# LouisRouss/DiffuLab

Measured on AMD Instinct MI355X. Metric: train images/sec/node (DiT-S/2 flow-matching, 256x256 latents), higher is better.
Workload: dtype bf16

## Files before the change

diffulab_amd/_lib.py:

```python

from __future__ import annotations

import ctypes
import os
import re
from functools import lru_cache

_HERE = os.path.dirname(os.path.abspath(__file__))
LIB_PATH = os.environ.get("DIFFULAB_HIP_LIB") or os.path.join(_HERE, "libdiffulab_hip.so")
HEADER_PATH = os.path.join(os.path.dirname(_HERE), "include", "diffulab_hip.h")

_CTYPES = {
    "int": ctypes.c_int,
    "int32_t": ctypes.c_int32,
    "int64_t": ctypes.c_int64,
    "float": ctypes.c_float,
    "dl_stream_t": ctypes.c_void_p,
}


_VALUE_RETURNING = {"dl_version", "dl_mse_loss_partials", "dl_grad_sumsq", "dl_muon_orthogonalize"}


def _ctype_of(decl: str):
    decl = decl.strip()
    if "*" in decl:
        return ctypes.c_char_p if re.match(r"^(const\s+)?char\s*\*", decl) and "arch" not in decl else ctypes.c_void_p
    base = decl.replace("const", "").split()[0]
    return _CTYPES[base]


def parse_header(path: str = HEADER_PATH) -> dict[str, tuple[object, list[object], list[str]]]:
    text = open(path).read()
    text = re.sub(r"/\*.*?\*/", " ", text, flags=re.S)
    protos: dict[str, tuple[object, list[object], list[str]]] = {}
    for m in re.finditer(r"DL_API\s+([\w\s\*]+?)\s*\b(dl_\w+)\s*\(([^;]*?)\)\s*;", text, flags=re.S):
        ret, name, args = m.group(1).strip(), m.group(2), m.group(3).strip()
        if ret.replace(" ", "") == "constchar*":
            restype = ctypes.c_char_p
        else:
            restype = _CTYPES[ret]
        argtypes, argnames = [], []
        if args and args != "void":
            for a in args.split(","):
                a = " ".join(a.split())
                argnames.append(re.split(r"[\s\*]+", a)[-1])
                argtypes.append(_ctype_of(a))
        protos[name] = (restype, argtypes, argnames)
    return protos


class _Lib:
    def __init__(self) -> None:
        if not os.path.exists(LIB_PATH):
            raise RuntimeError(
                f"{LIB_PATH} not found: build it with `python -c 'import __graft_entry__ as g; g.build()'` "
                "(or `make -C diffulab_amd/csrc`).  There is no CPU / PyTorch fallback for the hot path."
            )
        self.cdll = ctypes.CDLL(LIB_PATH)
        self.protos = parse_header()
        self._fns: dict[str, tuple] = {}
        for name, (restype, argtypes, _) in self.protos.items():
            fn = getattr(self.cdll, name)
            fn.restype = restype
            fn.argtypes = argtypes
            self._fns[name] = (fn, restype is ctypes.c_int and name not in _VALUE_RETURNING)

    def call(self, name: str, *args):
        fn, status = self._fns[name]
        rc = fn(*args)
        if status and rc != 0:
            raise RuntimeError(f"{name} failed ({rc}): {self.cdll.dl_last_error().decode()}")
        return rc


@lru_cache(maxsize=1)
def lib() -> _Lib:
    return _Lib()


def available() -> bool:
    return os.path.exists(LIB_PATH)
```

diffulab_amd/csrc/block.hip:

```cpp
#include <stdlib.h>

#include "common.h"

static thread_local hipEvent_t g_blk_event = nullptr;
static int fork_to_side(hipStream_t main, hipStream_t side) {
  if (main == side) return 0;
  if (!g_blk_event && hipEventCreateWithFlags(&g_blk_event, hipEventDisableTiming) != hipSuccess) return -1;
  if (hipEventRecord(g_blk_event, main) != hipSuccess) return -1;
  return hipStreamWaitEvent(side, g_blk_event, 0) == hipSuccess ? 0 : -1;
}

extern "C" int dl_stream_wait_stream(dl_stream_t waiter, dl_stream_t waited) {
  if (fork_to_side((hipStream_t)waited, (hipStream_t)waiter) != 0) {
    dl_set_error("dl_stream_wait_stream: %s", hipGetErrorString(hipGetLastError()));
    return DL_ERR_LAUNCH;
  }
  return DL_OK;
}
extern "C" int dl_memset_zero(void* p, int64_t bytes, dl_stream_t stream) {
  DL_CHECK_ARG(p && bytes >= 0, "dl_memset_zero: bad args");
  if (bytes && hipMemsetAsync(p, 0, (size_t)bytes, (hipStream_t)stream) != hipSuccess) {
    dl_set_error("dl_memset_zero: %s", hipGetErrorString(hipGetLastError()));
    return DL_ERR_LAUNCH;
  }
  return DL_OK;
}

#define P(k) (b->p[DL_BLK_##k])
#define RUN(call)               \
  do {                          \
    const int rc__ = (call);    \
    if (rc__ != DL_OK) return rc__; \
  } while (0)

static int mlp_up_swiglu(const dl_dit_block_t* b, int train, dl_stream_t stream) {
  const int64_t D = b->D, F = b->F, M = b->B * b->N;
  void* u = train ? P(U) : nullptr;
  if (!u) {
    const int rc = dl_gemm_nt_swiglu_stationary(P(XM2), D, P(W_UP_PERM), b->ldw_d, u, 2 * F, P(H), F, M, F, D, 0, stream);
    if (rc != DL_ERR_UNSUPPORTED) return rc;
  }
  return dl_gemm_nt_swiglu(P(XM2), D, P(W_UP_PERM), b->ldw_d, u, 2 * F, P(H), F, M, F, D, stream);
}

extern "C" int dl_dit_block_fwd(const dl_dit_block_t* b, int train, dl_stream_t stream) {
  DL_CHECK_ARG(b, "dl_dit_block_fwd: null block");
  const int64_t B = b->B, N = b->N, D = b->D, H = b->H, F = b->F, M = B * N, dh = D / H;
  DL_CHECK_ARG(B > 0 && N > 0 && D > 0 && H > 0 && F > 0 && dh == 64, "dl_dit_block_fwd: bad dims (head_dim must be 64)");
  const DlWgCapScope cap_scope(b->max_workgroups);
  const float sm = 0.125f;
  if (b->row_gemms & 1) {
    DL_CHECK_ARG(P(V) == nullptr && P(NEXT_X) && P(NEXT_XM) && P(NEXT_SCALE) && P(NEXT_SHIFT) && P(NEXT_MEAN) && P(NEXT_RSTD),
                 "dl_dit_block_fwd: row_gemms needs V in place and the DL_BLK_NEXT_* slots");
    if ((b->row_gemms & 8) && P(SSQ)) {
      const int rc = dl_dit_block_fwd_chain(b, train, stream);
      if (rc != DL_ERR_UNSUPPORTED) return rc;
    }
    if (P(SSQ)) {
      int rq = dl_gemm_nt_ssq_stationary(P(XM1), D, P(W_QKV), b->ldw_d, P(QKV), 3 * D, M, 3 * D, D, (float*)P(SSQ), 2, 0, stream);
      if (rq == DL_ERR_UNSUPPORTED) rq = dl_gemm_nt_ssq(P(XM1), D, P(W_QKV), b->ldw_d, P(QKV), 3 * D, M, 3 * D, D, (float*)P(SSQ), 2, stream);
      if (rq != DL_OK) return rq;
      RUN(dl_attn_fwd_qkn(P(QKV), (const float*)P(SSQ), (const float*)P(QN_SCALE), (const float*)P(KN_SCALE), (const float*)P(ROPE_COS),
                          (const float*)P(ROPE_SIN), 1e-6f, b->rot, train ? P(Q) : nullptr, train ? P(K) : nullptr,
                          train ? (float*)P(RRMS) : nullptr, P(A), (float*)P(LSE), B, H, N, dh, sm, stream));
    } else if (b->row_gemms & 2) {
      RUN(dl_gemm_nt_qk_norm_rope(P(XM1), D, P(W_QKV), b->ldw_d, B, N, H, dh, b->rot, 1e-6f, (const float*)P(QN_SCALE),
                                  (const float*)P(KN_SCALE), (const float*)P(ROPE_COS), (const float*)P(ROPE_SIN), P(QKV), P(Q), P(K),
                                  (float*)P(RRMS), N, 0, stream));
    } else {
      RUN(dl_gemm_nt(P(XM1), D, P(W_QKV), b->ldw_d, P(QKV), 3 * D, M, 3 * D, D, nullptr, DL_ACT_NONE, DL_BF16, nullptr, nullptr, 0, nullptr,
                     0, 1, stream));
      RUN(dl_qk_norm_rope_fwd(P(QKV), (const float*)P(QN_SCALE), (const float*)P(KN_SCALE), (const float*)P(ROPE_COS),
                              (const float*)P(ROPE_SIN), P(Q), P(K), nullptr, (float*)P(RRMS), B, N, H, dh, b->rot, 1e-6f, stream));
    }
    if (!P(SSQ))
      RUN(dl_attn_fwd_sv(P(Q), P(K), (const char*)P(QKV) + 2 * D * 2, N * 3 * D, dh, 3 * D, P(A), (float*)P(LSE), B, H, N, dh, sm, stream));
    RUN(dl_ln_modulate_gemm_fwd(P(A), D, P(W_PROJ), b->ldw_d, M, D, P(X_IN), P(GATE1), b->ld_mod, (const float*)P(LN2_W),
                                (const float*)P(LN2_B), P(SCALE2), P(SHIFT2), b->ld_mod, N, b->eps, P(T1), P(X1), P(XM2), (float*)P(MEAN2),
                                (float*)P(RSTD2), D, stream));
    RUN(mlp_up_swiglu(b, train, stream));
    RUN(dl_ln_modulate_gemm_fwd(P(H), F, P(W_DOWN), b->ldw_f, M, F, P(X1), P(GATE2), b->ld_mod, (const float*)P(NEXT_LN_W),
                                (const float*)P(NEXT_LN_B), P(NEXT_SCALE), P(NEXT_SHIFT), b->ld_mod, N, b->next_eps, P(T2), P(NEXT_X),
                                P(NEXT_XM), (float*)P(NEXT_MEAN), (float*)P(NEXT_RSTD), D, stream));
    return DL_OK;
  }
  RUN(dl_ln_modulate_fwd(P(PEND_X) ? P(PEND_X) : P(X_IN), (const float*)P(LN1_W), (const float*)P(LN1_B), P(SCALE1), P(SHIFT1),
                         b->ld_mod, N, b->eps, P(XM1), (float*)P(MEAN1), (float*)P(RSTD1), P(PEND_X) ? P(PEND_T) : nullptr,
                         P(PEND_X) ? P(PEND_GATE) : nullptr, b->ld_mod, P(PEND_X) ? P(X_IN) : nullptr, M, D, stream));
  RUN(dl_gemm_nt(P(XM1), D, P(W_QKV), b->ldw_d, P(QKV), 3 * D, M, 3 * D, D, nullptr, DL_ACT_NONE, DL_BF16, nullptr, nullptr, 0, nullptr, 0,
                 1, stream));
  const bool v_in_place = P(V) == nullptr;
  RUN(dl_qk_norm_rope_fwd(P(QKV), (const float*)P(QN_SCALE), (const float*)P(KN_SCALE), (const float*)P(ROPE_COS),
                          (const float*)P(ROPE_SIN), P(Q), P(K), P(V), (float*)P(RRMS), B, N, H, dh, b->rot, 1e-6f, stream));
  if (v_in_place)
    RUN(dl_attn_fwd_sv(P(Q), P(K), (const char*)P(QKV) + 2 * D * 2, N * 3 * D, dh, 3 * D, P(A), (float*)P(LSE), B, H, N, dh, sm, stream));
  else
    RUN(dl_attn_fwd(P(Q), P(K), P(V), P(A), (float*)P(LSE), B, H, N, dh, sm, stream));
  RUN(dl_gemm_nt(P(A), D, P(W_PROJ), b->ldw_d, P(T1), D, M, D, D, nullptr, DL_ACT_NONE, DL_BF16, nullptr, nullptr, 0, nullptr, 0, 1, stream));
  RUN(dl_ln_modulate_fwd(P(X_IN), (const float*)P(LN2_W), (const float*)P(LN2_B), P(SCALE2), P(SHIFT2), b->ld_mod, N, b->eps, P(XM2),
                         (float*)P(MEAN2), (float*)P(RSTD2), P(T1), P(GATE1), b->ld_mod, P(X1), M, D, stream));
  int rc = mlp_up_swiglu(b, train, stream);
  if (rc == DL_ERR_UNSUPPORTED) {
    DL_CHECK_ARG(P(U), "dl_dit_block_fwd: this shape has no fused MLP-up kernel and needs the U buffer");
    RUN(dl_gemm_nt(P(XM2), D, P(W_UP), b->ldw_d, P(U), 2 * F, M, 2 * F, D, nullptr, DL_ACT_NONE, DL_BF16, nullptr, nullptr, 0, nullptr, 0, 1,
                   stream));
    RUN(dl_swiglu_fwd(P(U), P(H), M, F, stream));
  } else if (rc != DL_OK) {
    return rc;
  }
  RUN(dl_gemm_nt(P(H), F, P(W_DOWN), b->ldw_f, P(T2), D, M, D, F, nullptr, DL_ACT_NONE, DL_BF16, nullptr, nullptr, 0, nullptr, 0, 1, stream));
  return DL_OK;
}

extern "C" int dl_dit_block_bwd(const dl_dit_block_t* b, dl_stream_t main_, dl_stream_t side_, int side_wgs) {
  DL_CHECK_ARG(b, "dl_dit_block_bwd: null block");
  hipStream_t main = (hipStream_t)main_, side = (hipStream_t)side_;
  const DlWgCapScope cap_scope(b->max_workgroups);
  const int64_t B = b->B, N = b->N, D = b->D, H = b->H, F = b->F, M = B * N, dh = D / H;
  const float sm = 0.125f;
  dl_wgrad_t wg[4];
  int nwg = 0;
  bool grouped = P(TN_SLAB) != nullptr && ((D % 384 == 0 && F % 192 == 0) || (D % 256 == 0 && F % 256 == 0)) && M % 32 == 0 && M >= 2048;
  auto wgrad = [&](const void* dy, int64_t ldy, const void* x, int64_t ldx, void* g, int64_t Mo, int64_t No) -> int {
    if (grouped) {
      wg[nwg++] = dl_wgrad_t{dy, ldy, x, ldx, (float*)g, Mo, No};
      return DL_OK;
    }
    if (fork_to_side(main, side)) return DL_ERR_LAUNCH;
    return dl_gemm_tn_ex(dy, ldy, x, ldx, (float*)g, No, Mo, No, M, side_wgs, side);
  };
  auto fold = [&](void* partial, void* g) -> int {
    if (fork_to_side(main, side)) return DL_ERR_LAUNCH;
    return dl_reduce_rows_f32((float*)partial, (float*)g, B, 2 * D, 1, side);
  };
  RUN(wgrad(P(DT2), D, P(H), F, P(G_DOWN), D, F));
  if (P(U)) {
    RUN(dl_gemm_nt(P(DT2), D, P(WT_DOWN), b->ldwt_d, P(DH), F, M, F, D, nullptr, DL_ACT_NONE, DL_BF16, nullptr, nullptr, 0, nullptr, 0, 1, main));
    RUN(dl_swiglu_bwd(P(DH), P(U), P(DU), M, F, main));
  } else {
    RUN(dl_mlp_dswiglu_recompute(P(XM2), D, P(W_UP_PERM), b->ldw_d, P(DT2), D, P(WT_DOWN), b->ldwt_d, P(DU), 2 * F, M, F, D, D, main));
  }
  RUN(wgrad(P(DU), 2 * F, P(XM2), D, P(G_UP), 2 * F, D));
  const bool rows = (b->row_gemms & 1) != 0, fold_here = (b->row_gemms & 4) == 0;
  if (rows) {
    RUN(dl_ln_modulate_gemm_bwd(P(DU), 2 * F, P(WT_UP), b->ldwt_f2, M, 2 * F, P(X1), (const float*)P(LN2_W), (const float*)P(LN2_B),
                                P(SCALE2), b->ld_mod, N, (const float*)P(MEAN2), (const float*)P(RSTD2), P(DX_IN), P(DX_MID),
                                (float*)P(DSCALE2), (float*)P(DSHIFT2), b->ld_dmod, (float*)P(DWB2), P(T1), P(GATE1), b->ld_mod, P(DT1),
                                (float*)P(DGATE1), D, main));
  } else {
    RUN(dl_gemm_nt(P(DU), 2 * F, P(WT_UP), b->ldwt_f2, P(DXM), D, M, D, 2 * F, nullptr, DL_ACT_NONE, DL_BF16, nullptr, nullptr, 0, nullptr,
                   0, 1, main));
    RUN(dl_ln_modulate_bwd(P(DXM), P(X1), (const float*)P(LN2_W), (const float*)P(LN2_B), P(SCALE2), b->ld_mod, N,
                           (const float*)P(MEAN2), (const float*)P(RSTD2), P(DX_IN), P(DX_MID), (float*)P(DSCALE2), (float*)P(DSHIFT2),
                           b->ld_dmod, (float*)P(DWB2), P(T1), P(GATE1), b->ld_mod, P(DT1), (float*)P(DGATE1), M, D, main));
  }
  if (fold_here) RUN(fold(P(DWB2), P(G_LN2)));
  RUN(wgrad(P(DT1), D, P(A), D, P(G_PROJ), D, D));
  RUN(dl_gemm_nt(P(DT1), D, P(WT_PROJ), b->ldwt_d, P(DA), D, M, D, D, nullptr, DL_ACT_NONE, DL_BF16, nullptr, nullptr, 0, nullptr, 0, 1, main));
  const bool v_in_place = P(V) == nullptr;
  if (v_in_place && P(QK_PARTIALS) && D <= 512) {
    RUN(dl_attn_bwd_tok(P(Q), P(K), P(QKV), P(A), P(DA), (const float*)P(LSE), P(DQKV), B, H, N, dh, sm, main));
    RUN(dl_qk_norm_rope_bwd_inplace(P(QKV), (const float*)P(QN_SCALE), (const float*)P(KN_SCALE), (const float*)P(ROPE_COS),
                                    (const float*)P(ROPE_SIN), (const float*)P(RRMS), P(DQKV), (float*)P(G_QK_SCALE),
                                    (float*)P(QK_PARTIALS), B, N, H, dh, b->rot, nullptr, main));
  } else {
    if (v_in_place)
      RUN(dl_attn_bwd_sv(P(Q), P(K), (const char*)P(QKV) + 2 * D * 2, N * 3 * D, dh, 3 * D, P(A), P(DA), (const float*)P(LSE), P(DQ), P(DK),
                         (char*)P(DQKV) + 2 * D * 2, N * 3 * D, dh, 3 * D, B, H, N, dh, sm, main));
    else
      RUN(dl_attn_bwd(P(Q), P(K), P(V), P(A), P(DA), (const float*)P(LSE), P(DQ), P(DK), P(DV), B, H, N, dh, sm, main));
    RUN(dl_qk_norm_rope_bwd(P(DQ), P(DK), v_in_place ? nullptr : P(DV), P(QKV), (const float*)P(QN_SCALE), (const float*)P(KN_SCALE),
                            (const float*)P(ROPE_COS), (const float*)P(ROPE_SIN), (const float*)P(RRMS), P(DQKV), (float*)P(G_QK_SCALE), B, N,
                            H, dh, b->rot, main));
  }
  RUN(wgrad(P(DQKV), 3 * D, P(XM1), D, P(G_QKV), 3 * D, D));
  if (grouped) {
    if (fork_to_side(main, side)) return DL_ERR_LAUNCH;
    RUN(dl_gemm_tn_group(wg, nwg, M, (float*)P(TN_SLAB), b->tn_slab_floats, side_wgs, side));
  }
  if (!rows)
    RUN(dl_gemm_nt(P(DQKV), 3 * D, P(WT_QKV), b->ldwt_3d, P(DXM), D, M, D, 3 * D, nullptr, DL_ACT_NONE, DL_BF16, nullptr, nullptr, 0,
                   nullptr, 0, 1, main));
  if (P(DFEAT)) RUN(dl_add_bf16(P(DX_MID), P(DFEAT), P(DX_MID), M * D, main));
  if (rows) {
    RUN(dl_ln_modulate_gemm_bwd(P(DQKV), 3 * D, P(WT_QKV), b->ldwt_3d, M, 3 * D, P(X_IN), (const float*)P(LN1_W), (const float*)P(LN1_B),
                                P(SCALE1), b->ld_mod, N, (const float*)P(MEAN1), (const float*)P(RSTD1), P(DX_MID), P(DX_OUT),
                                (float*)P(DSCALE1), (float*)P(DSHIFT1), b->ld_dmod, (float*)P(DWB1), P(PREV_T2), P(PREV_GATE2), b->ld_mod,
                                P(PREV_DT2), (float*)P(PREV_DGATE2), D, main));
  } else {
    RUN(dl_ln_modulate_bwd(P(DXM), P(X_IN), (const float*)P(LN1_W), (const float*)P(LN1_B), P(SCALE1), b->ld_mod, N,
                           (const float*)P(MEAN1), (const float*)P(RSTD1), P(DX_MID), P(DX_OUT), (float*)P(DSCALE1), (float*)P(DSHIFT1),
                           b->ld_dmod, (float*)P(DWB1), P(PREV_T2), P(PREV_GATE2), b->ld_mod, P(PREV_DT2), (float*)P(PREV_DGATE2), M, D,
                           main));
  }
  if (fold_here) RUN(fold(P(DWB1), P(G_LN1)));
  return DL_OK;
}
```

diffulab_amd/csrc/block_fused.hip:

```cpp
#include <stdlib.h>

#include "common.h"
#include "attention_body.h"
#include "gemm_rows_body.h"
#include "gemm_stationary_body.h"

#define CH_THREADS 512
#define CH_NKS 6

struct ChainRowGemm {
  const bf16_t* A;
  int64_t lda;
  const bf16_t* W;
  int64_t ldw;
  int K;
  RowEpi ep;
};
struct ChainAttn {
  const bf16_t* qkv;
  bf16_t* out;
  float* lse;
  int H;
  float scale;
  QkNorm qn;
};
struct ChainArgs {
  int B;
  StArgs qkv;
  ChainAttn attn;
  ChainRowGemm proj;
  StArgs up;
  ChainRowGemm down;
};

constexpr int ch_max(int a, int b) { return a > b ? a : b; }
constexpr int ch_lds_bytes() { return ch_max(ch_max(st_lds_bytes<CH_NKS>(), 2 * RK_STAGE), attn_pipe_lds_bytes(RK_BN)); }

static __device__ __forceinline__ void ch_phase_sync() {
  asm volatile("s_waitcnt vmcnt(0) lgkmcnt(0)" ::: "memory");
  __builtin_amdgcn_fence(__ATOMIC_RELEASE, "workgroup");
  __syncthreads();
  __builtin_amdgcn_fence(__ATOMIC_ACQUIRE, "workgroup");
}

static __device__ __forceinline__ const ChainArgs* ch_args() {
  auto p = __builtin_amdgcn_kernarg_segment_ptr();
  asm volatile("" : "+s"(p));
  return (const ChainArgs*)p;
}
static __device__ __forceinline__ int ch_tid() {
  int t = threadIdx.x;
  asm volatile("" : "+v"(t));
  return t;
}
static __device__ __forceinline__ void ch_row_gemm(const ChainRowGemm* gp, char* smem, int sample) {
  const ChainRowGemm g = *gp;
  rk_gemm_body<RK_LNF>(g.A, g.lda, g.W, g.ldw, RK_BN, g.K, g.ep, smem, ch_tid(), sample, 0, 1);
}
template <int EPI>
static __device__ __forceinline__ void ch_st_gemm(const StArgs* ap, char* smem, int sample) {
  const StArgs a = *ap;
  st_gemm_body<CH_NKS, EPI>(a, smem, ch_tid(), sample, 0, 1);
}
static __device__ __forceinline__ void ch_attention(const ChainAttn* ap, char* smem, int sample) {
  const ChainAttn a = *ap;
  attn_qkn_pipe_body(a.qkv, a.out, a.lse, a.H, a.scale, a.qn, smem, ch_tid(), sample * a.H, 1, a.H);
}

__global__ __launch_bounds__(CH_THREADS, 2) void dit_block_fwd_chain_k(ChainArgs a) {
  extern __shared__ __attribute__((aligned(16))) char smem[];
  for (int s = blockIdx.x; s < a.B; s += gridDim.x) {
    ch_st_gemm<1>(&ch_args()->qkv, smem, s);
    ch_phase_sync();
    ch_attention(&ch_args()->attn, smem, s);
    ch_phase_sync();
    ch_row_gemm(&ch_args()->proj, smem, s);
    ch_phase_sync();
    ch_st_gemm<0>(&ch_args()->up, smem, s);
    ch_phase_sync();
    ch_row_gemm(&ch_args()->down, smem, s);
    ch_phase_sync();
  }
}

#define P(k) (b->p[DL_BLK_##k])
#define CH_ALIGNED16(p) ((((uintptr_t)(p)) & 15) == 0)

static void ch_row_epi(RowEpi& ep, const void* resid, const void* gate, int64_t ld_gate, const void* ln_w, const void* ln_b,
                       const void* scale, const void* shift, int64_t ld_mod, float eps, void* t_out, void* x_out, void* xm_out,
                       void* mean, void* rstd) {
  ep.resid = (const bf16_t*)resid;
  ep.gate = (const bf16_t*)gate;
  ep.ld_gate = ld_gate;
  ep.ln_w = (const float*)ln_w;
  ep.ln_b = (const float*)ln_b;
  ep.scale = (const bf16_t*)scale;
  ep.shift = (const bf16_t*)shift;
  ep.ld_mod = ld_mod;
  ep.eps = eps;
  ep.t_out = (bf16_t*)t_out;
  ep.x_out = (bf16_t*)x_out;
  ep.xm_out = (bf16_t*)xm_out;
  ep.mean = (float*)mean;
  ep.rstd = (float*)rstd;
}

extern "C" int dl_dit_block_fwd_chain(const dl_dit_block_t* b, int train, dl_stream_t stream) {
  DL_CHECK_ARG(b, "dl_dit_block_fwd_chain: null block");
  const int64_t B = b->B, N = b->N, D = b->D, H = b->H, F = b->F;
  DL_CHECK_ARG(B > 0 && N > 0 && D > 0 && H > 0 && F > 0, "dl_dit_block_fwd_chain: bad dims");
  if (!(b->row_gemms & 1) || !P(SSQ) || P(V) || N != RK_BM || D != RK_BN || D != H * 64 || F % 64 || F % RK_BK ||
      B * N >= (1ll << 31) || F >= (1ll << 30)) {
    dl_set_error("dl_dit_block_fwd_chain: needs row_gemms bit 0, SSQ, V in place, N == 256, D == 384, head_dim == 64, F %% 64 == 0 "
                 "(N=%lld D=%lld H=%lld F=%lld)", (long long)N, (long long)D, (long long)H, (long long)F);
    return DL_ERR_UNSUPPORTED;
  }
  DL_CHECK_ARG(P(XM1) && P(W_QKV) && P(QKV) && P(QN_SCALE) && P(KN_SCALE) && P(LSE) && (!train || (P(Q) && P(K) && P(RRMS))) &&
                   b->rot >= 0 && b->rot % 8 == 0 && b->rot <= 64 && (b->rot == 0 || (P(ROPE_COS) && P(ROPE_SIN))),
               "dl_dit_block_fwd_chain: null qkv / attention operand, or rot not a multiple of 8 up to 64");
  DL_CHECK_ARG(CH_ALIGNED16(P(XM1)) && CH_ALIGNED16(P(W_QKV)) && CH_ALIGNED16(P(QKV)) && CH_ALIGNED16(P(QN_SCALE)) && CH_ALIGNED16(P(KN_SCALE)) &&
                   CH_ALIGNED16(P(ROPE_COS)) && CH_ALIGNED16(P(ROPE_SIN)) && CH_ALIGNED16(P(Q)) && CH_ALIGNED16(P(K)) &&
                   (((uintptr_t)P(SSQ)) & 7) == 0,
               "dl_dit_block_fwd_chain: 16-byte alignment (qkv / attention operands)");
  DL_CHECK_ARG(P(A) && P(W_PROJ) && P(X_IN) && P(GATE1) && P(SCALE2) && P(SHIFT2) && P(T1) && P(X1) && P(XM2) && P(MEAN2) && P(RSTD2) &&
                   P(W_UP_PERM) && P(H) && P(W_DOWN) && P(GATE2) && P(T2) && P(NEXT_X) && P(NEXT_XM) && P(NEXT_SCALE) && P(NEXT_SHIFT) &&
                   P(NEXT_MEAN) && P(NEXT_RSTD),
               "dl_dit_block_fwd_chain: null operand");
  DL_CHECK_ARG((P(LN2_W) == nullptr) == (P(LN2_B) == nullptr) && (P(NEXT_LN_W) == nullptr) == (P(NEXT_LN_B) == nullptr),
               "dl_dit_block_fwd_chain: LayerNorm w and b must both be given or both NULL");
  DL_CHECK_ARG(b->ldw_d % 8 == 0 && b->ldw_f % 8 == 0 && b->ldw_d >= D && b->ldw_f >= F && b->ldw_d < (1ll << 24) && b->ld_mod % 8 == 0,
               "dl_dit_block_fwd_chain: leading dimensions");
  void* u = train ? P(U) : nullptr;
  DL_CHECK_ARG(CH_ALIGNED16(P(A)) && CH_ALIGNED16(P(W_PROJ)) && CH_ALIGNED16(P(X_IN)) && CH_ALIGNED16(P(GATE1)) && CH_ALIGNED16(P(SCALE2)) &&
                   CH_ALIGNED16(P(SHIFT2)) && CH_ALIGNED16(P(T1)) && CH_ALIGNED16(P(X1)) && CH_ALIGNED16(P(XM2)) && CH_ALIGNED16(P(LN2_W)) &&
                   CH_ALIGNED16(P(LN2_B)) && CH_ALIGNED16(P(W_UP_PERM)) && CH_ALIGNED16(u) && CH_ALIGNED16(P(H)) && CH_ALIGNED16(P(W_DOWN)) &&
                   CH_ALIGNED16(P(GATE2)) && CH_ALIGNED16(P(T2)) && CH_ALIGNED16(P(NEXT_X)) && CH_ALIGNED16(P(NEXT_XM)) &&
                   CH_ALIGNED16(P(NEXT_SCALE)) && CH_ALIGNED16(P(NEXT_SHIFT)) && CH_ALIGNED16(P(NEXT_LN_W)) && CH_ALIGNED16(P(NEXT_LN_B)),
               "dl_dit_block_fwd_chain: 16-byte alignment");

  ChainArgs a{};
  a.B = (int)B;
  a.qkv = StArgs{(const bf16_t*)P(XM1), D, (const bf16_t*)P(W_QKV), b->ldw_d, (bf16_t*)P(QKV), 3 * D, nullptr, 0, 0, (float*)P(SSQ), 2,
                 (int)(B * N), (int)(3 * D)};
  a.attn.qkv = (const bf16_t*)P(QKV);
  a.attn.out = (bf16_t*)P(A);
  a.attn.lse = (float*)P(LSE);
  a.attn.H = (int)H;
  a.attn.scale = 0.125f;
  a.attn.qn = QkNorm{(const float*)P(SSQ), (const float*)P(QN_SCALE), (const float*)P(KN_SCALE), (const float*)P(ROPE_COS),
                     (const float*)P(ROPE_SIN), (bf16_t*)(train ? P(Q) : nullptr), (bf16_t*)(train ? P(K) : nullptr),
                     (float*)(train ? P(RRMS) : nullptr), 1.0f / (float)D, 1e-6f, (int)b->rot, (int)(3 * D)};
  a.proj.A = (const bf16_t*)P(A);
  a.proj.lda = D;
  a.proj.W = (const bf16_t*)P(W_PROJ);
  a.proj.ldw = b->ldw_d;
  a.proj.K = (int)D;
  ch_row_epi(a.proj.ep, P(X_IN), P(GATE1), b->ld_mod, P(LN2_W), P(LN2_B), P(SCALE2), P(SHIFT2), b->ld_mod, b->eps, P(T1), P(X1), P(XM2),
             P(MEAN2), P(RSTD2));
  a.up = StArgs{(const bf16_t*)P(XM2), D, (const bf16_t*)P(W_UP_PERM), b->ldw_d, (bf16_t*)u, 2 * F, (bf16_t*)P(H), F, (int)F, nullptr, 0,
                (int)(B * N), (int)(2 * F)};
  a.down.A = (const bf16_t*)P(H);
  a.down.lda = F;
  a.down.W = (const bf16_t*)P(W_DOWN);
  a.down.ldw = b->ldw_f;
  a.down.K = (int)F;
  ch_row_epi(a.down.ep, P(X1), P(GATE2), b->ld_mod, P(NEXT_LN_W), P(NEXT_LN_B), P(NEXT_SCALE), P(NEXT_SHIFT), b->ld_mod, b->next_eps,
             P(T2), P(NEXT_X), P(NEXT_XM), P(NEXT_MEAN), P(NEXT_RSTD));

  constexpr int LDS = ch_lds_bytes();
  static_assert(LDS <= 160 * 1024, "the chain kernel's LDS is the largest phase's");
  static DevOnce once;
  const int n_cu = dev_cus(once, [] {
    (void)hipFuncSetAttribute((const void*)dit_block_fwd_chain_k, hipFuncAttributeMaxDynamicSharedMemorySize, LDS);
  });
  const DlWgCapScope cap_scope(b->max_workgroups);
  const int budget = dl_wg_budget(n_cu);
  int grid = (int)(B < budget ? B : budget);
  if (b->max_workgroups > 0 && b->max_workgroups < grid) grid = b->max_workgroups;
  hipLaunchKernelGGL(dit_block_fwd_chain_k, grid, CH_THREADS, LDS, (hipStream_t)stream, a);
  DL_LAUNCH_CHECK();
  return DL_OK;
}
```

diffulab_amd/csrc/gemm_stationary_body.h:

```cpp
#ifndef DIFFULAB_GEMM_STATIONARY_BODY_H
#define DIFFULAB_GEMM_STATIONARY_BODY_H

#include <type_traits>

#include "common.h"

#define ST_THREADS 512
#define ST_PANEL 256
#define ST_ROWS 64

typedef __attribute__((address_space(3))) void st_lds_void_t;
typedef const __attribute__((address_space(1))) void st_glb_void_t;

struct StArgs {
  const bf16_t* X;
  int64_t ldx;
  const bf16_t* W;
  int64_t ldw;
  bf16_t* C;
  int64_t ldc;
  bf16_t* H;
  int64_t ldh;
  int F;
  float* ssq;
  int ssq_tiles;
  int M, N;
};

template <int NKS>
constexpr int st_lds_bytes() {
  constexpr int STAGE = ST_ROWS * NKS * 128;
  return ((3 * STAGE <= 160 * 1024) ? 3 : 2) * STAGE;
}

template <int N>
__device__ __forceinline__ void st_wait_vmcnt() {
  asm volatile("s_waitcnt vmcnt(%0)" ::"n"(N) : "memory");
}

template <int OFF>
__device__ __forceinline__ void st_lds_read(bf16x8_t& v, unsigned addr) {
  asm volatile("ds_read_b128 %0, %1 offset:%2" : "=v"(v) : "v"(addr), "n"(OFF));
}
template <int N>
__device__ __forceinline__ void st_lds_landed(bf16x8_t& v) {
  asm volatile("s_waitcnt lgkmcnt(%1)" : "+v"(v) : "n"(N));
}

static __device__ __forceinline__ void st_lds_landed_n(int n, bf16x8_t& v) {
  if (n >= 3) st_lds_landed<3>(v);
  else if (n == 2) st_lds_landed<2>(v);
  else if (n == 1) st_lds_landed<1>(v);
  else st_lds_landed<0>(v);
}

template <int NKS, int EPI>
__device__ __forceinline__ void st_gemm_body(const StArgs& a, char* smem, int tid, int first, int stride, int cnt) {
  constexpr int NF = NKS * 4;
  constexpr int PITCH = NKS * 128;
  constexpr int STAGE = ST_ROWS * PITCH;
  constexpr int NST = (3 * STAGE <= 160 * 1024) ? 3 : 2;
  constexpr bool WIDE = (PITCH % 256) == 0;
  constexpr int PD = NKS == 8 ? 2 : 3;
  const int lane = tid & 63, hi = lane >> 5, l31 = lane & 31;
  const int wave = __builtin_amdgcn_readfirstlane(tid >> 6);
  const int S = a.N / ST_ROWS;
  const int total = cnt * S;

  int src_off[NKS];
#pragma unroll
  for (int i = 0; i < NKS; ++i) {
    const int o = (wave * NKS + i) * 1024 + lane * 16;
    const int row = o / PITCH, sl = (o % PITCH) >> 4;
    const int g = WIDE ? (row & 15) : ((row >> 1) & 7);
    src_off[i] = row * (int)a.ldw + ((sl ^ g) << 3);
  }
  int s_it = 0, s_st = 0;
  auto stage_next = [&]() {
    char* base = smem + (s_it % NST) * STAGE + wave * (NKS * 1024);
    const bf16_t* w = a.W + (int64_t)s_st * ST_ROWS * a.ldw;
#pragma unroll
    for (int i = 0; i < NKS; ++i)
      __builtin_amdgcn_global_load_lds((st_glb_void_t*)(w + src_off[i]), (st_lds_void_t*)(base + i * 1024), 16, 0, 0);
    ++s_it;
    if (++s_st == S) s_st = 0;
  };
  const int g_rd = WIDE ? (l31 & 15) : ((l31 >> 1) & 7);
  const int rd_base = l31 * PITCH, rd_x = (hi ^ g_rd) << 4;
  const unsigned smem_lds = (unsigned)(uintptr_t)(st_lds_void_t*)smem;

  f32x16_t acc[4];
#pragma unroll
  for (int j = 0; j < 4; ++j)
#pragma unroll
    for (int r = 0; r < 16; ++r) acc[j][r] = 0.f;
  bf16x8_t x[NF];
  const bool upper = wave >= 4;
  int m = 0;
  float ss = 0.f;
  float ss_lo = 0.f;

#pragma unroll
  for (int s = 0; s < NST - 1; ++s)
    if (s < total) stage_next();

  auto epilogue = [&](auto half_tag, int st) {
    constexpr int HALF = decltype(half_tag)::value;
    const int n_base = st * ST_ROWS;
    if constexpr (EPI == 0) {
#pragma unroll
      for (int j = 0; j < 2; ++j) {
        f32x16_t& c = acc[2 * HALF + j];
        const int u0 = ((n_base + j * 32) >> 1) + 8 * hi;
        float v1[8], v3[8], hv[8], h8[8];
#pragma unroll
        for (int e = 0; e < 8; ++e) hv[e] = silu_f(c[e]) * c[8 + e];
#pragma unroll
        for (int e = 0; e < 4; ++e) {
          auto s1 = __builtin_amdgcn_permlane32_swap(__float_as_uint(c[e]), __float_as_uint(c[4 + e]), false, false);
          auto s3 = __builtin_amdgcn_permlane32_swap(__float_as_uint(c[8 + e]), __float_as_uint(c[12 + e]), false, false);
          auto sh = __builtin_amdgcn_permlane32_swap(__float_as_uint(hv[e]), __float_as_uint(hv[4 + e]), false, false);
          v1[e] = __uint_as_float(s1[0]);
          v1[4 + e] = __uint_as_float(s1[1]);
          v3[e] = __uint_as_float(s3[0]);
          v3[4 + e] = __uint_as_float(s3[1]);
          h8[e] = __uint_as_float(sh[0]);
          h8[4 + e] = __uint_as_float(sh[1]);
        }
#pragma unroll
        for (int e = 0; e < 16; ++e) c[e] = 0.f;
        if (a.C) {
          *(u32x4_t*)(a.C + (int64_t)m * a.ldc + u0) = pack8(v1);
          *(u32x4_t*)(a.C + (int64_t)m * a.ldc + a.F + u0) = pack8(v3);
        }
        *(u32x4_t*)(a.H + (int64_t)m * a.ldh + u0) = pack8(h8);
      }
    } else {
#pragma unroll
      for (int j = 0; j < 2; ++j)
#pragma unroll
        for (int gp = 0; gp < 2; ++gp) {
          f32x16_t& c = acc[2 * HALF + j];
          float v[8];
#pragma unroll
          for (int e = 0; e < 4; ++e) {
            auto sw2 = __builtin_amdgcn_permlane32_swap(__float_as_uint(c[8 * gp + e]), __float_as_uint(c[8 * gp + 4 + e]), false, false);
            v[e] = __uint_as_float(sw2[0]);
            v[4 + e] = __uint_as_float(sw2[1]);
            c[8 * gp + e] = 0.f;
            c[8 * gp + 4 + e] = 0.f;
          }
          const u32x4_t pk = pack8(v);
          *(u32x4_t*)(a.C + (int64_t)m * a.ldc + n_base + j * 32 + 16 * gp + 8 * hi) = pk;
          float r[8];
          unpack8(pk, r);
#pragma unroll
          for (int e = 0; e < 8; ++e) ss += r[e] * r[e];
        }
      if (st % 6 == 2) {
        ss_lo = xor32_sum(ss);
        ss = 0.f;
      }
      if ((st + 1) % 6 == 0 || st + 1 == S) {
        if (st / 6 < a.ssq_tiles) {
          const float t = ss_lo + xor32_sum(ss);
          if (hi == 0) a.ssq[(int64_t)m * a.ssq_tiles + st / 6] = t;
        }
        ss = 0.f;
        ss_lo = 0.f;
      }
    }
  };

  int it = 0;
  auto stage = [&](auto half_tag, int st) {
    constexpr int HALF = decltype(half_tag)::value;
    constexpr int YOUNG = (NST - 2) * NKS;
    if (it + NST - 2 < total) {
      if (st < 2) st_wait_vmcnt<YOUNG>();
      else if (EPI == 1) st_wait_vmcnt<YOUNG + 4>();
      else if (a.C) st_wait_vmcnt<YOUNG + 6>();
      else st_wait_vmcnt<YOUNG + 2>();
    } else {
      st_wait_vmcnt<0>();
    }
    __builtin_amdgcn_s_barrier();
    if (NST < 3 && s_it < total) stage_next();
    if (upper && st > 0) epilogue(std::integral_constant<int, 1 - HALF>{}, st - 1);
    const unsigned sw = smem_lds + (it % NST) * STAGE + rd_base;
    bf16x8_t wq[PD + 1];
    auto rd = [&](int s) {
      const int f = s >> 1;
      const unsigned ad = sw + (((f & 7) << 5) ^ rd_x);
      bf16x8_t& v = wq[s % (PD + 1)];
      switch ((f >> 3) * 2 + (s & 1)) {
        case 0: st_lds_read<0>(v, ad); break;
        case 1: st_lds_read<32 * PITCH>(v, ad); break;
        case 2: st_lds_read<256>(v, ad); break;
        case 3: st_lds_read<32 * PITCH + 256>(v, ad); break;
        case 4: st_lds_read<512>(v, ad); break;
        case 5: st_lds_read<32 * PITCH + 512>(v, ad); break;
        case 6: st_lds_read<768>(v, ad); break;
        default: st_lds_read<32 * PITCH + 768>(v, ad); break;
      }
    };
#pragma unroll
    for (int s = 0; s < PD; ++s) rd(s);
#pragma unroll
    for (int s = 0; s < 2 * NF; ++s) {
      __builtin_amdgcn_sched_barrier(0);
      if (s + PD < 2 * NF) rd(s + PD);
      st_lds_landed_n(2 * NF - 1 - s < PD ? 2 * NF - 1 - s : PD, wq[s % (PD + 1)]);
      acc[2 * HALF + (s & 1)] =
          __builtin_amdgcn_mfma_f32_32x32x16_bf16(wq[s % (PD + 1)], x[s >> 1], acc[2 * HALF + (s & 1)], 0, 0, 0);
    }
    __builtin_amdgcn_sched_barrier(0);
    if (NST >= 3 && s_it < total) stage_next();
    if (!upper) epilogue(half_tag, st);
    ++it;
  };

  int panel = first;
  for (int p = 0; p < cnt; ++p, panel += stride) {
    m = panel * ST_PANEL + wave * 32 + l31;
    {
      const bf16_t* xr = a.X + (int64_t)m * a.ldx + hi * 8;
#pragma unroll
      for (int f = 0; f < NF; ++f) x[f] = *(const bf16x8_t*)(xr + f * 16);
      st_wait_vmcnt<0>();
#pragma unroll
      for (int f = 0; f < NF; ++f) asm volatile("" : "+v"(x[f]));
    }
    for (int st = 0; st < S; st += 2) {
      stage(std::integral_constant<int, 0>{}, st);
      stage(std::integral_constant<int, 1>{}, st + 1);
    }
    if (upper) epilogue(std::integral_constant<int, 1>{}, S - 1);
  }
}

#endif
```

diffulab_amd/csrc/norm.hip:

```cpp
#include <stdlib.h>

#include "common.h"

#define MAXJ 2
#define ROW_MAX_D 4096

template <int NJ, int S = 64>
__device__ __forceinline__ void load_row(const bf16_t* __restrict__ p, int D8, int lane, float (&v)[NJ][8]) {
#pragma unroll
  for (int j = 0; j < NJ; ++j) {
    const int c = lane + S * j;
    if (c < D8) {
      unpack8(*(const u32x4_t*)(p + c * 8), v[j]);
    } else {
#pragma unroll
      for (int e = 0; e < 8; ++e) v[j][e] = 0.f;
    }
  }
}
template <int NJ, int S = 64>
__device__ __forceinline__ void load_row_f32(const float* __restrict__ p, int D8, int lane, float (&v)[NJ][8], float fill) {
#pragma unroll
  for (int j = 0; j < NJ; ++j) {
    const int c = lane + S * j;
// ... 1207 lines not shown
                                   const float* rrms, void* dqkv, float* dscale, int64_t B, int64_t N, int64_t H,
                                   int64_t dh, int64_t rot, const int32_t* pos, int64_t n_dst, int64_t n_off, dl_stream_t stream);
extern "C" int dl_qk_norm_rope_bwd(const void* dq, const void* dk, const void* dv, const void* qkv,
                                   const float* scale_q, const float* scale_k, const float* cos, const float* sin,
                                   const float* rrms, void* dqkv, float* dscale, int64_t B, int64_t N, int64_t H,
                                   int64_t dh, int64_t rot, dl_stream_t stream) {
  return dl_qk_norm_rope_bwd_ex(dq, dk, dv, qkv, scale_q, scale_k, cos, sin, rrms, dqkv, dscale, B, N, H, dh, rot, nullptr, N, 0, stream);
}
extern "C" int dl_qk_norm_rope_bwd_ex(const void* dq, const void* dk, const void* dv, const void* qkv,
                                   const float* scale_q, const float* scale_k, const float* cos, const float* sin,
                                   const float* rrms, void* dqkv, float* dscale, int64_t B, int64_t N, int64_t H,
                                   int64_t dh, int64_t rot, const int32_t* pos, int64_t n_dst, int64_t n_off, dl_stream_t stream) {
  DL_CHECK_ARG(dq && dk && qkv && scale_q && scale_k && cos && sin && rrms && dqkv && dscale && B > 0 && N > 0,
               "dl_qk_norm_rope_bwd: null operand");
  const int64_t D = H * dh;
  DL_CHECK_ARG(H > 0 && D <= ROW_MAX_D, "dl_qk_norm_rope_bwd: inner width H * dh = %lld (at most 4096)", (long long)D);
  DL_CHECK_ARG(dh % 8 == 0 && rot % 8 == 0 && rot <= dh && n_off >= 0 && n_off + N <= n_dst,
               "dl_qk_norm_rope_bwd: bad dims (dh=%lld rot=%lld, rows [%lld, %lld) of n_dst=%lld)", (long long)dh, (long long)rot,
               (long long)n_off, (long long)(n_off + N), (long long)n_dst);
  const int64_t M = B * N;
  int grid = cdiv(M, M >= 32768 ? 4 * 16 : 4 * 4);
  if (grid > 1024) grid = 1024;
  if (grid < 1) grid = 1;
  const int nj = cdiv(D, 512);
  if (nj > 2) {
    const int grid_r = (int)(cdiv(M, 16) < 1024 ? cdiv(M, 16) : 1024);
#define LAUNCH_ROWS(NJ)                                                                                                        \
  hipLaunchKernelGGL(qk_norm_rope_bwd_rows_k<NJ>, grid_r, 256, 0, (hipStream_t)stream, (const bf16_t*)dq, (const bf16_t*)dk, \
                     (const bf16_t*)dv, (const bf16_t*)qkv, scale_q, scale_k, cos, sin, rrms, (bf16_t*)dqkv, dscale, M,       \
                     (int)N, (int)H, (int)dh, (int)rot, pos, (int)n_dst, (int)n_off)
    if (D <= 2048) LAUNCH_ROWS(1);
    else LAUNCH_ROWS(2);
#undef LAUNCH_ROWS
    DL_LAUNCH_CHECK();
    return DL_OK;
  }
  const size_t lds = (size_t)4 * 2 * D * sizeof(float);
#define QKB_KERN_1 qk_norm_rope_bwd_k
#define QKB_KERN_2 qk_norm_rope_bwd_wide_k
#define LAUNCH(NJ)                                                                                                   \
  hipLaunchKernelGGL(QKB_KERN_##NJ, grid, 256, lds, (hipStream_t)stream, (const bf16_t*)dq, (const bf16_t*)dk, \
                     (const bf16_t*)dv, (const bf16_t*)qkv, scale_q, scale_k, cos, sin, rrms, (bf16_t*)dqkv, dscale, M, \
                     (int)N, (int)H, (int)dh, (int)rot, pos, (int)n_dst, (int)n_off)
  if (nj == 1) LAUNCH(1);
  else LAUNCH(2);
#undef LAUNCH
  DL_LAUNCH_CHECK();
  return DL_OK;
}

template <int OCC>
__device__ __forceinline__ void qk_norm_rope_bwd_inplace_body(
    const bf16_t* __restrict__ qkv, const float* __restrict__ sq, const float* __restrict__ sk, const float* __restrict__ cs,
    const float* __restrict__ sn, const float* __restrict__ rrms, bf16_t* dqkv, float* __restrict__ partials, int64_t M, int N,
    int H, int dh, int rot, const int* __restrict__ pos) {
  extern __shared__ __attribute__((aligned(16))) char smem[];
  float* red = (float*)smem;
  const int lane = threadIdx.x & 63, wave = threadIdx.x >> 6;
  const int D = H * dh, D8 = D >> 3;
  const bool on = lane < D8;
  const float invD = 1.0f / (float)D;
  const int col = lane * 8, hh = on ? col / dh : 0, d0 = col - hh * dh;
  const bool rope = on && d0 < rot;
  float wq[8], wk[8], aq[8], ak[8];
#pragma unroll
  for (int e = 0; e < 8; ++e) {
    wq[e] = on ? sq[col + e] : 0.f;
    wk[e] = on ? sk[col + e] : 0.f;
    aq[e] = ak[e] = 0.f;
  }
  const int64_t stride = (int64_t)gridDim.x * 4;
  u32x4_t nxq = {0, 0, 0, 0}, nxk = nxq, ngq = nxq, ngk = nxq;
  f32x4_t ncc = {0.f, 0.f, 0.f, 0.f}, nss = ncc;
  float nrq = 0.f, nrk = 0.f;
  auto fetch = [&](int64_t r) {
    const bf16_t* p = qkv + r * 3 * D + col;
    const bf16_t* g = dqkv + r * 3 * D + col;
    if (on) {
      nxq = *(const u32x4_t*)p;
      nxk = *(const u32x4_t*)(p + D);
      ngq = *(const u32x4_t*)g;
      ngk = *(const u32x4_t*)(g + D);
    }
    nrq = rrms[r * 2];
    nrk = rrms[r * 2 + 1];
    if (rope) {
      const int nt = pos ? pos[r] : (int)(r % N);
      ncc = *(const f32x4_t*)(cs + (int64_t)nt * (rot >> 1) + (d0 >> 1));
      nss = *(const f32x4_t*)(sn + (int64_t)nt * (rot >> 1) + (d0 >> 1));
    }
  };
  int64_t row = (int64_t)blockIdx.x * 4 + wave;
  if (row < M) fetch(row);
  for (; row < M; row += stride) {
    float xq[8], xk[8], gq[8], gk[8];
    unpack8(nxq, xq);
    unpack8(nxk, xk);
    unpack8(ngq, gq);
    unpack8(ngk, gk);
    const f32x4_t cc = ncc, ss = nss;
    const float rq = nrq, rk = nrk;
    if (row + stride < M) fetch(row + stride);
    if (rope) {
#pragma unroll
      for (int i = 0; i < 4; ++i) {
        const float qa = gq[2 * i], qb = gq[2 * i + 1], ka = gk[2 * i], kb = gk[2 * i + 1];
        gq[2 * i] = qa * cc[i] + qb * ss[i];
        gq[2 * i + 1] = -qa * ss[i] + qb * cc[i];
        gk[2 * i] = ka * cc[i] + kb * ss[i];
        gk[2 * i + 1] = -ka * ss[i] + kb * cc[i];
      }
    }
    float s1 = 0.f, s2 = 0.f;
#pragma unroll
    for (int e = 0; e < 8; ++e) {
      aq[e] += gq[e] * xq[e] * rq;
      ak[e] += gk[e] * xk[e] * rk;
      gq[e] *= wq[e];
      gk[e] *= wk[e];
      s1 += gq[e] * xq[e];
      s2 += gk[e] * xk[e];
    }
    const float mq = wave_sum(s1) * invD * rq * rq * rq, mk = wave_sum(s2) * invD * rk * rk * rk;
#pragma unroll
    for (int e = 0; e < 8; ++e) {
      gq[e] = rq * gq[e] - xq[e] * mq;
      gk[e] = rk * gk[e] - xk[e] * mk;
    }
    if (on) {
      bf16_t* o = dqkv + row * 3 * D + col;
      *(u32x4_t*)o = pack8(gq);
      *(u32x4_t*)(o + D) = pack8(gk);
    }
  }
  if (on) {
#pragma unroll
    for (int e = 0; e < 8; ++e) {
      red[(size_t)wave * 2 * D + col + e] = aq[e];
      red[(size_t)wave * 2 * D + D + col + e] = ak[e];
    }
  }
  __syncthreads();
  for (int i = threadIdx.x; i < 2 * D; i += 256)
    partials[(size_t)blockIdx.x * 2 * D + i] = (red[i] + red[2 * D + i]) + (red[4 * D + i] + red[6 * D + i]);
}
#define QKI_ARGS                                                                                                                  \
  const bf16_t *__restrict__ qkv, const float *__restrict__ sq, const float *__restrict__ sk, const float *__restrict__ cs,         \
      const float *__restrict__ sn, const float *__restrict__ rrms, bf16_t *dqkv, float *__restrict__ partials, int64_t M, int N, \
      int H, int dh, int rot, const int *__restrict__ pos
__global__ __launch_bounds__(256) void qk_norm_rope_bwd_inplace_k(QKI_ARGS) {
  qk_norm_rope_bwd_inplace_body<3>(qkv, sq, sk, cs, sn, rrms, dqkv, partials, M, N, H, dh, rot, pos);
}
#define FOLD_LANES 16
__global__ __launch_bounds__(64 * FOLD_LANES) void fold_rows_k(const float* __restrict__ partial, float* __restrict__ out, int G, int n) {
  __shared__ float red[FOLD_LANES][64];
  const int cl = threadIdx.x & 63, rl = threadIdx.x >> 6;
  const int c = blockIdx.x * 64 + cl;
  float a0 = 0.f, a1 = 0.f, a2 = 0.f, a3 = 0.f;
  if (c < n) {
    const float* p = partial + c;
    int g = rl;
    for (; g + 3 * FOLD_LANES < G; g += 4 * FOLD_LANES) {
      a0 += p[(size_t)g * n];
      a1 += p[(size_t)(g + FOLD_LANES) * n];
      a2 += p[(size_t)(g + 2 * FOLD_LANES) * n];
      a3 += p[(size_t)(g + 3 * FOLD_LANES) * n];
    }
    for (; g < G; g += FOLD_LANES) a0 += p[(size_t)g * n];
  }
  red[rl][cl] = (a0 + a1) + (a2 + a3);
  __syncthreads();
  float t = 0.f;
  if (rl < 4) t = (red[rl][cl] + red[rl + 4][cl]) + (red[rl + 8][cl] + red[rl + 12][cl]);
  __syncthreads();
  if (rl < 4) red[rl][cl] = t;
  __syncthreads();
  if (rl == 0 && c < n) out[c] += (red[0][cl] + red[1][cl]) + (red[2][cl] + red[3][cl]);
}
int dl_fold_rows_launch(const float* partial, float* out, int G, int n, hipStream_t stream) {
  hipLaunchKernelGGL(fold_rows_k, cdiv(n, 64), 64 * FOLD_LANES, 0, stream, partial, out, G, n);
  DL_LAUNCH_CHECK();
  return DL_OK;
}
extern "C" int dl_qk_norm_rope_bwd_inplace(const void* qkv, const float* scale_q, const float* scale_k, const float* cos,
                                           const float* sin, const float* rrms, void* dqkv, float* dscale, float* dscale_partials,
                                           int64_t B, int64_t N, int64_t H, int64_t dh, int64_t rot, const int32_t* pos,
                                           dl_stream_t stream) {
  DL_CHECK_ARG(qkv && scale_q && scale_k && cos && sin && rrms && dqkv && dscale && dscale_partials && B > 0 && N > 0,
               "dl_qk_norm_rope_bwd_inplace: null operand");
  const int64_t D = H * dh;
  if (D > 512 || D % 8) {
    dl_set_error("dl_qk_norm_rope_bwd_inplace: inner width %lld (one wave owns a row of at most 512 columns)", (long long)D);
    return DL_ERR_UNSUPPORTED;
  }
  DL_CHECK_ARG(dh % 8 == 0 && rot % 8 == 0 && rot <= dh, "dl_qk_norm_rope_bwd_inplace: dh=%lld rot=%lld", (long long)dh, (long long)rot);
  DL_CHECK_ARG((((uintptr_t)qkv | (uintptr_t)dqkv | (uintptr_t)cos | (uintptr_t)sin) & 15) == 0,
               "dl_qk_norm_rope_bwd_inplace: 16-byte alignment");
  const int64_t M = B * N;
  int grid = cdiv(M, M >= 32768 ? 4 * 16 : 4 * 4);
  if (grid > 768) grid = 768;
  const size_t lds = (size_t)4 * 2 * D * sizeof(float);
  hipLaunchKernelGGL(qk_norm_rope_bwd_inplace_k, grid, 256, lds, (hipStream_t)stream, (const bf16_t*)qkv, scale_q, scale_k, cos, sin,
                     rrms, (bf16_t*)dqkv, dscale_partials, M, (int)N, (int)H, (int)dh, (int)rot, pos);
  hipLaunchKernelGGL(fold_rows_k, cdiv(2 * D, 64), 64 * FOLD_LANES, 0, (hipStream_t)stream, dscale_partials, dscale, grid, (int)(2 * D));
  DL_LAUNCH_CHECK();
  return DL_OK;
}

__global__ void swiglu_fwd_k(const bf16_t* __restrict__ u, bf16_t* __restrict__ h, int64_t M, int F8) {
  const int64_t total = M * F8, stride = (int64_t)gridDim.x * blockDim.x;
  for (int64_t i = (int64_t)blockIdx.x * blockDim.x + threadIdx.x; i < total; i += stride) {
    const int64_t row = i / F8;
    const int c = (int)(i - row * F8);
    const bf16_t* p = u + row * (int64_t)F8 * 16 + c * 8;
    float a[8], b[8];
    unpack8(*(const u32x4_t*)p, a);
    unpack8(*(const u32x4_t*)(p + (int64_t)F8 * 8), b);
#pragma unroll
    for (int e = 0; e < 8; ++e) a[e] = silu_f(a[e]) * b[e];
    *(u32x4_t*)(h + row * (int64_t)F8 * 8 + c * 8) = pack8(a);
  }
}
__global__ void swiglu_bwd_k(const bf16_t* __restrict__ dh, const bf16_t* __restrict__ u, bf16_t* __restrict__ du,
                             int64_t M, int F8) {
  const int64_t total = M * F8, stride = (int64_t)gridDim.x * blockDim.x;
  for (int64_t i = (int64_t)blockIdx.x * blockDim.x + threadIdx.x; i < total; i += stride) {
    const int64_t row = i / F8;
    const int c = (int)(i - row * F8);
    const int64_t uo = row * (int64_t)F8 * 16 + c * 8;
    float a[8], b[8], g[8], da[8], db[8];
    unpack8(*(const u32x4_t*)(u + uo), a);
    unpack8(*(const u32x4_t*)(u + uo + (int64_t)F8 * 8), b);
    unpack8(*(const u32x4_t*)(dh + row * (int64_t)F8 * 8 + c * 8), g);
#pragma unroll
    for (int e = 0; e < 8; ++e) {
      da[e] = g[e] * b[e] * dsilu_f(a[e]);
      db[e] = g[e] * silu_f(a[e]);
    }
    *(u32x4_t*)(du + uo) = pack8(da);
    *(u32x4_t*)(du + uo + (int64_t)F8 * 8) = pack8(db);
  }
}
extern "C" int dl_swiglu_fwd(const void* u, void* h, int64_t M, int64_t F, dl_stream_t stream) {
  DL_CHECK_ARG(u && h && M > 0 && F > 0 && F % 8 == 0, "dl_swiglu_fwd: bad args");
  int64_t g = (M * (F / 8) + 255) / 256;
  if (g > 4096) g = 4096;
  hipLaunchKernelGGL(swiglu_fwd_k, (int)g, 256, 0, (hipStream_t)stream, (const bf16_t*)u, (bf16_t*)h, M, (int)(F / 8));
  DL_LAUNCH_CHECK();
  return DL_OK;
}
extern "C" int dl_swiglu_bwd(const void* dh, const void* u, void* du, int64_t M, int64_t F, dl_stream_t stream) {
  DL_CHECK_ARG(dh && u && du && M > 0 && F > 0 && F % 8 == 0, "dl_swiglu_bwd: bad args");
  int64_t g = (M * (F / 8) + 255) / 256;
  if (g > 4096) g = 4096;
  hipLaunchKernelGGL(swiglu_bwd_k, (int)g, 256, 0, (hipStream_t)stream, (const bf16_t*)dh, (const bf16_t*)u,
                     (bf16_t*)du, M, (int)(F / 8));
  DL_LAUNCH_CHECK();
  return DL_OK;
}
```

diffulab_amd/engine.py:

```python

from __future__ import annotations

import functools
import math
from dataclasses import dataclass, field

import torch
from torch import Tensor

from . import ops, tuning


_PARAM_EPOCH = 0


def bump_param_epoch() -> None:
    global _PARAM_EPOCH
    _PARAM_EPOCH += 1


def _must(ok: bool) -> None:
    if not ok:
        raise RuntimeError("a HIP kernel declined a shape the engine had selected it for")

# ... 347 lines not shown

    def params_changed(self) -> None:
        self.manual_version += 1

    def _z(self, *shape, dtype: torch.dtype = torch.bfloat16) -> Tensor:
        with torch.inference_mode(False):
            return torch.zeros(*shape, device=self.dev, dtype=dtype)

    def _zr(self, rows: int, *rest, dtype: torch.dtype = torch.bfloat16) -> Tensor:
        return self._z(_rup(rows, 64), *rest, dtype=dtype)[:rows]

    def _cached(self, key: tuple) -> bool:
        if key == self._ws_key:
            return True
        if key in self._ws_cache:
            self.ws, self.geo = self._ws_cache[key]
            self._ws_key = key
            return True
        return False

    def _publish(self, w: dict, key: tuple, geo: tuple, rope_key: tuple, rope_fn) -> None:
        self.ws, self._ws_key, self.geo = w, key, geo
        if len(self._ws_cache) >= 8:
            self._ws_cache.pop(next(iter(self._ws_cache)))
        self._ws_cache[key] = (w, geo)
        if rope_key not in self._rope:
            c, s = rope_fn()
            self._rope[rope_key] = (c.to(self.dev), s.to(self.dev))

    def _cond_buffers(self, w: dict, B: int, H: int, W: int, train: bool, grouped: bool) -> None:
        d, z, f32 = self.d, self._z, torch.float32
        D, E, p = d.inner_dim, d.embedding_dim, d.patch_size
        M, Bp, Fo, R = B * (H // p) * (W // p), _rup(B, 64), p * p * d.output_channels, self.layout.mod_rows
        w["tokP"] = z(M, self._ki)
        w["temb"], w["pre1"], w["h1"] = z(Bp, d.frequency_embedding), z(Bp, E), z(Bp, E)
        w["e"], w["emb"], w["se"] = z(Bp, E, dtype=f32), z(Bp, E, dtype=f32), z(Bp, E)
        w["mod"] = z(Bp, R)
        if self._pooled_dim:
            w["poolP"], w["ppre1"], w["ph1"], w["pe"] = z(Bp, _rup(self._pooled_dim, 64)), z(Bp, 2 * E), z(Bp, 2 * E), z(Bp, E, dtype=f32)
            if train:
                w["dph1"], w["dppre1"] = z(Bp, 2 * E, dtype=f32), z(Bp, 2 * E)
        w["meanf"], w["rstdf"], w["xf"] = z(M, dtype=f32), z(M, dtype=f32), z(M, D)
        w["otok"] = z(M, _rup(Fo, 8), dtype=f32)
        w["pred"] = z(B, d.output_channels, H, W, dtype=f32)
        if not train:
            return
        w["dO"] = z(M, self._ko)
        w["dmod"] = z(Bp, R)
        w["dmod32"] = z(Bp, R, dtype=f32)
        w["dse"], w["demb"], w["demb16"] = z(Bp, E, dtype=f32), z(Bp, E, dtype=f32), z(Bp, E)
        w["dh1"], w["dpre1"] = z(Bp, E, dtype=f32), z(Bp, E)
        w["scr_last"], w["scr_conv"] = z(_rup(Fo, 8), D, dtype=f32), z(D, self._ki, dtype=f32)
        w["det_scr"] = torch.empty(max(2 * R * E, 1 << 22), device=self.dev, dtype=f32)
        if grouped:
            w["tn_slab"] = torch.empty(ops.WgradGroups.slab_floats(D, d.mlp_ratio * D), device=self.dev, dtype=f32)

    def _grouped_widths(self) -> bool:
        return ops.WgradGroups.widths_ok(self.d.inner_dim, self.d.mlp_ratio * self.d.inner_dim) and tuning.on("DL_WGRAD_GROUP")

    def _dit_block_buffers(self, B: int, nt: int, train: bool, nq: int | None = None) -> dict:
        d, z, f32 = self.d, self._z, torch.float32
        D, Hh, F, mt = d.inner_dim, d.num_heads, d.mlp_ratio * d.inner_dim, B * nt
        nq = nt if nq is None else nq
        a = {"x0": z(mt, D), "mean1": z(mt, dtype=f32), "rstd1": z(mt, dtype=f32), "xm1": z(mt, D), "qkv": z(mt, 3 * D),
             "q": z(B, Hh, nq, 64), "k": z(B, Hh, nq, 64), "v": z(B, Hh, nq, 64), "rrms": z(mt, 2, dtype=f32), "a": z(mt, D),
             "lse": z(B, Hh, nq, dtype=f32), "t1": z(mt, D), "x1": z(mt, D), "mean2": z(mt, dtype=f32), "rstd2": z(mt, dtype=f32),
             "xm2": z(mt, D), "u": ops.mlp_u_buffer(z, mt, D, F, train), "h": z(mt, F), "t2": z(mt, D)}
        if train:
            a["wg"] = {"dt2": z(mt, D), "du": z(mt, 2 * F), "dt1": z(mt, D), "dqkv": z(mt, 3 * D)}
        return a

    def _joint_stream_buffers(self, B: int, nt: int, train: bool) -> dict:
        d, zr, f32 = self.d, self._zr, torch.float32
        D, F, mt = d.inner_dim, d.mlp_ratio * d.inner_dim, B * nt
        a = {"x0": zr(mt, D), "mean1": zr(mt, dtype=f32), "rstd1": zr(mt, dtype=f32), "xm1": zr(mt, D), "qkv": zr(mt, 3 * D),
             "rrms": zr(mt, 2, dtype=f32), "a": zr(mt, D), "t1": zr(mt, D), "x1": zr(mt, D), "mean2": zr(mt, dtype=f32),
             "rstd2": zr(mt, dtype=f32), "xm2": zr(mt, D), "u": ops.mlp_u_buffer(zr, mt, D, F, train), "h": zr(mt, F), "t2": zr(mt, D)}
        if train:
            a["wg"] = {"dt2": zr(mt, D), "du": zr(mt, 2 * F), "dt1": zr(mt, D), "dqkv": zr(mt, 3 * D)}
            a["dwb"] = self._z(2, B, 2, D, dtype=f32)
        return a

    def _single_stream_buffers(self, B: int, T: int, train: bool) -> dict:
        d, zr, f32 = self.d, self._zr, torch.float32
        D, F, mt = d.inner_dim, d.mlp_ratio * d.inner_dim, B * T
        a = {"x0": zr(mt, D), "mean": zr(mt, dtype=f32), "rstd": zr(mt, dtype=f32), "m": zr(mt, D), "qkv": zr(mt, 3 * D),
             "rrms": zr(mt, 2, dtype=f32), "a": zr(mt, D), "ta": zr(mt, D), "u": ops.mlp_u_buffer(zr, mt, D, F, train), "h": zr(mt, F),
             "t": zr(mt, D)}
        if train:
            a["wg"] = {"dt": zr(mt, D), "du": zr(mt, 2 * F), "dqkv": zr(mt, 3 * D)}
            a["dwb"] = self._z(1, B, 2, D, dtype=f32)
        return a

    def _joint_attn_buffers(self, B: int, Tp: int) -> dict:
        z, Hh = self._z, self.d.num_heads
        return {"ao": z(B * Tp, self.d.inner_dim), "lse": z(B, Hh, Tp, dtype=torch.float32), "q": z(B, Hh, Tp, 64),
                "k": z(B, Hh, Tp, 64), "v": z(B, Hh, Tp, 64)}

    def _alloc(self, B: int, H: int, W: int, train: bool) -> None:
        key = (B, H, W, train)
        if self._cached(key):
            return
        d, z = self.d, self._z
        D, p, L = d.inner_dim, d.patch_size, d.depth
        gh, gw = H // p, W // p
        N = gh * gw
        M = B * N
        pad = ops.attn_needs_padding(N)
        Nd = _rup(N, 256) if pad else N
        if pad and type(self) is DiTEngine and Nd <= ops.ATTN_MAX_TOKENS and M % 64:
            raise NotImplementedError(f"token grid {gh}x{gw} ({N} tokens) in the bf16 regime: batch * tokens must be a multiple of 64 (got "
                                      f"{B} * {N}); the fp32 regime (precision_type=\"no\" / set_precision(\"fp32\")) takes any grid and batch")
        if Nd > ops.ATTN_MAX_TOKENS or (pad and type(self) is not DiTEngine):
            raise NotImplementedError(f"token grid {gh}x{gw}: the bf16 regime's attention takes up to {ops.ATTN_MAX_TOKENS} tokens"
                                      + ("" if type(self) is DiTEngine else ", N % 64 == 0 up to 256 or N % 256 == 0 beyond, in this engine")
                                      + f" (got {N}); the fp32 regime (precision_type=\"no\" / set_precision(\"fp32\")) takes any grid")
        Bp = _rup(B, 64)
        Fo = p * p * d.output_channels
        ops.check_row_extent(B * Nd, max(2 * d.mlp_ratio * D, 6 * D), "DiT bf16 path")
        f32 = torch.float32
        w: dict[str, object] = {}
        self._cond_buffers(w, B, H, W, train, train and self._grouped_wgrad(M))
        nl = L if train else 1
        F_ = d.mlp_ratio * D
        rc_u = train and type(self) is DiTEngine and ops.mlp_recompute_ok(M, D, F_)
        w["mlp_recompute"] = rc_u
        w["x"] = [z(M, D) for _ in range((L + 1) if train else 2)]
        per = []
        for _ in range(nl):
            per.append({
                "mean1": z(M, dtype=f32), "rstd1": z(M, dtype=f32), "xm1": z(M, D), "qkv": z(M, 3 * D),
                "q": z(B, d.num_heads, Nd, 64), "k": z(B, d.num_heads, Nd, 64),
                "v": None if ops.v_in_place(N) else z(B, d.num_heads, Nd, 64),
                "ao": z(B * Nd, D) if pad else None,
                "rrms": z(M, 2, dtype=f32), "a": z(M, D), "lse": z(B, d.num_heads, Nd, dtype=f32), "t1": z(M, D),
                "x1": z(M, D), "mean2": z(M, dtype=f32), "rstd2": z(M, dtype=f32), "xm2": z(M, D),
                "u": None if rc_u else z(M, 2 * d.mlp_ratio * D), "h": z(M, d.mlp_ratio * D), "t2": z(M, D),
            })
        w["layers"] = per
        if pad:
            w["kb"] = z(B, Nd, dtype=f32)
            w["kb"][:, N:] = float("-inf")
        if self._qkn_on_load(M, N):
            w["ssq_all"] = z(L, M, 2, dtype=f32)
        if train:
            w["dxa"], w["dxb"] = z(M, D), z(M, D)
            w["dxm"], w["da"] = z(M, D), z(M, D)
            w["dh"] = z(M, d.mlp_ratio * D)
            w["wg"] = [{"dt2": z(M, D), "du": z(M, 2 * d.mlp_ratio * D), "dt1": z(M, D), "dqkv": z(M, 3 * D)}
                       for _ in range(L)]
            if ops.v_in_place(N) and D <= 512 and M >= 32768 and type(self) is DiTEngine and tuning.on("DL_QK_INPLACE"):
                w["qk_part"] = torch.empty(1024 * 2 * D, device=self.dev, dtype=f32)
                w["dq"] = w["dk"] = None
            else:
                w["dq"], w["dk"] = z(B, d.num_heads, Nd, 64), z(B, d.num_heads, Nd, 64)
            w["dv"] = None if ops.v_in_place(N) else z(B, d.num_heads, Nd, 64)
            if pad:
                w["dao"] = z(B * Nd, D)
            w["dwb"] = z(2 * L, B, 2, D, dtype=f32)
        self._publish(w, key, (B, H, W, gh, gw, N, M, Bp, Fo), (gh, gw), lambda: rope_grid_tables(gh, gw, d.rope_axes_dim, d.rope_base))

    def _stem_fwd(self, x: Tensor, t: Tensor, y_eff: Tensor | None, x0: Tensor | None = None, patch_gemm: bool = True) -> Tensor:
        d, w, sh = self.d, self.ws, self.sh
        B, _, _, _, _, _, M, _, _ = self.geo
        D, E = d.inner_dim, d.embedding_dim
        ops.patchify(x, w["tokP"], d.patch_size, ops.PATCH_CPP)
        if patch_gemm:
            ops.gemm_nt(w["tokP"], sh[self._conv_name + "|f"], w["x"][0] if x0 is None else x0, M=M, N=D, K=self._ki)
        ops.timestep_embedding(t, w["temb"][:B])
        ops.gemm_nt(w["temb"], sh["time_embed.0.weight|f"], w["h1"], bias=self.P("time_embed.0.bias"), act=ops.ACT_SILU,
                    pre_out=w["pre1"], M=B, N=E, K=d.frequency_embedding)
        ops.gemm_nt(w["h1"], sh["time_embed.2.weight|f"], w["e"], bias=self.P("time_embed.2.bias"), M=B, N=E, K=E)
        if self._pooled_dim:
            self._pooled_fwd(B)
        else:
            table = self.P("label_embed.embedding.weight") if d.n_classes is not None else None
            ops.cond_combine_fwd(w["e"][:B], table, y_eff if table is not None else None, w["emb"][:B], w["se"][:B])
        mod_bias = self.params[self.layout.entries[self.layout.mod_b0][0] :][: self.layout.mod_rows]
        ops.gemm_nt(w["se"], sh["@mod|f"], w["mod"], bias=mod_bias, M=B, N=self.layout.mod_rows, K=E)
        return w["mod"]

    def _pooled_fwd(self, B: int) -> None:
        d, w, sh = self.d, self.ws, self.sh
        E, P = d.embedding_dim, self._pooled_dim
        pooled = self.pooled
        assert pooled is not None and tuple(pooled.shape) == (B, P), "pooled context embedding [B, pooled_dim] not set for this step"
        w["poolP"][:B, :P].copy_(pooled)
        ops.gemm_nt(w["poolP"], sh["mlp_pooled_context.0.weight|f"], w["ph1"], bias=self.P("mlp_pooled_context.0.bias"), act=ops.ACT_SILU,
                    pre_out=w["ppre1"], M=B, N=2 * E, K=w["poolP"].shape[1])
        ops.gemm_nt(w["ph1"], sh["mlp_pooled_context.2.weight|f"], w["pe"], bias=self.P("mlp_pooled_context.2.bias"), M=B, N=E, K=2 * E)
        ops.cond_combine_dense_fwd(w["e"][:B], w["pe"][:B], w["emb"][:B], w["se"][:B])

    def _pooled_bwd(self, B: int, det: Tensor | None) -> None:
        d, w, sh = self.d, self.ws, self.sh
        E, P = d.embedding_dim, self._pooled_dim
        ops.colsum(w["demb"], self.G("mlp_pooled_context.2.bias"), B, E, scratch=det)
        ops.gemm_tn(w["demb16"], w["ph1"], self.G("mlp_pooled_context.2.weight"), scratch=det)
        ops.gemm_nt(w["demb16"], sh["mlp_pooled_context.2.weight|t"], w["dph1"], M=B, N=2 * E, K=E)
        ops.silu_bwd(w["dph1"][:B], w["ppre1"][:B], w["dppre1"][:B])
        ops.gemm_tn(w["dppre1"], w["poolP"], self.G("mlp_pooled_context.0.weight"), M=2 * E, N=P, scratch=det)
        ops.colsum(w["dppre1"], self.G("mlp_pooled_context.0.bias"), B, 2 * E, scratch=det)

    def _main_wgs(self) -> int:
        explicit = tuning.integer("DL_MAIN_WGS", 0)
        if explicit:
            return explicit
        reserve = tuning.integer("DL_DP_RESERVE_CUS", 0)
        if reserve and self.reducer is not None and getattr(self.reducer, "enabled", True):
            if getattr(self, "_cus", None) is None:
                self._cus = torch.cuda.get_device_properties(self.dev).multi_processor_count
            return max(8, (self._cus - reserve) & ~7)
        return 0

    def _native_blocks(self) -> bool:
        return type(self) is DiTEngine and tuning.on("DL_NATIVE_BLOCK") and not (self.geo is not None and ops.attn_needs_padding(self.geo[5]))

    def _block_args(self, i: int, train: bool):
        key = (self._ws_key, i, self.reducer is None, self._main_wgs())
        blk = self._blk_cache.get(key)
        if blk is not None:
            return blk
        from ._block import DitBlock

        d, w, sh = self.d, self.ws, self.sh
        B, _, _, gh, gw, N, M, Bp, Fo = self.geo
        D, L, F = d.inner_dim, d.depth, d.mlp_ratio * d.inner_dim
        pre, mo = f"layers.{i}.", i * 6 * D
        mod, xs = w["mod"], w["x"]
        a = w["layers"][i if train else 0]
        xin = xs[i] if train else xs[i & 1]
        cos, sin = self._rope[(gh, gw)]
        mrow = lambda off: mod.data_ptr() + 2 * off
        blk = DitBlock()
        blk.B, blk.N, blk.D, blk.H, blk.F = B, N, D, d.num_heads, F
        blk.ld_mod = mod.stride(0)
        blk.ldw_d, blk.ldw_f = sh[pre + "attention.qkv.weight|f"].stride(0), sh[pre + "mlp_input.2.weight|f"].stride(0)
        blk.ldwt_d, blk.ldwt_f2 = sh[pre + "attention.proj_out.weight|t"].stride(0), sh[pre + "mlp_input.0.weight|t"].stride(0)
        blk.ldwt_3d = sh[pre + "attention.qkv.weight|t"].stride(0)
        blk.rot, blk.eps = sum(d.rope_axes_dim), 1e-5
        blk.max_workgroups = self._main_wgs()
        prev = None
        if i > 0:
            ap = w["layers"][(i - 1) if train else 0]
            prev = (ap["x1"], ap["t2"], mrow((i - 1) * 6 * D + 5 * D))
        blk.set(x_in=xin, pend_x=prev[0] if prev else None, pend_t=prev[1] if prev else None, pend_gate=prev[2] if prev else None,
                scale1=mrow(mo), shift1=mrow(mo + D), gate1=mrow(mo + 2 * D), scale2=mrow(mo + 3 * D), shift2=mrow(mo + 4 * D),
                gate2=mrow(mo + 5 * D),
                ln1_w=self.P(pre + "norm_1.weight"), ln1_b=self.P(pre + "norm_1.bias"), ln2_w=self.P(pre + "norm_2.weight"),
                ln2_b=self.P(pre + "norm_2.bias"), qn_scale=self.P(pre + "attention.qk_norm.query_norm.scale"),
                kn_scale=self.P(pre + "attention.qk_norm.key_norm.scale"),
                w_qkv=sh[pre + "attention.qkv.weight|f"], w_proj=sh[pre + "attention.proj_out.weight|f"],
                w_up=sh[pre + "mlp_input.0.weight|f"], w_up_perm=sh[pre + "mlp_input.0.weight|g"], w_down=sh[pre + "mlp_input.2.weight|f"],
                wt_qkv=sh[pre + "attention.qkv.weight|t"], wt_proj=sh[pre + "attention.proj_out.weight|t"],
                wt_up=sh[pre + "mlp_input.0.weight|t"], wt_down=sh[pre + "mlp_input.2.weight|t"], rope_cos=cos, rope_sin=sin,
                xm1=a["xm1"], mean1=a["mean1"], rstd1=a["rstd1"], qkv=a["qkv"], q=a["q"], k=a["k"], v=a["v"], rrms=a["rrms"], a=a["a"],
                lse=a["lse"], t1=a["t1"], x1=a["x1"], xm2=a["xm2"], mean2=a["mean2"], rstd2=a["rstd2"], u=a["u"], h=a["h"], t2=a["t2"],
                ssq=w["ssq_all"][i] if "ssq_all" in w else None)
        rows = self._row_gemms(M, N)
        blk.row_gemms = 0
        if rows:
            if i + 1 < L:
                nx, mn, nxt = w["layers"][(i + 1) if train else 0], (i + 1) * 6 * D, f"layers.{i + 1}."
                lnw, lnb, blk.next_eps = self.P(nxt + "norm_1.weight"), self.P(nxt + "norm_1.bias"), 1e-5
                xm_n, mu_n, rs_n = nx["xm1"], nx["mean1"], nx["rstd1"]
            else:
                mn, lnw, lnb, blk.next_eps = L * 6 * D, None, None, 1e-6
                xm_n, mu_n, rs_n = w["xf"], w["meanf"], w["rstdf"]
            blk.set(next_ln_w=lnw, next_ln_b=lnb, next_scale=mrow(mn), next_shift=mrow(mn + D),
                    next_x=xs[i + 1] if train else xs[(i + 1) & 1], next_xm=xm_n, next_mean=mu_n, next_rstd=rs_n)
            blk.row_gemms = (1 | (2 if tuning.on("DL_ROW_GEMM_QK") else 0) | (4 if self.reducer is None else 0)
                             | (8 if tuning.on("DL_BLOCK_CHAIN") else 0))
        if train and self.grads is not None:
            g, dmod = w["wg"][i], w["dmod32"]
            blk.ld_dmod = dmod.stride(0)
            drow = lambda off: dmod.data_ptr() + 4 * off
            pg = None
            if i > 0:
                mp = (i - 1) * 6 * D
                pg = (w["layers"][i - 1]["t2"], mrow(mp + 5 * D), w["wg"][i - 1]["dt2"], drow(mp + 5 * D))
            blk.set(dt2=g["dt2"], dx_in=w["dxa"], dx_mid=w["dxb"], dx_out=w["dxa"], dh=w["dh"], du=g["du"], dxm=w["dxm"], dt1=g["dt1"],
                    da=w["da"], dq=w["dq"], dk=w["dk"], dv=w["dv"], dqkv=g["dqkv"], dfeat=None,
                    dscale1=drow(mo), dshift1=drow(mo + D), dgate1=drow(mo + 2 * D), dscale2=drow(mo + 3 * D), dshift2=drow(mo + 4 * D),
                    dwb1=w["dwb"][2 * i], dwb2=w["dwb"][2 * i + 1],
                    prev_t2=pg[0] if pg else None, prev_gate2=pg[1] if pg else None, prev_dt2=pg[2] if pg else None,
                    prev_dgate2=pg[3] if pg else None,
                    g_qkv=self.G(pre + "attention.qkv.weight"), g_proj=self.G(pre + "attention.proj_out.weight"),
                    g_up=self.G(pre + "mlp_input.0.weight"), g_down=self.G(pre + "mlp_input.2.weight"),
                    g_ln1=self.G(pre + "norm_1.weight"), g_ln2=self.G(pre + "norm_2.weight"),
                    g_qk_scale=self.G(pre + "attention.qk_norm.query_norm.scale"), tn_slab=w.get("tn_slab"),
                    qk_partials=w.get("qk_part"))
            blk.tn_slab_floats = w["tn_slab"].numel() if "tn_slab" in w else 0
        self._blk_cache[key] = blk
        return blk

    def forward(self, x: Tensor, t: Tensor, y_eff: Tensor | None, train: bool = True, refresh: bool = True) -> Tensor:
        d = self.d
        B, C, H, W = x.shape
        assert C == d.input_channels and x.dtype == torch.float32 and x.is_cuda
        self._alloc(B, H, W, train)
        if refresh:
            self.refresh_shadows(force=train)
        w, sh = self.ws, self.sh
        _, _, _, gh, gw, N, M, _, _ = self.geo
        D, L = d.inner_dim, d.depth
        cos, sin = self._rope[(gh, gw)]
        self._train = train
        self._yeff = y_eff

        fused = self._row_gemms(M, N)
        if "ssq_all" in w:
            w["ssq_all"].zero_()
        mod = self._stem_fwd(x, t, y_eff, patch_gemm=not fused)
        xs = w["x"]
        if fused:
            if self._native_blocks():
                a0 = w["layers"][0]
                _must(ops.ln_modulate_gemm_fwd(w["tokP"], sh[self._conv_name + "|f"], None, None, self.P("layers.0.norm_1.weight"),
                                               self.P("layers.0.norm_1.bias"), mod[:, 0:D], mod[:, D : 2 * D], N, 1e-5, None, xs[0],
                                               a0["xm1"], a0["mean1"], a0["rstd1"], K=self._ki))
                for i in range(L):
                    ops.dit_block_fwd(self._block_args(i, train), train)
            else:
                self._forward_row_gemms(mod, train)
            return self._head_fwd(None, w["xf"])

        pend = None
        native = self._native_blocks()
        for i in range(L):
            a = w["layers"][i if train else 0]
            if native:
                ops.dit_block_fwd(self._block_args(i, train), train)
                pend = (a["x1"], a["t2"], mod[:, i * 6 * D + 5 * D : i * 6 * D + 6 * D])
                continue
            pend = self._dit_block_fwd(a, f"layers.{i}.", xs[i] if train else xs[i & 1], pend, Modulation(mod, None, i * 6 * D, D, N), N,
                                       cos, sin, kb=w.get("kb"))
        return self._head_fwd(Modulation(mod, None, L * 6 * D, D, N), xs[L] if train else xs[L & 1], pend)

    def _half1_fwd(self, a: dict, nm: dict, xin: Tensor, pend: tuple | None, m: Modulation, nt: int, cos: Tensor, sin: Tensor,
                   q: Tensor, k: Tensor, v: Tensor | None, pos: Tensor | None = None, n_off: int = 0) -> None:
        n1w, n1b = self.P(nm["n1"] + ".weight"), self.P(nm["n1"] + ".bias")
        if pend is None:
            ops.ln_modulate_fwd(xin, n1w, n1b, m.col(0), m.col(1), m.rows, 1e-5, a["xm1"], a["mean1"], a["rstd1"])
        else:
            ops.ln_modulate_fwd(pend[0], n1w, n1b, m.col(0), m.col(1), m.rows, 1e-5, a["xm1"], a["mean1"], a["rstd1"], t=pend[1],
                                gate=pend[2], x_out=xin)
        ops.gemm_nt(a["xm1"], self.sh[nm["qkv"] + ".weight|f"], a["qkv"])
        ops.qk_norm_rope_fwd(a["qkv"], self.P(nm["qk"] + ".query_norm.scale"), self.P(nm["qk"] + ".key_norm.scale"), cos, sin, q, k, v,
                             a["rrms"], self.geo[0], nt, self.d.num_heads, 64, sum(self.d.rope_axes_dim), pos=pos, n_off=n_off)

    def _half2_fwd(self, a: dict, nm: dict, xin: Tensor, m: Modulation) -> tuple:
        sh = self.sh
        ops.gemm_nt(a["a"], sh[nm["proj"] + ".weight|f"], a["t1"])
        ops.ln_modulate_fwd(xin, self.P(nm["n2"] + ".weight"), self.P(nm["n2"] + ".bias"), m.col(3), m.col(4), m.rows, 1e-5, a["xm2"],
                            a["mean2"], a["rstd2"], t=a["t1"], gate=m.col(2), x_out=a["x1"])
        u = a["u"] if self._train else None
        if not ops.gemm_nt_swiglu(a["xm2"], sh[nm["up"] + ".weight|g"], u, a["h"], stationary=u is None):
            assert a["u"] is not None, "the recompute mode is only chosen for shapes the fused MLP-up kernel serves"
            ops.gemm_nt(a["xm2"], sh[nm["up"] + ".weight|f"], a["u"])
            ops.swiglu_fwd(a["u"], a["h"])
        ops.gemm_nt(a["h"], sh[nm["down"] + ".weight|f"], a["t2"])
        return a["x1"], a["t2"], m.col(5)

    def _attn_fwd(self, a: dict, nt: int, kb: Tensor | None) -> None:
        B, Hh, D = self.geo[0], self.d.num_heads, self.d.inner_dim
        if a.get("ao") is not None:
            Np = a["q"].shape[2]
            ops.attn_fwd_ex(a["q"], a["k"], a["v"], a["ao"], a["lse"], B, Hh, Np, Np, 64, 64**-0.5, kb)
            ops.copy_rows3d(a["ao"], Np * D, D, a["a"], nt * D, D, B, nt, D)
        elif ops.v_in_place(nt):
            ops.attn_fwd_qkv(a["q"], a["k"], a["qkv"], a["a"], a["lse"], B, Hh, nt, 64, 64**-0.5)
        else:
            ops.attn_fwd(a["q"], a["k"], a["v"], a["a"], a["lse"], B, Hh, nt, 64, 64**-0.5)

    def _dit_block_fwd(self, a: dict, pre: str, xin: Tensor, pend: tuple | None, m: Modulation, nt: int, cos: Tensor, sin: Tensor,
                       pos: Tensor | None = None, kb: Tensor | None = None) -> tuple:
        nm = block_names(pre)
        self._half1_fwd(a, nm, xin, pend, m, nt, cos, sin, a["q"], a["k"], None if ops.v_in_place(nt) else a["v"], pos)
        self._attn_fwd(a, nt, kb)
        return self._half2_fwd(a, nm, xin, m)

    def _head_fwd(self, m: Modulation | None, x: Tensor, pend: tuple | None = None) -> Tensor:
        w = self.ws
        M, Fo = self.geo[6], self.geo[8]
        if m is not None and pend is None:
            ops.ln_modulate_fwd(x, None, None, m.col(0), m.col(1), m.rows, 1e-6, w["xf"], w["meanf"], w["rstdf"])
        elif m is not None:
            ops.ln_modulate_fwd(pend[0], None, None, m.col(0), m.col(1), m.rows, 1e-6, w["xf"], w["meanf"], w["rstdf"], t=pend[1],
                                gate=pend[2], x_out=x)
        ops.gemm_nt(w["xf"], self.sh["last_layer.linear.weight|f"], w["otok"], bias=self.P("last_layer.linear.bias"), M=M, N=Fo,
                    K=self.d.inner_dim)
        ops.unpatchify(w["otok"], w["pred"], self.d.patch_size)
        return w["pred"]

    def _half2_bwd(self, a: dict, g: dict, nm: dict, s: dict, m: Modulation, dx: Tensor | None, sw: "SideWork") -> Tensor:
        sh = self.sh
        sw.wgrad(g["dt2"], a["h"], nm["down"] + ".weight")
        ops.mlp_swiglu_bwd(g["dt2"], sh[nm["down"] + ".weight|t"], a["xm2"], sh[nm["up"] + ".weight|g"], a["u"], s["dh"], g["du"])
        sw.wgrad(g["du"], a["xm2"], nm["up"] + ".weight")
        ops.gemm_nt(g["du"], sh[nm["up"] + ".weight|t"], s["dxm"])
        nx = _other(s, dx)
        m.ln_bwd(s["dxm"], a["x1"], self.P(nm["n2"] + ".weight"), self.P(nm["n2"] + ".bias"), 3, a["mean2"], a["rstd2"], dx, nx,
                 m.part[1], gate=(a["t1"], m.off + 2 * m.D, g["dt1"]))
        sw.fold(m.part[1], nm["n2"] + ".weight", m.groups)
        sw.wgrad(g["dt1"], a["a"], nm["proj"] + ".weight")
        ops.gemm_nt(g["dt1"], sh[nm["proj"] + ".weight|t"], s["da"])
        return nx

    def _half1_bwd(self, a: dict, g: dict, nm: dict, s: dict, m: Modulation, xin: Tensor, dx: Tensor | None, prev: tuple | None,
                   dres: Tensor | None, sw: "SideWork") -> Tensor:
        sw.wgrad(g["dqkv"], a["xm1"], nm["qkv"] + ".weight")
        ops.gemm_nt(g["dqkv"], self.sh[nm["qkv"] + ".weight|t"], s["dxm"])
        if dres is not None and dx is not None:
            ops.add_bf16(dx, dres, dx)
        nx = _other(s, dx)
        m.ln_bwd(s["dxm"], xin, self.P(nm["n1"] + ".weight"), self.P(nm["n1"] + ".bias"), 0, a["mean1"], a["rstd1"], dx, nx, m.part[0],
                 gate=prev)
        sw.fold(m.part[0], nm["n1"] + ".weight", m.groups)
        return nx

    def _attn_bwd(self, a: dict, g: dict, nm: dict, s: dict, nt: int, cos: Tensor, sin: Tensor, pos: Tensor | None,
                  kb: Tensor | None, dao: Tensor | None) -> None:
        w = self.ws
        B, Hh, D, rot = self.geo[0], self.d.num_heads, self.d.inner_dim, sum(self.d.rope_axes_dim)
        sq, sk = self.P(nm["qk"] + ".query_norm.scale"), self.P(nm["qk"] + ".key_norm.scale")
        dscale = self._qk_scale_sink(nm["qk"]) if self._input_only else self.G(nm["qk"] + ".query_norm.scale")
        if ops.qk_inplace_ok(w, B, nt):
            ops.attn_bwd_tok(a["q"], a["k"], a["qkv"], a["a"], s["da"], a["lse"], g["dqkv"], B, Hh, nt, 64, 64**-0.5)
            _must(ops.qk_norm_rope_bwd_inplace(a["qkv"], sq, sk, cos, sin, a["rrms"], g["dqkv"], dscale, w["qk_part"], B, nt, Hh, 64, rot,
                                                pos=pos))
            return
        v_in_place = ops.v_in_place(nt)
        if a.get("ao") is not None:
            Np = a["q"].shape[2]
            ops.copy_rows3d(s["da"], nt * D, D, dao, Np * D, D, B, nt, D)
            ops.attn_bwd_ex(a["q"], a["k"], a["v"], a["ao"], dao, a["lse"], s["dq"], s["dk"], s["dv"], B, Hh, Np, Np, 64, 64**-0.5, kb)
        elif v_in_place:
            ops.attn_bwd_qkv(a["q"], a["k"], a["qkv"], a["a"], s["da"], a["lse"], s["dq"], s["dk"], g["dqkv"], B, Hh, nt, 64, 64**-0.5)
        else:
            ops.attn_bwd(a["q"], a["k"], a["v"], a["a"], s["da"], a["lse"], s["dq"], s["dk"], s["dv"], B, Hh, nt, 64, 64**-0.5)
        ops.qk_norm_rope_bwd(s["dq"], s["dk"], None if v_in_place else s["dv"], a["qkv"], sq, sk, cos, sin, a["rrms"], g["dqkv"], dscale,
                             B, nt, Hh, 64, rot, pos=pos)

    def _dit_block_bwd(self, a: dict, g: dict, pre: str, xin: Tensor, dx: Tensor, prev: tuple | None, dres: Tensor | None, s: dict,
                       m: Modulation, nt: int, cos: Tensor, sin: Tensor, sw: "SideWork", pos: Tensor | None = None,
                       kb: Tensor | None = None, dao: Tensor | None = None) -> Tensor:
        nm = block_names(pre)
        dx = self._half2_bwd(a, g, nm, s, m, dx, sw)
        self._attn_bwd(a, g, nm, s, nt, cos, sin, pos, kb, dao)
        return self._half1_bwd(a, g, nm, s, m, xin, dx, prev, dres, sw)

    def _grouped_wgrad(self, M: int) -> bool:
        D, F = self.d.inner_dim, self.d.mlp_ratio * self.d.inner_dim
        return (type(self) is DiTEngine and ops.WgradGroups.shapes_ok(D, F, M) and tuning.on("DL_WGRAD_GROUP"))

    def _qkn_on_load(self, M: int, N: int) -> bool:
        return (self._row_gemms(M, N) and self.d.inner_dim % 384 == 0 and (M // 256) * (3 * self.d.inner_dim // 384) >= 64
                and tuning.on("DL_QKN_ON_LOAD") and not tuning.on("DL_ROW_GEMM_QK"))

    def _row_gemms(self, M: int, N: int) -> bool:
        return type(self) is DiTEngine and ops.v_in_place(N) and ops.row_gemm_ok(M, self.d.inner_dim, N)

    def _forward_row_gemms(self, mod: Tensor, train: bool) -> None:
        d, w, sh = self.d, self.ws, self.sh
        B, _, _, gh, gw, N, M, _, _ = self.geo
        D, L, Hh = d.inner_dim, d.depth, d.num_heads
        cos, sin = self._rope[(gh, gw)]
        rot = sum(d.rope_axes_dim)
        xs = w["x"]
        lay = lambda i: w["layers"][i if train else 0]
        xbuf = lambda i: xs[i] if train else xs[i & 1]
        fused_qk = tuning.on("DL_ROW_GEMM_QK")
        a0 = lay(0)
        _must(ops.ln_modulate_gemm_fwd(w["tokP"], sh[self._conv_name + "|f"], None, None, self.P("layers.0.norm_1.weight"),
                                        self.P("layers.0.norm_1.bias"), mod[:, 0:D], mod[:, D : 2 * D], N, 1e-5, None, xbuf(0),
                                        a0["xm1"], a0["mean1"], a0["rstd1"], K=self._ki))
        for i in range(L):
            a, xin, pre, mo = lay(i), xbuf(i), f"layers.{i}.", i * 6 * D
            if "ssq_all" in w:
                ssq = w["ssq_all"][i]
                _must(ops.gemm_nt_ssq(a["xm1"], sh[pre + "attention.qkv.weight|f"], a["qkv"], ssq, stationary=True))
                ops.attn_fwd_qkn(a["qkv"], ssq, self.P(pre + "attention.qk_norm.query_norm.scale"),
                                 self.P(pre + "attention.qk_norm.key_norm.scale"), cos, sin, a["q"] if train else None,
                                 a["k"] if train else None, a["rrms"] if train else None, a["a"], a["lse"], B, Hh, N, 64, rot, 64**-0.5)
            elif fused_qk:
                _must(ops.gemm_nt_qk_norm_rope(a["xm1"], sh[pre + "attention.qkv.weight|f"],
                                                self.P(pre + "attention.qk_norm.query_norm.scale"),
                                                self.P(pre + "attention.qk_norm.key_norm.scale"), cos, sin, a["qkv"], a["q"], a["k"],
                                                a["rrms"], B, N, Hh, 64, rot))
            else:
                ops.gemm_nt(a["xm1"], sh[pre + "attention.qkv.weight|f"], a["qkv"])
                ops.qk_norm_rope_fwd(a["qkv"], self.P(pre + "attention.qk_norm.query_norm.scale"),
                                     self.P(pre + "attention.qk_norm.key_norm.scale"), cos, sin, a["q"], a["k"], None, a["rrms"], B, N,
                                     Hh, 64, rot)
            if "ssq_all" not in w:
                ops.attn_fwd_qkv(a["q"], a["k"], a["qkv"], a["a"], a["lse"], B, Hh, N, 64, 64**-0.5)
            _must(ops.ln_modulate_gemm_fwd(a["a"], sh[pre + "attention.proj_out.weight|f"], xin, mod[:, mo + 2 * D : mo + 3 * D],
                                            self.P(pre + "norm_2.weight"), self.P(pre + "norm_2.bias"), mod[:, mo + 3 * D : mo + 4 * D],
                                            mod[:, mo + 4 * D : mo + 5 * D], N, 1e-5, a["t1"], a["x1"], a["xm2"], a["mean2"], a["rstd2"]))
            u = a["u"] if train else None
            if not ops.gemm_nt_swiglu(a["xm2"], sh[pre + "mlp_input.0.weight|g"], u, a["h"], stationary=u is None):
                raise RuntimeError("the row-complete path needs the fused MLP-up kernel")
            if i + 1 < L:
                nx, mn, nxt = lay(i + 1), (i + 1) * 6 * D, f"layers.{i + 1}."
                lnw, lnb, eps = self.P(nxt + "norm_1.weight"), self.P(nxt + "norm_1.bias"), 1e-5
                xm_n, mu_n, rs_n = nx["xm1"], nx["mean1"], nx["rstd1"]
            else:
                mn, lnw, lnb, eps = L * 6 * D, None, None, 1e-6
                xm_n, mu_n, rs_n = w["xf"], w["meanf"], w["rstdf"]
            _must(ops.ln_modulate_gemm_fwd(a["h"], sh[pre + "mlp_input.2.weight|f"], a["x1"], mod[:, mo + 5 * D : mo + 6 * D], lnw, lnb,
                                            mod[:, mn : mn + D], mod[:, mn + D : mn + 2 * D], N, eps, a["t2"], xbuf(i + 1), xm_n, mu_n,
                                            rs_n))

    def _jstage_fwd(self, blocks, x_in: Tensor, c_in: Tensor, nx: int, pos: Tensor | None, kb: Tensor, x_out: Tensor | None,
                    c_out: Tensor | None) -> tuple | None:
        d, w = self.d, self.ws
        B, Lc = self.geo[0], self._Lc
        D, Hh = d.inner_dim, d.num_heads
        cos, sin = self._tabs
        mod = w["mod"]
        Tp = kb.shape[1]
        streams = (("input", nx, Lc, 0, pos), ("context", Lc, 0, 6 * D, None))
        cur = {"input": x_in, "context": c_in}
        pend: dict[str, tuple | None] = {"input": None, "context": None}
        blocks = list(blocks)
        for bi in blocks:
            per, pre, base = w["blk"][bi], self.prefixes[bi], self.layout.mod_off[bi]
            q, k, v = (per["q"], per["k"], per["v"]) if "q" in per else (w["q"], w["k"], w["v"])
            for st, nt, off, mc, ps in streams:
                a = per[st]
                a["xin"] = cur[st] if pend[st] is None else a["x0"]
                self._half1_fwd(a, block_names(pre, st), a["xin"], pend[st], Modulation(mod, None, base + mc, D, nt), nt, cos[off:],
                                sin[off:], q, k, v, ps, off)
            ops.attn_fwd_ex(q, k, v, per["ao"], per["lse"], B, Hh, Tp, Tp, 64, 64**-0.5, kb)
            for st, nt, off, mc, ps in streams:
                if st == "context" and c_out is None and bi == blocks[-1]:
                    continue
                a = per[st]
                ops.copy_rows3d(per["ao"][off:], Tp * D, D, a["a"], nt * D, D, B, nt, D)
                pend[st] = self._half2_fwd(a, block_names(pre, st), a["xin"], Modulation(mod, None, base + mc, D, nt))
        if x_out is None:
            return pend["input"]
        ops.gated_residual_fwd(*pend["input"], nx, x_out)
        if c_out is not None:
            ops.gated_residual_fwd(*pend["context"], Lc, c_out)
        return None

    def _jstage_bwd(self, blocks, dx_x: Tensor, dx_c: Tensor | None, nx: int, pos: Tensor | None, kb: Tensor, scr: dict, att: tuple,
                    dfe: dict, sw: "SideWork", pending: bool = False):
        d, w = self.d, self.ws
        B, Lc = self.geo[0], self._Lc
        D, Hh = d.inner_dim, d.num_heads
        cos, sin = self._tabs
        rot = sum(d.rope_axes_dim)
        mod, dmod = w["mod"], w["dmod32"]
        Tp = kb.shape[1]
        streams = (("input", nx, Lc, 0, pos), ("context", Lc, 0, 6 * D, None))
        dao, dq, dk, dv = att
        blocks = list(blocks)
        last = blocks[-1]
        dx: dict[str, Tensor | None] = {"input": dx_x, "context": dx_c}
        if not pending:
            if last in dfe:
                ops.add_bf16(dx_x, dfe[last], dx_x)
            for st, nt, off, mc, ps in streams:
                if dx[st] is None:
                    continue
                a, mo = w["blk"][last][st], self.layout.mod_off[last] + mc
                ops.gate_bwd(dx[st], a["t2"], mod[:, mo + 5 * D : mo + 6 * D], nt, a["wg"]["dt2"], dmod[:, mo + 5 * D : mo + 6 * D])
        skip_ctx_last = dx_c is None
        for j in reversed(range(len(blocks))):
            bi = blocks[j]
            per, pre = w["blk"][bi], self.prefixes[bi]
            ms = {st: Modulation(mod, dmod, self.layout.mod_off[bi] + mc, D, nt, part=per[st]["dwb"], groups=B) for st, nt, _, mc, _ in streams}
            dao.zero_()
            for st, nt, off, mc, ps in streams:
                if st == "context" and skip_ctx_last and bi == last:
                    continue
                a, s = per[st], scr[st]
                dx[st] = self._half2_bwd(a, a["wg"], block_names(pre, st), s, ms[st], dx[st], sw)
                ops.copy_rows3d(s["da"], nt * D, D, dao[off:], Tp * D, D, B, nt, D)
            ops.attn_bwd_ex(per["q"], per["k"], per["v"], per["ao"], dao, per["lse"], dq, dk, dv, B, Hh, Tp, Tp, 64, 64**-0.5, kb)
            for st, nt, off, mc, ps in streams:
                a, nm = per[st], block_names(pre, st)
                ops.qk_norm_rope_bwd(dq, dk, dv, a["qkv"], self.P(nm["qk"] + ".query_norm.scale"), self.P(nm["qk"] + ".key_norm.scale"),
                                     cos[off:], sin[off:], a["rrms"], a["wg"]["dqkv"], self.G(nm["qk"] + ".query_norm.scale"), B, nt, Hh,
                                     64, rot, pos=ps, n_off=off)
                prev = dres = None
                if j > 0:
                    bp = blocks[j - 1]
                    ap = w["blk"][bp][st]
                    prev = (ap["t2"], self.layout.mod_off[bp] + mc + 5 * D, ap["wg"]["dt2"])
                    dres = dfe.get(bp) if st == "input" else None
                dx[st] = self._half1_bwd(a, a["wg"], nm, scr[st], ms[st], a["xin"], dx[st], prev, dres, sw)
            self._end_block(sw, bi)
        return dx["input"], dx["context"]

    def feature(self, k: int) -> Tensor:
        assert self._train, "block outputs are only kept by the train-mode launch sequence"
        B, _, _, _, _, N, _, _, _ = self.geo
        return self.ws["x"][k + 1].view(B, N, self.d.inner_dim)

    def backward(self, dpred: Tensor, dfeats: dict[int, Tensor] | None = None, need_dx: bool = False,
                 input_only: bool = False) -> Tensor | None:
        assert self._train and self.grads is not None
        if input_only:
            self._input_only = True
            try:
                return self._backward_input_only(dpred, dfeats)
            finally:
                self._input_only = False
        dfeats = self._dfeat_rows(dfeats)
        d, w, sh = self.d, self.ws, self.sh
        B, _, _, gh, gw, N, M, _, _ = self.geo
        D, E, L = d.inner_dim, d.embedding_dim, d.depth
        cos, sin = self._rope[(gh, gw)]
        mod, dmod, xs = w["mod"], w["dmod32"], w["x"]
        dmod[:B].zero_()
        s = {k: w[k] for k in ("dxa", "dxb", "dxm", "da", "dh", "dq", "dk", "dv")}

        fused = self._row_gemms(M, N)
        self._head_bwd(dpred, None if fused else w["dxm"], scratch=w["det_scr"])
        mo, ml = L * 6 * D, (L - 1) * 6 * D
        dx = w["dxa"]
        if fused:
            _must(ops.ln_modulate_gemm_bwd(w["dO"], sh["last_layer.linear.weight|t"], xs[L], None, None, mod[:, mo : mo + D], N,
                                            w["meanf"], w["rstdf"], dfeats.get(L - 1), dx, dmod[:, mo : mo + D],
                                            dmod[:, mo + D : mo + 2 * D], None, gate_t=w["layers"][L - 1]["t2"],
                                            gate=mod[:, ml + 5 * D : ml + 6 * D], dt=w["wg"][L - 1]["dt2"],
                                            dgate=dmod[:, ml + 5 * D : ml + 6 * D], K=self._ko))
        else:
            Modulation(mod, dmod, mo, D, N).ln_bwd(w["dxm"], xs[L], None, None, 0, w["meanf"], w["rstdf"], dfeats.get(L - 1), dx, None,
                                                   gate=(w["layers"][L - 1]["t2"], ml + 5 * D, w["wg"][L - 1]["dt2"]))

        serial = tuning.on("DL_WGRAD_SERIAL")
        sw = SideWork(self, grouped_wgs=256, serial=serial, strict=True)
        main, side = sw.main, sw.side

        early_mod = self.reducer is not None and type(self) is DiTEngine and tuning.on("DL_DP_EARLY_MOD")
        self._early_mod_done = early_mod
        w_mod = self.layout.entries[self.mod_name][0]
        b_mod = self.layout.entries[self.layout.mod_b0][0]

        def early_mod_rows(r0: int, r1: int) -> None:
            ops.cast2d_f32_to_bf16(w["dmod32"][:B, r0:r1], w["dmod"][:B, r0:r1])
            ops.gemm_tn(w["dmod"][:, r0:r1], w["se"], self.grads[w_mod + r0 * E : w_mod + r1 * E].view(r1 - r0, E))
            ops.colsum(w["dmod"][:, r0:r1], self.grads[b_mod + r0 : b_mod + r1], B, r1 - r0)

        def block_done(i: int) -> None:
            if self.reducer is None:
                return
            if early_mod:
                sw.run(lambda: early_mod_rows(i * 6 * D, (i + 1) * 6 * D))
            ev_side = side.record_event()
            self.reducer.ready(*self.layer_ranges[i], extra_events=(ev_side,))
            if early_mod:
                self.reducer.ready(w_mod + i * 6 * D * E, w_mod + (i + 1) * 6 * D * E, flush=i < 3)

        native = self._native_blocks() and not serial
        inline_wgrad = tuning.on("DL_WGRAD_INLINE")
        defer_fold = fused and self.reducer is None
        for i in reversed(range(L)):
            dres = dfeats.get(i - 1)
            if native:
                blk = self._block_args(i, True)
                blk.set(dfeat=dres)
                ops.dit_block_bwd(blk, main.cuda_stream, main.cuda_stream if inline_wgrad else side.cuda_stream, sw.side_wgs)
            elif fused:
                dx = self._block_bwd_row_gemms(i, dx, dres, s, sw, not defer_fold)
            else:
                prev = (w["layers"][i - 1]["t2"], (i - 1) * 6 * D + 5 * D, w["wg"][i - 1]["dt2"]) if i > 0 else None
                m = Modulation(mod, dmod, i * 6 * D, D, N, part=(w["dwb"][2 * i], w["dwb"][2 * i + 1]), groups=B)
                dx = self._dit_block_bwd(w["layers"][i], w["wg"][i], f"layers.{i}.", xs[i], dx, prev, dres, s, m, N, cos, sin, sw,
                                         kb=w.get("kb"), dao=w.get("dao"))
            block_done(i)
        join_last = self.reducer is None and tuning.on("DL_JOIN_LAST")
        if not join_last:
            sw.join()
        if defer_fold:
            ent = self.layout.entries
            stride = ent[self.prefixes[1] + "norm_1.weight"][0] - ent[self.prefixes[0] + "norm_1.weight"][0] if L > 1 else 0
            for j, nm in enumerate(("norm_1.weight", "norm_2.weight")):
                ops.reduce_rows_batched_f32(w["dwb"][j], 2 * B * 2 * D, self.G(self.prefixes[0] + nm), stride, L, B, 2 * D)

        self._cond_bwd(dx)
        if join_last:
            sw.join()
        return self._input_grad(dx) if need_dx else None

    _input_only = False

    def _input_grad(self, dx: Tensor) -> Tensor:
        B, H, W = self.geo[0], self.geo[1], self.geo[2]
        dimg = torch.empty(B, self.d.input_channels, H, W, device=self.dev, dtype=torch.float32)
        return ops.patch_embed_dgrad(dx, self.P(self._conv_name), dimg, self.d.patch_size)

    def _qk_scale_sink(self, qk: str) -> Tensor:
        ent = self.layout.entries
        (q0, qs), (k0, ks) = ent[qk + ".query_norm.scale"], ent[qk + ".key_norm.scale"]
        n = k0 - q0 + math.prod(ks)
        sink = getattr(self, "_qk_sink", None)
        if sink is None or sink.numel() < n:
            sink = self._qk_sink = self._z(n, dtype=torch.float32)
        return sink[: math.prod(qs)]

    def _backward_input_only(self, dpred: Tensor, dfeats: dict[int, Tensor] | None) -> Tensor:
        dfeats = self._dfeat_rows(dfeats)
        d, w, sh = self.d, self.ws, self.sh
        B, _, _, gh, gw, N, M, _, _ = self.geo
        D, L = d.inner_dim, d.depth
        cos, sin = self._rope[(gh, gw)]
        mod, dmod, xs = w["mod"], w["dmod32"], w["x"]
        dmod[:B].zero_()
        s = {k: w[k] for k in ("dxa", "dxb", "dxm", "da", "dh", "dq", "dk", "dv")}
        fused = self._row_gemms(M, N)
        ops.patchify(dpred, w["dO"], d.patch_size, ops.PATCH_PPC)
        if not fused:
            ops.gemm_nt(w["dO"], sh["last_layer.linear.weight|t"], w["dxm"], M=M, N=D, K=self._ko)
        mo, ml = L * 6 * D, (L - 1) * 6 * D
        dx = w["dxa"]
        if fused:
            _must(ops.ln_modulate_gemm_bwd(w["dO"], sh["last_layer.linear.weight|t"], xs[L], None, None, mod[:, mo : mo + D], N,
                                            w["meanf"], w["rstdf"], dfeats.get(L - 1), dx, dmod[:, mo : mo + D],
                                            dmod[:, mo + D : mo + 2 * D], None, gate_t=w["layers"][L - 1]["t2"],
                                            gate=mod[:, ml + 5 * D : ml + 6 * D], dt=w["wg"][L - 1]["dt2"],
                                            dgate=dmod[:, ml + 5 * D : ml + 6 * D], K=self._ko))
        else:
            Modulation(mod, dmod, mo, D, N).ln_bwd(w["dxm"], xs[L], None, None, 0, w["meanf"], w["rstdf"], dfeats.get(L - 1), dx, None,
                                                   gate=(w["layers"][L - 1]["t2"], ml + 5 * D, w["wg"][L - 1]["dt2"]))
        sw = _NoSideWork()
        for i in reversed(range(L)):
            dres = dfeats.get(i - 1)
            if fused:
                dx = self._block_bwd_row_gemms(i, dx, dres, s, sw, False)
            else:
                prev = (w["layers"][i - 1]["t2"], (i - 1) * 6 * D + 5 * D, w["wg"][i - 1]["dt2"]) if i > 0 else None
                m = Modulation(mod, dmod, i * 6 * D, D, N, part=(None, None), groups=B)
                dx = self._dit_block_bwd(w["layers"][i], w["wg"][i], f"layers.{i}.", xs[i], dx, prev, dres, s, m, N, cos, sin, sw,
                                         kb=w.get("kb"), dao=w.get("dao"))
        return self._input_grad(dx)

    def _block_bwd_row_gemms(self, i: int, dx: Tensor, dres: Tensor | None, s: dict, sw: "SideWork", fold: bool) -> Tensor:
        d, w, sh = self.d, self.ws, self.sh
        _, _, _, gh, gw, N, _, _, _ = self.geo
        D = d.inner_dim
        mod, dmod = w["mod"], w["dmod32"]
        a, g, nm, mo = w["layers"][i], w["wg"][i], block_names(f"layers.{i}."), i * 6 * D
        sw.wgrad(g["dt2"], a["h"], nm["down"] + ".weight")
        ops.mlp_swiglu_bwd(g["dt2"], sh[nm["down"] + ".weight|t"], a["xm2"], sh[nm["up"] + ".weight|g"], a["u"], s["dh"], g["du"])
        sw.wgrad(g["du"], a["xm2"], nm["up"] + ".weight")
        nx = _other(s, dx)
        _must(ops.ln_modulate_gemm_bwd(g["du"], sh[nm["up"] + ".weight|t"], a["x1"], self.P(nm["n2"] + ".weight"),
                                        self.P(nm["n2"] + ".bias"), mod[:, mo + 3 * D : mo + 4 * D], N, a["mean2"], a["rstd2"], dx, nx,
                                        dmod[:, mo + 3 * D : mo + 4 * D], dmod[:, mo + 4 * D : mo + 5 * D], w["dwb"][2 * i + 1],
                                        gate_t=a["t1"], gate=mod[:, mo + 2 * D : mo + 3 * D], dt=g["dt1"],
                                        dgate=dmod[:, mo + 2 * D : mo + 3 * D]))
        if fold:
            sw.fold(w["dwb"][2 * i + 1], nm["n2"] + ".weight", self.geo[0])
        dx = nx
        sw.wgrad(g["dt1"], a["a"], nm["proj"] + ".weight")
        ops.gemm_nt(g["dt1"], sh[nm["proj"] + ".weight|t"], s["da"])
        self._attn_bwd(a, g, nm, s, N, *self._rope[(gh, gw)], None, None, None)
        sw.wgrad(g["dqkv"], a["xm1"], nm["qkv"] + ".weight")
        if dres is not None:
            ops.add_bf16(dx, dres, dx)
        nxt = {}
        if i > 0:
            mp = (i - 1) * 6 * D
            nxt = dict(gate_t=w["layers"][i - 1]["t2"], gate=mod[:, mp + 5 * D : mp + 6 * D], dt=w["wg"][i - 1]["dt2"],
                       dgate=dmod[:, mp + 5 * D : mp + 6 * D])
        nx = _other(s, dx)
        _must(ops.ln_modulate_gemm_bwd(g["dqkv"], sh[nm["qkv"] + ".weight|t"], w["x"][i], self.P(nm["n1"] + ".weight"),
                                        self.P(nm["n1"] + ".bias"), mod[:, mo : mo + D], N, a["mean1"], a["rstd1"], dx, nx,
                                        dmod[:, mo : mo + D], dmod[:, mo + D : mo + 2 * D], w["dwb"][2 * i], **nxt))
        if fold:
            sw.fold(w["dwb"][2 * i], nm["n1"] + ".weight", self.geo[0])
        return nx

    def _head_bwd(self, dpred: Tensor, dxm: Tensor | None, scratch: Tensor | None = None) -> None:
        d, w = self.d, self.ws
        M, Fo, D = self.geo[6], self.geo[8], d.inner_dim
        ops.patchify(dpred, w["dO"], d.patch_size, ops.PATCH_PPC)
        gl = self.G("last_layer.linear.weight")
        if Fo % 8 == 0:
            ops.gemm_tn(w["dO"], w["xf"], gl, M=Fo, N=D, scratch=scratch)
        else:
            w["scr_last"].zero_()
            ops.gemm_tn(w["dO"], w["xf"], w["scr_last"], M=_rup(Fo, 8), N=D, scratch=scratch)
            ops.reduce_rows_f32(w["scr_last"], gl, 1, Fo * D)
        ops.colsum(w["dO"], self.G("last_layer.linear.bias"), M, Fo, scratch=scratch)
        if dxm is not None:
            ops.gemm_nt(w["dO"], self.sh["last_layer.linear.weight|t"], dxm, M=M, N=D, K=self._ko)

    def _dfeat_rows(self, dfeats: dict[int, Tensor] | None) -> dict[int, Tensor]:
        return {k: g.reshape(-1, self.d.inner_dim).to(torch.bfloat16).contiguous() for k, g in (dfeats or {}).items()}

    def _patch_wgrad(self, dx: Tensor, name: str, scratch: Tensor | None) -> None:
        d, w = self.d, self.ws
        D, Fi = d.inner_dim, d.input_channels * d.patch_size**2
        gc = self.G(name).view(D, Fi)
        if Fi % 8 == 0:
            ops.gemm_tn(dx, w["tokP"], gc, M=D, N=Fi, scratch=scratch)
        else:
            w["scr_conv"].zero_()
            ops.gemm_tn(dx, w["tokP"], w["scr_conv"], M=D, N=_rup(Fi, 8), scratch=scratch)
            gc.add_(w["scr_conv"][:, :Fi])

    def _end_block(self, sw: "SideWork", bi: int) -> None:
        sw.flush()
        if self.reducer is not None:
            self.reducer.ready(*self.layer_ranges[bi], extra_events=(sw.side.record_event(),))

    def _cond_bwd(self, dx: Tensor, extra_demb: Tensor | None = None) -> None:
        d, w, sh = self.d, self.ws, self.sh
        B, _, _, _, _, _, M, _, _ = self.geo
        D, E = d.inner_dim, d.embedding_dim
        dmod = w["dmod32"]
        det = w.get("det_scr")
        self._patch_wgrad(dx, self._conv_name, det)

        R = self.layout.mod_rows
        g_modw = self.grads[self.layout.entries[self.mod_name][0] :][: R * E].view(R, E)
        g_modb = self.grads[self.layout.entries[self.layout.mod_b0][0] :][:R]
        L6 = len(self.prefixes) * 6 * D if getattr(self, "_early_mod_done", False) else 0
        if L6:
            ops.cast2d_f32_to_bf16(dmod[:B, L6:], w["dmod"][:B, L6:])
            dmod = w["dmod"]
            ops.gemm_tn(dmod[:, L6:], w["se"], g_modw[L6:], scratch=det)
            ops.colsum(dmod[:, L6:], g_modb[L6:], B, R - L6, scratch=det)
        else:
            ops.cast_f32_to_bf16(dmod[:B], w["dmod"][:B])
            dmod = w["dmod"]
            ops.gemm_tn(dmod, w["se"], g_modw, scratch=det)
            ops.colsum(dmod, g_modb, B, R, scratch=det)
        ops.gemm_nt(dmod, sh["@mod|t"], w["dse"], M=B, N=E, K=R, scratch=det)
        table = d.n_classes is not None
        if self._pooled_dim:
            ops.cond_combine_dense_bwd(w["dse"][:B], w["emb"][:B], w["demb"][:B], w["demb16"][:B])
            self._pooled_bwd(B, det)
        else:
            ops.cond_combine_bwd(w["dse"][:B], w["emb"][:B], self._yeff if table else None, w["demb"][:B], w["demb16"][:B],
                                 self.G("label_embed.embedding.weight") if table else None)
        if extra_demb is not None:
            w["demb"][:B].add_(extra_demb[:B])
            ops.cast_f32_to_bf16(w["demb"][:B], w["demb16"][:B])
        ops.colsum(w["demb"], self.G("time_embed.2.bias"), B, E, scratch=det)
        ops.gemm_tn(w["demb16"], w["h1"], self.G("time_embed.2.weight"), scratch=det)
        ops.gemm_nt(w["demb16"], sh["time_embed.2.weight|t"], w["dh1"], M=B, N=E, K=E)
        ops.silu_bwd(w["dh1"][:B], w["pre1"][:B], w["dpre1"][:B])
        ops.gemm_tn(w["dpre1"], w["temb"], self.G("time_embed.0.weight"), scratch=det)
        ops.colsum(w["dpre1"], self.G("time_embed.0.bias"), B, E, scratch=det)
        if self.reducer is not None:
            if L6:
                w_mod = self.layout.entries[self.mod_name][0]
                self.reducer.ready(0, w_mod)
                self.reducer.ready(w_mod + L6 * E, self.layer_ranges[0][0])
            else:
                self.reducer.ready(0, self.layer_ranges[0][0])
            self.reducer.finish()


class _StrictWgradGroups(ops.WgradGroups):

    def _issue(self, key: int) -> None:
        probs = self.pending.pop(key, [])
        if probs:
            self.launch(lambda: _must(ops.gemm_tn_group(probs, self.slab, max_wgs=self.max_wgs)))


class _NoSideWork:

    def wgrad(self, dy: Tensor, x: Tensor, name: str) -> None:
        pass

    def fold(self, partial: Tensor | None, name: str, groups: int) -> None:
        pass

    def flush(self) -> None:
        pass

    def join(self) -> None:
        pass


class SideWork:

    def __init__(self, eng: DiTEngine, grouped_wgs: int = 128, serial: bool = False, strict: bool = False) -> None:
        self.G, self.width = eng.G, 2 * eng.d.inner_dim
        self.main = torch.cuda.current_stream()
        self.side = eng._side_stream()
        self.side.wait_stream(self.main)
        slab = eng.ws.get("tn_slab")
        self.side_wgs = tuning.integer("DL_SIDE_WGS", grouped_wgs if slab is not None else 128)
        self.wgs, self.launch = (0, lambda fn: fn()) if serial else (self.side_wgs, self.run)
        groups = _StrictWgradGroups if strict else ops.WgradGroups
        self.groups = groups(slab, self.launch, max_wgs=self.wgs) if slab is not None else None

    def run(self, fn) -> None:
        ev = self.main.record_event()
        with torch.cuda.stream(self.side):
            self.side.wait_event(ev)
            fn()

    def wgrad(self, dy: Tensor, x: Tensor, name: str) -> None:
        if self.groups is not None:
            self.groups.add(dy, x, self.G(name))
        else:
            self.launch(lambda: ops.gemm_tn(dy, x, self.G(name), max_wgs=self.wgs))

    def flush(self) -> None:
        if self.groups is not None:
            self.groups.flush()

    def fold(self, partial: Tensor, name: str, groups: int) -> None:
        self.run(lambda: ops.reduce_rows_f32(partial, self.G(name), groups, self.width, clear=True))
# ... 4 lines not shown
```

diffulab_amd/ops.py:

```python

from __future__ import annotations

import ctypes
import math
import os

import numpy as np
import torch
from torch import Tensor

from ._lib import lib
from . import tuning

BF16, F32 = 0, 1
ACT_NONE, ACT_SILU, ACT_GELU = 0, 1, 2
LOSS_FLOW, LOSS_EPS = 0, 1
MEAN_TYPES = {"epsilon": 0, "xstart": 1, "xprev": 2, "v": 3}
VAR_MODES = {"learned": 0, "learned_range": 1}
VAR_FIXED = -1
PATCH_CPP, PATCH_PPC = 0, 1


_raw_stream = getattr(torch._C, "_cuda_getCurrentRawStream", None)

# ... 650 lines not shown
        def run() -> None:
            if not gemm_tn_group(probs, self.slab, max_wgs=self.max_wgs):
                for dy, x, g in probs:
                    gemm_tn(dy, x, g, max_wgs=self.max_wgs)

        self.launch(run)

    def flush(self) -> None:
        for key in list(self.pending):
            self._issue(key)


def ln_modulate_fwd(x, w, b, scale, shift, rows_per_mod, eps, out, mean, rstd, t=None, gate=None, x_out=None):
    M, D = x.shape
    _call("dl_ln_modulate_fwd", _p(x), _p(w), _p(b), _p(scale), _p(shift), scale.stride(0), rows_per_mod, float(eps),
          _p(out), _p(mean), _p(rstd), _p(t), _p(gate), gate.stride(0) if gate is not None else 0, _p(x_out), M, D, _s())


def ln_modulate_bwd(dout, x, w, b, scale, rows_per_mod, mean, rstd, dres, dx, dscale, dshift, dwb_partial, gate_t=None,
                    gate=None, dt=None, dgate=None):
    M, D = x.shape
    assert dscale.dtype == torch.float32 and dshift.dtype == torch.float32
    assert dgate is None or (dgate.dtype == torch.float32 and dgate.stride(0) == dscale.stride(0))
    _call("dl_ln_modulate_bwd", _p(dout), _p(x), _p(w), _p(b), _p(scale), scale.stride(0), rows_per_mod, _p(mean),
          _p(rstd), _p(dres), _p(dx), _p(dscale), _p(dshift), dscale.stride(0), _p(dwb_partial), _p(gate_t), _p(gate),
          gate.stride(0) if gate is not None else 0, _p(dt), _p(dgate), M, D, _s())


def row_gemm_ok(M: int, D: int, rows_per_mod: int) -> bool:
    return tuning.on("DL_ROW_GEMM") and D == 384 and rows_per_mod == 256 and M % 256 == 0 and M // 256 >= 8


def ln_modulate_gemm_fwd(a, w_sh, resid, gate, ln_w, ln_b, scale, shift, rows_per_mod, eps, t_out, x_out, xm_out, mean, rstd,
                         K=None) -> bool:
    M, D = xm_out.shape
    return _maybe("dl_ln_modulate_gemm_fwd", _p(a), a.stride(0), _p(w_sh), w_sh.stride(0), M, a.shape[1] if K is None else K, _p(resid),
                  _p(gate), gate.stride(0) if gate is not None else 0, _p(ln_w), _p(ln_b), _p(scale), _p(shift), scale.stride(0),
                  rows_per_mod, float(eps), _p(t_out), _p(x_out), _p(xm_out), _p(mean), _p(rstd), D, _s())


def ln_modulate_gemm_bwd(a, wt_sh, x, ln_w, ln_b, scale, rows_per_mod, mean, rstd, dres, dx, dscale, dshift, dwb_partial,
                         gate_t=None, gate=None, dt=None, dgate=None, K=None) -> bool:
    M, D = x.shape
    assert dscale.dtype == torch.float32 and dshift.dtype == torch.float32 and dshift.stride(0) == dscale.stride(0)
    assert dgate is None or (dgate.dtype == torch.float32 and dgate.stride(0) == dscale.stride(0))
    return _maybe("dl_ln_modulate_gemm_bwd", _p(a), a.stride(0), _p(wt_sh), wt_sh.stride(0), M, a.shape[1] if K is None else K, _p(x),
                  _p(ln_w), _p(ln_b), _p(scale), scale.stride(0), rows_per_mod, _p(mean), _p(rstd), _p(dres), _p(dx), _p(dscale),
                  _p(dshift), dscale.stride(0), _p(dwb_partial), _p(gate_t), _p(gate), gate.stride(0) if gate is not None else 0,
                  _p(dt), _p(dgate), D, _s())


def gemm_nt_qk_norm_rope(a, w_qkv, scale_q, scale_k, cos, sin, qkv, q, k, rrms, B, N, H, dh, rot, eps=1e-6, n_off=0) -> bool:
    return _maybe("dl_gemm_nt_qk_norm_rope", _p(a), a.stride(0), _p(w_qkv), w_qkv.stride(0), B, N, H, dh, rot, float(eps),
                  _p(scale_q), _p(scale_k), _p(cos), _p(sin), _p(qkv), _p(q), _p(k), _p(rrms), q.shape[2], n_off, _s())


def ln_modulate_bwd_tok(dout, x, w, b, scale, mean, rstd, dres, dx, dscale, dshift, dwb_partial, gate_t=None, gate=None, dt=None,
                        dgate=None):
    M, D = x.shape
    assert dscale.dtype == torch.bfloat16 and dshift.stride(0) == dscale.stride(0)
    _call("dl_ln_modulate_bwd_tok", _p(dout), _p(x), _p(w), _p(b), _p(scale), scale.stride(0), _p(mean), _p(rstd), _p(dres), _p(dx),
          _p(dscale), _p(dshift), dscale.stride(0), _p(dwb_partial), dwb_partial.shape[0] if dwb_partial is not None else 0,
          _p(gate_t), _p(gate), gate.stride(0) if gate is not None else 0, _p(dt), _p(dgate), M, D, _s())


def ddt_cond_fwd(enc, temb, B, N, out):
    _call("dl_ddt_cond_fwd", _p(enc), enc.stride(0), _p(temb), temb.stride(0), B, N, out.shape[1], _p(out), _s())


def ddt_cond_bwd(dsz, enc, temb, B, N, denc, dtemb):
    _call("dl_ddt_cond_bwd", _p(dsz), _p(enc), enc.stride(0), _p(temb), temb.stride(0), B, N, dsz.shape[1], _p(denc), _p(dtemb), _s())


def gate_bwd(dout, t, gate, rows_per_mod, dt, dgate):
    M, D = dout.shape
    _call("dl_gate_bwd", _p(dout), _p(t), _p(gate), gate.stride(0), rows_per_mod, _p(dt), _p(dgate), dgate.stride(0), M,
          D, _s())


def qk_norm_rope_fwd(qkv, scale_q, scale_k, cos, sin, q, k, v, rrms, B, N, H, dh, rot, eps=1e-6, pos=None, n_off=0):
    _call("dl_qk_norm_rope_fwd_ex", _p(qkv), _p(scale_q), _p(scale_k), _p(cos), _p(sin), _p(q), _p(k), _p(v), _p(rrms), B, N,
          H, dh, rot, float(eps), _p(pos), q.shape[2], n_off, _s())


def qk_norm_rope_bwd(dq, dk, dv, qkv, scale_q, scale_k, cos, sin, rrms, dqkv, dscale, B, N, H, dh, rot, pos=None, n_off=0):
    _call("dl_qk_norm_rope_bwd_ex", _p(dq), _p(dk), _p(dv), _p(qkv), _p(scale_q), _p(scale_k), _p(cos), _p(sin), _p(rrms),
          _p(dqkv), _p(dscale), B, N, H, dh, rot, _p(pos), dq.shape[2], n_off, _s())


def copy_rows3d(src, src_bs, src_rs, dst, dst_bs, dst_rs, B, rows, cols):
    _call("dl_copy_rows3d", _p(src), src_bs, src_rs, _p(dst), dst_bs, dst_rs, B, rows, cols, _s())


def gather_tokens(src, idx, dst, B, N, k, D, keep=None):
    _call("dl_gather_tokens", _p(src), src.stride(0), _p(idx), _p(keep), _p(dst), dst.stride(0), B, N, k, D, _s())


def scatter_tokens_add(src, idx, dst, B, N, k, D):
    _call("dl_scatter_tokens_add", _p(src), src.stride(0), _p(idx), _p(dst), dst.stride(0), B, N, k, D, _s())


def restore_tokens(xd, inv, mask, out, B, N, k, D):
    _call("dl_restore_tokens", _p(xd), xd.stride(0), _p(inv), _p(mask), _p(out), out.stride(0), B, N, k, D, _s())


def masked_colsum(x, sel, out, R, C):
    _call("dl_masked_colsum", _p(x), x.stride(0), _p(sel), _p(out), R, C, _s())


def gated_residual_fwd(x, t, gate, rows_per_mod, out):
    M, D = x.shape
    _call("dl_gated_residual_fwd", _p(x), _p(t), _p(gate), gate.stride(0), rows_per_mod, _p(out), out.stride(0), M, D, _s())


def attn_fwd(q, k, v, out, lse, B, H, N, dh, scale):
    _call("dl_attn_fwd", _p(q), _p(k), _p(v), _p(out), _p(lse), B, H, N, dh, float(scale), _s())


def attn_bwd(q, k, v, out, dout, lse, dq, dk, dv, B, H, N, dh, scale):
    _call("dl_attn_bwd", _p(q), _p(k), _p(v), _p(out), _p(dout), _p(lse), _p(dq), _p(dk), _p(dv), B, H, N, dh,
          float(scale), _s())


ATTN_MAX_TOKENS = 32768
_INT32_ELEMS = 2 ** 31


def check_row_extent(rows: int, width: int, what: str) -> None:
    if rows * width >= _INT32_ELEMS:
        raise NotImplementedError(f"{what}: {rows} token rows x {width} columns = {rows * width} elements exceed the 2^31 elements the "
                                  "bf16 regime's kernels index; use a smaller batch")


def attn_needs_padding(N: int) -> bool:
    return N % 64 != 0 or (N > 256 and N % 256 != 0)


def v_in_place(N: int) -> bool:
    return N <= 256 and N % 64 == 0 and tuning.on("DL_ATTN_V_IN_PLACE")


def dit_block_fwd(blk, train: bool) -> None:
    _call("dl_dit_block_fwd", ctypes.addressof(blk), int(train), _s())


def dit_block_fwd_chain(blk, train: bool) -> bool:
    return _maybe("dl_dit_block_fwd_chain", ctypes.addressof(blk), int(train), _s())


def dit_block_bwd(blk, main_stream: int, side_stream: int, side_wgs: int) -> None:
    _call("dl_dit_block_bwd", ctypes.addressof(blk), main_stream, side_stream, int(side_wgs))


def attn_fwd_qkv(q, k, qkv, out, lse, B, H, N, dh, scale):
    D = H * dh
    _call("dl_attn_fwd_sv", _p(q), _p(k), qkv.data_ptr() + 2 * D * 2, N * 3 * D, dh, 3 * D, _p(out), _p(lse), B, H, N, dh,
          float(scale), _s())


def gemm_nt_ssq(a, w_sh, out, ssq, stationary: bool = False, max_workgroups: int = 0) -> bool:
    args = (_p(a), a.stride(0), _p(w_sh), w_sh.stride(0), _p(out), out.stride(0), a.shape[0], w_sh.shape[0], a.shape[1], _p(ssq), ssq.shape[1])
    if stationary and _maybe("dl_gemm_nt_ssq_stationary", *args, int(max_workgroups), _s()):
        return True
    return _maybe("dl_gemm_nt_ssq", *args, _s())


def attn_fwd_qkn(qkv, ssq, scale_q, scale_k, cos, sin, q, k, rrms, out, lse, B, H, N, dh, rot, scale, eps=1e-6):
    _call("dl_attn_fwd_qkn", _p(qkv), _p(ssq), _p(scale_q), _p(scale_k), _p(cos), _p(sin), float(eps), rot, _p(q), _p(k), _p(rrms), _p(out),
          _p(lse), B, H, N, dh, float(scale), _s())


def attn_bwd_qkv(q, k, qkv, out, dout, lse, dq, dk, dqkv, B, H, N, dh, scale):
    D = H * dh
    _call("dl_attn_bwd_sv", _p(q), _p(k), qkv.data_ptr() + 2 * D * 2, N * 3 * D, dh, 3 * D, _p(out), _p(dout), _p(lse), _p(dq),
          _p(dk), dqkv.data_ptr() + 2 * D * 2, N * 3 * D, dh, 3 * D, B, H, N, dh, float(scale), _s())


def attn_bwd_tok(q, k, qkv, out, dout, lse, dqkv, B, H, N, dh, scale):
    _call("dl_attn_bwd_tok", _p(q), _p(k), _p(qkv), _p(out), _p(dout), _p(lse), _p(dqkv), B, H, N, dh, float(scale), _s())


def qk_inplace_ok(ws: dict, B: int, tokens: int) -> bool:
    return ws.get("qk_part") is not None and v_in_place(tokens) and B * tokens >= 32768


def qk_norm_rope_bwd_inplace(qkv, scale_q, scale_k, cos, sin, rrms, dqkv, dscale, partials, B, N, H, dh, rot, pos=None) -> bool:
    assert partials.numel() >= 1024 * 2 * H * dh and partials.dtype == torch.float32
    return _maybe("dl_qk_norm_rope_bwd_inplace", _p(qkv), _p(scale_q), _p(scale_k), _p(cos), _p(sin), _p(rrms), _p(dqkv), _p(dscale),
                  _p(partials), B, N, H, dh, rot, _p(pos), _s())


def attn_fwd_ex(q, k, v, out, lse, B, H, Nq, Nk, dh, scale, key_bias=None):
    _call("dl_attn_fwd_ex", _p(q), _p(k), _p(v), _p(out), _p(lse), B, H, Nq, Nk, dh, float(scale), _p(key_bias), _s())


def attn_bwd_ex(q, k, v, out, dout, lse, dq, dk, dv, B, H, Nq, Nk, dh, scale, key_bias=None):
    _call("dl_attn_bwd_ex", _p(q), _p(k), _p(v), _p(out), _p(dout), _p(lse), _p(dq), _p(dk), _p(dv), B, H, Nq, Nk, dh,
          float(scale), _p(key_bias), _s())


def swiglu_fwd(u, h):
    _call("dl_swiglu_fwd", _p(u), _p(h), u.shape[0], h.shape[1], _s())


def swiglu_bwd(dh, u, du):
    _call("dl_swiglu_bwd", _p(dh), _p(u), _p(du), u.shape[0], dh.shape[1], _s())


def patchify(x, tok, p, order):
    B, C, H, W = x.shape
    _call("dl_patchify", _p(x), _p(tok), B, C, H, W, p, tok.stride(0), order, _s())


def unpatchify(tok, img, p):
    B, C, H, W = img.shape
    _call("dl_unpatchify", _p(tok), _p(img), B, C, H, W, p, tok.stride(0), _s())


def patch_embed_dgrad(dtok, w, dimg, p):
    B, C, H, W = dimg.shape
    D = w.shape[0]
    assert w.dtype == torch.float32 and w.is_contiguous() and w.numel() == D * C * p * p and dimg.dtype == torch.float32
    assert dimg.is_contiguous() and dtok.stride(1) == 1 and dtok.shape[1] >= D and dtok.dtype in (torch.bfloat16, torch.float32)
    assert dtok.shape[0] >= B * (H // p) * (W // p)
    _call("dl_patch_embed_dgrad", _p(dtok), BF16 if dtok.dtype == torch.bfloat16 else F32, dtok.stride(0), _p(w), _p(dimg), B, C, H, W,
          p, D, _s())
    return dimg


def timestep_embedding(t, out, max_period=10000.0):
    _call("dl_timestep_embedding", _p(t), _p(out), out.shape[0], out.shape[1], float(max_period), _s())


def cond_combine_fwd(e, table, idx, emb, act):
    _call("dl_cond_combine_fwd", _p(e), _p(table), _p(idx), _p(emb), _p(act), e.shape[0], e.shape[1], _s())


def cond_combine_bwd(dact, emb, idx, demb, demb16, dtable):
    _call("dl_cond_combine_bwd", _p(dact), _p(emb), _p(idx), _p(demb), _p(demb16), _p(dtable), emb.shape[0], emb.shape[1],
          _s())


def cond_combine_dense_fwd(e, pe, emb, act):
    _call("dl_cond_combine_dense_fwd", _p(e), _p(pe), _p(emb), _p(act), e.shape[0], e.shape[1], _s())


def cond_combine_dense_bwd(dact, emb, demb, demb16):
    _call("dl_cond_combine_dense_bwd", _p(dact), _p(emb), _p(demb), _p(demb16), emb.shape[0], emb.shape[1], _s())


def silu_bwd(dy, pre, dx):
    _call("dl_silu_bwd", _p(dy), _p(pre), _p(dx), dy.numel(), _s())


def gelu_bwd(dy, pre, dx):
    _call("dl_gelu_bwd", _p(dy), _p(pre), _p(dx), dy.numel(), _s())


def heads_split_rope(src, dst, B, H, n_src, n_off, cos=None, sin=None, rot=0):
    _call("dl_heads_split_rope", _p(src), src.stride(0), _p(dst), B, H, n_src, dst.shape[2], n_off, _p(cos), _p(sin), rot, _s())


def heads_merge_rope_bwd(dst_grad, src_grad, B, H, n_src, n_off, cos=None, sin=None, rot=0, accumulate=False):
    _call("dl_heads_merge_rope_bwd", _p(dst_grad), _p(src_grad), src_grad.stride(0), B, H, n_src, dst_grad.shape[2], n_off,
          _p(cos), _p(sin), rot, int(accumulate), _s())


def colsum(x, out, R=None, C=None, scratch=None):
    R = x.shape[0] if R is None else R
    C = x.shape[1] if C is None else C
    if scratch is not None:
        _call("dl_colsum_det", _p(x), F32 if x.dtype == torch.float32 else BF16, x.stride(0), _p(out), R, C, _p(scratch), scratch.numel(),
              _s())
        return
    _call("dl_colsum", _p(x), F32 if x.dtype == torch.float32 else BF16, x.stride(0), _p(out), R, C, _s())


class _ColsumDesc(ctypes.Structure):
    _fields_ = [("x", ctypes.c_void_p), ("ld", ctypes.c_int64), ("out", ctypes.c_void_p), ("R", ctypes.c_int64), ("C", ctypes.c_int64)]


def colsum_batched(items: list) -> None:
    arr = (_ColsumDesc * len(items))()
    for i, (x, out, R, C) in enumerate(items):
        assert x.dtype == torch.bfloat16 and out.dtype == torch.float32
        arr[i] = _ColsumDesc(_p(x), x.stride(0), _p(out), R, C)
    _call("dl_colsum_batched", ctypes.cast(arr, ctypes.c_void_p), len(items), _s())


def reduce_rows_f32(partial, out, G, n, clear=False):
    _call("dl_reduce_rows_f32", _p(partial), _p(out), G, n, int(clear), _s())


def reduce_rows_batched_f32(partial, partial_stride, out, out_stride, K, G, n):
    _call("dl_reduce_rows_batched_f32", _p(partial), partial_stride, _p(out), out_stride, K, G, n, _s())


def cosine_rows_fwd(p, d, cosv, pn2, dn2, eps=1e-8):
    M, E = p.shape
    _call("dl_cosine_rows_fwd", _p(p), p.stride(0), _p(d), d.stride(0), _p(cosv), _p(pn2), _p(dn2), M, E, float(eps), _s())


def cosine_rows_bwd(p, d, cosv, pn2, dn2, gscale, gscale_dev, dp, eps=1e-8):
    M, E = p.shape
    _call("dl_cosine_rows_bwd", _p(p), p.stride(0), _p(d), d.stride(0), _p(cosv), _p(pn2), _p(dn2), float(gscale),
          _p(gscale_dev), _p(dp), dp.stride(0), M, E, float(eps), _s())


def adamw_step(p, g, m, v, lr, beta1, beta2, eps, wd, step, grad_scale=1.0):
    _call("dl_adamw_step", _p(p), _p(g), _p(m), _p(v), p.numel(), float(lr), float(beta1), float(beta2), float(eps),
          float(wd), float(1.0 - beta1**step), float(1.0 - beta2**step), float(grad_scale), _s())


def adamw_step_dev(p, g, m, v, hyper):
    _call("dl_adamw_step_dev", _p(p), _p(g), _p(m), _p(v), p.numel(), _p(hyper), _s())


def grad_sumsq_chain(n: int) -> int:
    return int(lib().call("dl_grad_sumsq_chain", int(n)))


def grad_sumsq_slots(n: int) -> int:
    return int(lib().call("dl_grad_sumsq_slots", int(n)))


def grad_sumsq(x, partials, slot=0) -> int:
    if x.dtype != torch.float32 or not x.is_contiguous() or partials.dtype != torch.float32 or not partials.is_contiguous():
        raise RuntimeError("grad_sumsq needs contiguous f32 tensors")
    global _LIB
    if _LIB is None:
        _LIB = lib()
    args = (_p(x), x.numel(), _p(partials), int(slot), partials.numel(), _s())
    k = _LIB.call("dl_grad_sumsq", *args)
    if k <= 0:
        raise RuntimeError(f"dl_grad_sumsq failed ({k}): {_LIB.cdll.dl_last_error().decode()}")
    if _REC is not None:
        _REC.calls.append((_negative_is_failure(_LIB._fns["dl_grad_sumsq"][0]), args))
    return k


def _negative_is_failure(fn):
    return lambda *a: fn(*a) < 0
# ... 760 lines not shown
```

diffulab_amd/tuning.py:

```python

from __future__ import annotations

import os

SWITCHES: dict[str, tuple[str, str]] = {
    "DL_NATIVE_BLOCK": ("1", "DiT blocks issued by the C ABI's block drivers (dl_dit_block_fwd / _bwd) instead of one Python call per kernel"),
    "DL_ROW_GEMM": ("1", "LayerNorm-modulate forward / backward as epilogues of the row-complete 256x384 GEMMs (D = 384, 256 tokens per sample)"),
    "DL_ROW_GEMM_QK": ("0", "QK-norm + RoPE as the epilogue of the qkv GEMM (measured slower than the separate row kernel)"),
    "DL_QKN_ON_LOAD": ("1", "QK-RMSNorm statistics leave with the qkv GEMM (dl_gemm_nt_ssq) and norm + RoPE are applied as the attention "
                       "forward stages q and k (dl_attn_fwd_qkn): no qk_norm_rope_fwd pass (row-complete path, <= 256 tokens)"),
    "DL_BLOCK_CHAIN": ("1", "block forward of the row-complete path as one per-sample chain launch (dl_dit_block_fwd_chain; native block "
                       "driver, 256 tokens per sample, QK-norm on load)"),
    "DL_MLP_RECOMPUTE": ("1", "SwiGLU backward recomputes the MLP-up pre-activations instead of storing them in the forward"),
    "DL_ATTN_V_IN_PLACE": ("1", "attention reads V / writes dV inside the token-major qkv rows (N <= 256)"),
    "DL_QK_INPLACE": ("1", "attention backward writes dQ / dK token-major and the QK-norm backward runs in place on the dqkv rows"),
    "DL_WGRAD_GROUP": ("1", "the four weight gradients of a block as one atomics-free launch (dl_gemm_tn_group)"),
    "DL_WGRAD_INLINE": ("0", "grouped weight gradients on the main stream instead of the side stream"),
    "DL_WGRAD_SERIAL": ("0", "per-problem weight gradients on the main stream (engines without the grouped form)"),
    "DL_SIDE_WGS": ("", "workgroup cap of the side-stream weight gradients (default: 256 grouped, 128 per-problem)"),
    "DL_SIDE_CU_MASK": ("", "CU mask of the side stream (dl_stream_create_masked): 'i4' = every 4th CU, 'b128' = the first 128"),
    "DL_SIDE_LOW_PRIORITY": ("0", "DiT engines: the side stream of the weight gradients is created with the device's lowest stream priority "
                             "(measured +-0: DiT-S/2 20.83 / 20.80 vs 20.73 / 20.77 ms; SPRINT joint 28.77 / 28.58 vs 28.79 / 28.62; DDT 38.93 / 38.97 vs "
                             "39.01 / 39.00; joint MMDiT 49.14 / 49.13 vs 49.24 / 49.31; REPA 11.71 / 11.68 vs 11.76 / 11.73)"),
    "DL_UNET_SIDE_LOW_PRIORITY": ("1", "UNet: the same (the dispatcher serves the main chain's workgroups first: 26.42 / 26.50 vs 26.66 / 26.64 ms)"),
    "DL_JOIN_LAST": ("1", "single GPU: the side stream is joined after the conditioning backward instead of before it"),
    "DL_DP_RESERVE_CUS": ("0", "data parallel: CUs left to the communication library's workgroups (persistent main-chain grids shrink by it; "
                          "measured a loss at the headline shape, whose tile counts are whole multiples of 256: DESIGN.md section 5)"),
    "DL_MAIN_WGS": ("", "workgroup budget of the persistent main-chain kernels (experiments; default: all CUs, or CUs - reserve with a reducer)"),
    "DL_DP_EARLY_MOD": ("1", "data parallel: each block's adaLN rows are reduced as the block finishes"),
    "DL_HIPGRAPH": ("1", "samplers replay the denoiser forward as a captured hipGraph"),
    "DL_CFG_PAIR": ("1", "guided sampler steps run the conditional and the label-dropped forward as ONE forward over [x ; x] "
                    "(class-conditional MMDiT / DDT / UNetModel: same values per row, the weights stream once)"),
    "DL_LAUNCH_PLAN": ("0", "UNet (bf16 regime): a training forward / backward is recorded on its second run for a shape and re-issued as a "
                       "flat list of C calls afterwards (ops.LaunchPlan: the engine's Python costs the host ~24 us per launch, 716 "
                       "launches per step).  Measured (profiles/r06_e_*): the step at B = 64 is NOT host-bound -- its main queue is busy "
                       "19.2 of 20.3 ms and `host_issue` is the full launch queue pushing back -- so the plan changes nothing there "
                       "(20.03 vs 20.11 ms); it pays where the host is the slower side (under a profiler's per-launch overhead: 20.3 vs "
                       "22.7 ms), hence opt-in"),
    "DL_UNET_SIDE": ("1", "UNet weight gradients on a side stream"),
    "DL_UNET_NT_PAIR": ("1", "UNet AttentionBlock: the q and kv projections (and their data gradients) as one launch of the 128 x 128 GEMM "
                        "kernel where both are small (dl_gemm_nt_pair: 64 + 128 tiles on 256 CUs at the 4 x 4 level); bit-identical"),
    "DL_UNET_XATTN_HIP": ("1", "UNet TransformerBlock (context conditioning): the cross-attention core as dl_attn_cross_* (bf16 operands, f32 "
                          "softmax; MFMA with the keys streamed in 64-key tiles where dh % 64 == 0, VALU otherwise) where Nq <= 64, L <= 512, "
                          "dh % 8 == 0; 0 = the f32 copies + batched dl_f32_gemm + masked softmax fallback"),
    "DL_UNET_SPLITK": ("1", "split-K convolutions at the UNet's low-resolution levels (partial images + fixed-order fold: -7 % per step)"),
    "DL_UNET_WGRAD_WGS": ("128", "workgroup cap of the UNet's side-stream convolution weight gradients (0 = one per CU).  Round 6, with the "
                          "tap-reusing kernel and partial images (every workgroup stores its 295 KB of accumulators once, so the cap also "
                          "halves the stage bytes), B = 128: 0 -> 25.4 ms/step, 160 -> 24.1, 128 -> 23.9, 96 -> 24.4, 64 -> 25.0, 48 -> 26.8; "
                          "B = 64: 0 -> 19.0, 128 -> 18.0 (profiles/r06_q_*).  Round 5 (implicit-GEMM kernels, atomics): 0 was best"),
    "DL_UNET_FOLD_BATCHED": ("1", "UNet convolution weight gradients stay in a persistent transposed staging arena during the backward; one "
                             "launch at its end folds all of them into the [Co, Ci, 3, 3] gradients (instead of a zero-fill and a fold per convolution)"),
    "DL_UNET_WGRAD_PARTS": ("1", "UNet convolution weight gradients as partial images per pixel range (plain stores + fixed-order fold in the "
                            "batched fold launch: bit-reproducible) instead of f32 atomics into one image.  With the tap-reusing kernel of "
                            "round 6 (conv_wgrad.hip) the atomics were 56 % of a launch (1.45 TB/s of read-modify-writes against 6 TB/s of "
                            "stores) and the fold takes one tap of a channel tile per workgroup when eight or more images wait: B = 128 "
                            "24.7 -> 23.9 ms/step, B = 64 19.0 -> 18.0 (same workgroup cap).  With the implicit-GEMM kernels alone it was "
                            "slower (28.5 vs 26.8 ms: session e)"),
    "DL_UNET_DET_COLSUM": ("0", "UNet bias gradients through the bit-reproducible column sum (measured 2 % slower)"),
}


def text(name: str) -> str:
    return os.environ.get(name, SWITCHES[name][0])


def on(name: str) -> bool:
    return text(name) not in ("", "0")


def integer(name: str, default: int) -> int:
    v = text(name)
    return int(v) if v else default
```

include/diffulab_hip.h:

```cpp
#ifndef DIFFULAB_HIP_H
#define DIFFULAB_HIP_H

#include <stdint.h>

#ifdef __cplusplus
extern "C" {
#endif

#define DL_API __attribute__((visibility("default")))

typedef void* dl_stream_t;

enum { DL_OK = 0, DL_ERR_INVALID = -1, DL_ERR_LAUNCH = -2, DL_ERR_UNSUPPORTED = -3 };
enum { DL_BF16 = 0, DL_F32 = 1 };
enum { DL_ACT_NONE = 0, DL_ACT_SILU = 1, DL_ACT_GELU = 2 };
enum { DL_LOSS_FLOW = 0, DL_LOSS_EPS = 1 };
enum { DL_MEAN_EPSILON = 0, DL_MEAN_XSTART = 1, DL_MEAN_XPREV = 2, DL_MEAN_V = 3 };
enum { DL_VAR_LEARNED = 0, DL_VAR_LEARNED_RANGE = 1 };
enum { DL_VAR_FIXED = -1 };
enum { DL_PATCH_CPP = 0, DL_PATCH_PPC = 1 };

DL_API int dl_version(void);
DL_API const char* dl_last_error(void);
DL_API int dl_device_info(int device, int* cu_count, int* lds_bytes_per_cu, int64_t* hbm_bytes, char* arch,
// ... 67 lines not shown
                        int64_t batch, int64_t chw, dl_stream_t stream);
DL_API int dl_ddpm_step_lv(const float* pred, const float* pred_uncond, float guidance, const float* xt,
                           const float* noise, const int32_t* t, const float* tables, int32_t T, int mean_type,
                           int var_mode, int clamp_x, float* x_prev, float* x0_est, float* mean, float* std,
                           float* logprob, int64_t batch, int64_t chw, dl_stream_t stream);
DL_API int dl_ddim_step(const float* pred, const float* pred_uncond, float guidance, const float* xt,
                        const float* noise, const int32_t* t, const float* tables, int32_t T, int mean_type,
                        const float* ddpm_coefs ,
                        int clamp_x, float eta, float* x_prev, float* x0_est, float* mean, float* std,
                        float* logprob, int64_t batch, int64_t chw, dl_stream_t stream);
DL_API int dl_ddim_step_lv(const float* pred, const float* pred_uncond, float guidance, const float* xt,
                           const float* noise, const int32_t* t, const float* tables, int32_t T, int mean_type,
                           const float* ddpm_coefs, int clamp_x, float eta, float* x_prev, float* x0_est, float* mean,
                           float* std, float* logprob, int64_t batch, int64_t chw, dl_stream_t stream);
DL_API int dl_ddpm_step_v(const float* pred, const float* pred_uncond, float guidance, const float* xt, const float* noise,
                          const int32_t* t, const float* tables, int32_t T, int var_mode, int clamp_x, float* x_prev,
                          float* x0_est, float* mean, float* std, float* logprob, int64_t batch, int64_t chw,
                          dl_stream_t stream);
DL_API int dl_ddim_step_v(const float* pred, const float* pred_uncond, float guidance, const float* xt, const float* noise,
                          const int32_t* t, const float* tables, int32_t T, int var_mode, int clamp_x, float eta, float* x_prev,
                          float* x0_est, float* mean, float* std, float* logprob, int64_t batch, int64_t chw,
                          dl_stream_t stream);
DL_API int dl_cfg_rescale_coef(const float* pred, const float* pred_uncond, float guidance, float phi, float* r, int64_t batch,
                               int64_t chw, int64_t sample_stride, dl_stream_t stream);
DL_API int dl_abs_quantile_rows(const float* x, int64_t k, float f, float* q, float* lohi, int64_t batch, int64_t n,
                                dl_stream_t stream);
DL_API int dl_x0_threshold(const float* pred, const float* pred_uncond, float guidance, const float* cfg_mul, const float* xt,
                           const int32_t* t, const float* tables, int32_t T, int mean_type, const float* coefs, int64_t k, float f,
                           float threshold_max, float* s, float* lohi, int64_t batch, int64_t chw, int64_t sample_stride,
                           dl_stream_t stream);
DL_API int dl_euler_step_g(const float* x, const float* v, const float* v_uncond, float guidance, const float* cfg_mul,
                           float t_curr, float dt, float* x_prev, float* x0_est, int64_t batch, int64_t chw, dl_stream_t stream);
DL_API int dl_euler_maruyama_step_g(const float* x, const float* v, const float* v_uncond, float guidance, const float* cfg_mul,
                                    const float* noise, const float* x_prev_in, float t_curr, float dt, float sigma, float std,
                                    float* x_prev, float* mean, float* x0_est, float* logprob, int64_t batch, int64_t chw,
                                    dl_stream_t stream);
DL_API int dl_ddpm_step_g(const float* pred, const float* pred_uncond, float guidance, const float* cfg_mul, const float* x0_thr,
                          const float* xt, const float* noise, const int32_t* t, const float* tables, int32_t T, int mean_type,
                          int var_mode, int clamp_x, float* x_prev, float* x0_est, float* mean, float* std, float* logprob,
                          int64_t batch, int64_t chw, dl_stream_t stream);
DL_API int dl_ddim_step_g(const float* pred, const float* pred_uncond, float guidance, const float* cfg_mul, const float* x0_thr,
                          const float* xt, const float* noise, const int32_t* t, const float* tables, int32_t T, int mean_type,
                          int var_mode, const float* ddpm_coefs, int clamp_x, float eta, float* x_prev, float* x0_est, float* mean,
                          float* std, float* logprob, int64_t batch, int64_t chw, dl_stream_t stream);
DL_API int dl_ab2_step(const float* x, const float* v, const float* v_uncond, float guidance, const float* cfg_mul,
                       const float* v_last, float t_curr, float dt, float w, float* x_prev, float* x0_est, float* v_out,
                       int64_t batch, int64_t chw, dl_stream_t stream);
DL_API int dl_dpmpp_2m_step(const float* pred, const float* pred_uncond, float guidance, const float* cfg_mul, const float* x0_thr,
                            const float* xt, const float* x0_last, const int32_t* t, const float* tables, int32_t T, int mean_type,
                            int var_mode, int clamp_x, float a, float b, float c, float* x_prev, float* x0_est, int64_t batch,
                            int64_t chw, dl_stream_t stream);
DL_API int dl_inpaint_blend(const float* x, const float* ref, const float* noise, const float* mask, float a, float b,
                            float* out, int64_t batch, int64_t channels, int64_t hw, int64_t mask_channels,
                            dl_stream_t stream);

DL_API int dl_gemm_nt(const void* A, int64_t lda, const void* B, int64_t ldb, void* C, int64_t ldc, int64_t M,
                      int64_t N, int64_t K, const float* bias, int act, int out_dtype, void* pre_out,
                      const void* resid, int64_t ldr, const void* gate, int64_t ldg, int64_t rows_per_gate,
                      dl_stream_t stream);
typedef struct dl_nt_problem_t {
  const void* A;
  int64_t lda;
  const void* B;
  int64_t ldb;
  void* C;
  int64_t ldc;
  int64_t M, N, K;
  const float* bias;
  const void* resid;
  int64_t ldr;
} dl_nt_problem_t;
DL_API int dl_gemm_nt_pair(const dl_nt_problem_t* problems, int n, dl_stream_t stream);
DL_API int dl_gemm_nt_swiglu(const void* X, int64_t ldx, const void* Wp, int64_t ldw, void* U, int64_t ldu, void* H,
                             int64_t ldh, int64_t M, int64_t F, int64_t K, dl_stream_t stream);
DL_API int dl_gemm_nt_swiglu_stationary(const void* X, int64_t ldx, const void* Wp, int64_t ldw, void* U, int64_t ldu, void* H,
                                        int64_t ldh, int64_t M, int64_t F, int64_t K, int max_workgroups, dl_stream_t stream);
DL_API int dl_mlp_dswiglu_recompute(const void* X, int64_t ldx, const void* Wp, int64_t ldwp, const void* dT, int64_t ldt,
                                    const void* W2t, int64_t ldw2, void* dU, int64_t lddu, int64_t M, int64_t F, int64_t K1,
                                    int64_t K2, dl_stream_t stream);
DL_API int dl_gemm_tn(const void* A, int64_t lda, const void* B, int64_t ldb, float* C, int64_t ldc, int64_t M,
                      int64_t N, int64_t R, dl_stream_t stream);
DL_API int dl_gemm_tn_ex(const void* A, int64_t lda, const void* B, int64_t ldb, float* C, int64_t ldc, int64_t M,
                         int64_t N, int64_t R, int max_workgroups, dl_stream_t stream);
typedef struct dl_wgrad_t {
  const void* dy;
  int64_t ld_dy;
  const void* x;
  int64_t ld_x;
  float* g;
  int64_t m_out, n_in;
} dl_wgrad_t;
DL_API int dl_gemm_tn_group(const dl_wgrad_t* probs, int n_probs, int64_t R, float* slab, int64_t slab_floats, int max_workgroups,
                            dl_stream_t stream);
DL_API int dl_gemm_tn_det(const void* A, int64_t lda, const void* B, int64_t ldb, float* C, int64_t ldc, int64_t M, int64_t N,
                          int64_t R, float* scratch, int64_t scratch_floats, dl_stream_t stream);
DL_API int dl_gemm_nt_f32_det(const void* A, int64_t lda, const void* B, int64_t ldb, float* C, int64_t ldc, int64_t M, int64_t N,
                              int64_t K, float* scratch, int64_t scratch_floats, dl_stream_t stream);
DL_API int dl_colsum_det(const void* x, int dtype, int64_t ld, float* out, int64_t R, int64_t C, float* scratch,
                         int64_t scratch_floats, dl_stream_t stream);

DL_API int dl_ln_modulate_fwd(const void* x, const float* w, const float* b, const void* scale, const void* shift,
                              int64_t ld_mod, int64_t rows_per_mod, float eps, void* out, float* mean,
                              float* rstd, const void* t, const void* gate, int64_t ld_gate, void* x_out, int64_t M,
                              int64_t D, dl_stream_t stream);
DL_API int dl_ln_modulate_bwd(const void* dout, const void* x, const float* w, const float* b, const void* scale,
                              int64_t ld_mod, int64_t rows_per_mod, const float* mean, const float* rstd,
                              const void* dres, void* dx, float* dscale, float* dshift, int64_t ld_dmod,
                              float* dwb_partial, const void* gate_t, const void* gate, int64_t ld_gate, void* dt,
                              float* dgate, int64_t M, int64_t D, dl_stream_t stream);
DL_API int dl_ln_modulate_bwd_tok(const void* dout, const void* x, const float* w, const float* b, const void* scale,
                                  int64_t ld_mod, const float* mean, const float* rstd, const void* dres, void* dx, void* dscale,
                                  void* dshift, int64_t ld_dmod, float* dwb_partial, int64_t n_part, const void* gate_t,
                                  const void* gate, int64_t ld_gate, void* dt, void* dgate, int64_t M, int64_t D,
                                  dl_stream_t stream);
DL_API int dl_ln_modulate_gemm_fwd(const void* A, int64_t lda, const void* W, int64_t ldw, int64_t M, int64_t K, const void* resid,
                                   const void* gate, int64_t ld_gate, const float* ln_w, const float* ln_b, const void* scale,
                                   const void* shift, int64_t ld_mod, int64_t rows_per_mod, float eps, void* t_out, void* x_out,
                                   void* xm_out, float* mean, float* rstd, int64_t D, dl_stream_t stream);
DL_API int dl_ln_modulate_gemm_bwd(const void* A, int64_t lda, const void* Wt, int64_t ldw, int64_t M, int64_t K, const void* x,
                                   const float* ln_w, const float* ln_b, const void* scale, int64_t ld_mod, int64_t rows_per_mod,
                                   const float* mean, const float* rstd, const void* dres, void* dx, float* dscale, float* dshift,
                                   int64_t ld_dmod, float* dwb_partial, const void* gate_t, const void* gate, int64_t ld_gate,
                                   void* dt, float* dgate, int64_t D, dl_stream_t stream);
DL_API int dl_gemm_nt_qk_norm_rope(const void* A, int64_t lda, const void* Wqkv, int64_t ldw, int64_t B, int64_t N, int64_t H,
                                   int64_t dh, int64_t rot, float eps, const float* scale_q, const float* scale_k, const float* cos,
                                   const float* sin, void* qkv, void* q, void* k, float* rrms, int64_t n_dst, int64_t n_off,
                                   dl_stream_t stream);
DL_API int dl_ddt_cond_fwd(const void* enc, int64_t ld, const float* temb, int64_t ld_t, int64_t B, int64_t N, int64_t D, void* out,
                           dl_stream_t stream);
DL_API int dl_ddt_cond_bwd(const void* dsz, const void* enc, int64_t ld, const float* temb, int64_t ld_t, int64_t B, int64_t N,
                           int64_t D, void* denc, float* dtemb, dl_stream_t stream);
DL_API int dl_gate_bwd(const void* dout, const void* t, const void* gate, int64_t ld_mod, int64_t rows_per_mod,
                       void* dt, float* dgate, int64_t ld_dmod, int64_t M, int64_t D, dl_stream_t stream);
DL_API int dl_qk_norm_rope_fwd(const void* qkv, const float* scale_q, const float* scale_k, const float* cos,
                               const float* sin, void* q, void* k, void* v, float* rrms, int64_t B, int64_t N,
                               int64_t H, int64_t dh, int64_t rot, float eps, dl_stream_t stream);
DL_API int dl_qk_norm_rope_bwd(const void* dq, const void* dk, const void* dv, const void* qkv,
                               const float* scale_q, const float* scale_k, const float* cos, const float* sin,
                               const float* rrms, void* dqkv, float* dscale, int64_t B, int64_t N, int64_t H,
                               int64_t dh, int64_t rot, dl_stream_t stream);
DL_API int dl_qk_norm_rope_fwd_ex(const void* qkv, const float* scale_q, const float* scale_k, const float* cos,
                                  const float* sin, void* q, void* k, void* v, float* rrms, int64_t B, int64_t N,
                                  int64_t H, int64_t dh, int64_t rot, float eps, const int32_t* pos, int64_t n_dst,
                                  int64_t n_off, dl_stream_t stream);
DL_API int dl_qk_norm_rope_bwd_ex(const void* dq, const void* dk, const void* dv, const void* qkv,
                                  const float* scale_q, const float* scale_k, const float* cos, const float* sin,
                                  const float* rrms, void* dqkv, float* dscale, int64_t B, int64_t N, int64_t H,
                                  int64_t dh, int64_t rot, const int32_t* pos, int64_t n_dst, int64_t n_off,
                                  dl_stream_t stream);
DL_API int dl_qk_norm_rope_bwd_inplace(const void* qkv, const float* scale_q, const float* scale_k, const float* cos,
                                       const float* sin, const float* rrms, void* dqkv, float* dscale, float* dscale_partials,
                                       int64_t B, int64_t N, int64_t H, int64_t dh, int64_t rot, const int32_t* pos,
                                       dl_stream_t stream);
DL_API int dl_attn_fwd(const void* q, const void* k, const void* v, void* out, float* lse, int64_t B, int64_t H,
                       int64_t N, int64_t dh, float scale, dl_stream_t stream);
DL_API int dl_attn_bwd(const void* q, const void* k, const void* v, const void* out, const void* dout,
                       const float* lse, void* dq, void* dk, void* dv, int64_t B, int64_t H, int64_t N,
                       int64_t dh, float scale, dl_stream_t stream);
DL_API int dl_attn_fwd_ex(const void* q, const void* k, const void* v, void* out, float* lse, int64_t B, int64_t H,
                          int64_t Nq, int64_t Nk, int64_t dh, float scale, const float* key_bias, dl_stream_t stream);
DL_API int dl_attn_bwd_ex(const void* q, const void* k, const void* v, const void* out, const void* dout,
                          const float* lse, void* dq, void* dk, void* dv, int64_t B, int64_t H, int64_t Nq, int64_t Nk,
                          int64_t dh, float scale, const float* key_bias, dl_stream_t stream);
DL_API int dl_attn_fwd_sv(const void* q, const void* k, const void* v, int64_t v_batch_stride, int64_t v_head_stride,
                          int64_t v_pitch, void* out, float* lse, int64_t B, int64_t H, int64_t N, int64_t dh, float scale,
                          dl_stream_t stream);
DL_API int dl_attn_bwd_sv(const void* q, const void* k, const void* v, int64_t v_batch_stride, int64_t v_head_stride,
                          int64_t v_pitch, const void* out, const void* dout, const float* lse, void* dq, void* dk, void* dv,
                          int64_t dv_batch_stride, int64_t dv_head_stride, int64_t dv_pitch, int64_t B, int64_t H, int64_t N,
                          int64_t dh, float scale, dl_stream_t stream);
DL_API int dl_attn_bwd_tok(const void* q, const void* k, const void* qkv, const void* out, const void* dout, const float* lse,
                           void* dqkv, int64_t B, int64_t H, int64_t N, int64_t dh, float scale, dl_stream_t stream);
DL_API int dl_gemm_nt_ssq(const void* A, int64_t lda, const void* B, int64_t ldb, void* C, int64_t ldc, int64_t M, int64_t N,
                          int64_t K, float* ssq, int64_t ssq_tiles, dl_stream_t stream);
DL_API int dl_gemm_nt_ssq_stationary(const void* A, int64_t lda, const void* B, int64_t ldb, void* C, int64_t ldc, int64_t M, int64_t N,
                                     int64_t K, float* ssq, int64_t ssq_tiles, int max_workgroups, dl_stream_t stream);
DL_API int dl_attn_fwd_qkn(const void* qkv, const float* ssq, const float* scale_q, const float* scale_k, const float* cos,
                           const float* sin, float eps, int64_t rot, void* q_out, void* k_out, float* rrms, void* out, float* lse,
                           int64_t B, int64_t H, int64_t N, int64_t dh, float scale, dl_stream_t stream);
DL_API int dl_swiglu_fwd(const void* u, void* h, int64_t M, int64_t F, dl_stream_t stream);
DL_API int dl_swiglu_bwd(const void* dh, const void* u, void* du, int64_t M, int64_t F, dl_stream_t stream);

DL_API int dl_patchify(const float* x, void* tok, int64_t B, int64_t C, int64_t H, int64_t W, int64_t p,
                       int64_t ld, int order, dl_stream_t stream);
DL_API int dl_unpatchify(const float* tok, float* img, int64_t B, int64_t C, int64_t H, int64_t W, int64_t p,
                         int64_t ld, dl_stream_t stream);
DL_API int dl_patch_embed_dgrad(const void* dtok, int dtype, int64_t ld, const float* w, float* dimg, int64_t B, int64_t C,
                                int64_t H, int64_t W, int64_t p, int64_t D, dl_stream_t stream);
DL_API int dl_timestep_embedding(const float* t, void* out, int64_t B, int64_t dim, float max_period,
                                 dl_stream_t stream);
DL_API int dl_cond_combine_fwd(const float* e, const float* table, const int64_t* idx, float* emb, void* act,
                               int64_t B, int64_t E, dl_stream_t stream);
DL_API int dl_cond_combine_bwd(const float* dact, const float* emb, const int64_t* idx, float* demb,
                               void* demb_bf16, float* dtable, int64_t B, int64_t E, dl_stream_t stream);
DL_API int dl_cond_combine_dense_fwd(const float* e, const float* pe, float* emb, void* act, int64_t B, int64_t E,
                                     dl_stream_t stream);
DL_API int dl_cond_combine_dense_bwd(const float* dact, const float* emb, float* demb, void* demb_bf16, int64_t B, int64_t E,
                                     dl_stream_t stream);
DL_API int dl_silu_bwd(const float* dy, const void* pre, void* dx, int64_t n, dl_stream_t stream);
DL_API int dl_gelu_bwd(const float* dy, const void* pre, void* dx, int64_t n, dl_stream_t stream);
DL_API int dl_heads_split_rope(const void* src, int64_t ld, void* dst, int64_t B, int64_t H, int64_t n_src, int64_t n_dst,
                               int64_t n_off, const float* cos, const float* sin, int64_t rot, dl_stream_t stream);
DL_API int dl_heads_merge_rope_bwd(const void* dst_grad, void* src_grad, int64_t ld, int64_t B, int64_t H, int64_t n_src,
                                   int64_t n_dst, int64_t n_off, const float* cos, const float* sin, int64_t rot,
                                   int accumulate, dl_stream_t stream);
DL_API int dl_colsum(const void* x, int dtype, int64_t ld, float* out, int64_t R, int64_t C,
                     dl_stream_t stream);
typedef struct dl_colsum_desc_t {
  const void* x;
  int64_t ld;
  float* out;
  int64_t R, C;
} dl_colsum_desc_t;
DL_API int dl_colsum_batched(const dl_colsum_desc_t* desc, int n, dl_stream_t stream);
DL_API int dl_reduce_rows_f32(float* partial, float* out, int64_t G, int64_t n, int clear_partial, dl_stream_t stream);
DL_API int dl_reduce_rows_batched_f32(const float* partial, int64_t partial_stride, float* out, int64_t out_stride, int64_t K,
                                      int64_t G, int64_t n, dl_stream_t stream);

DL_API int dl_cosine_rows_fwd(const void* p, int64_t ldp, const float* d, int64_t ldd, float* cosv, float* pn2, float* dn2,
                              int64_t M, int64_t E, float eps, dl_stream_t stream);
DL_API int dl_cosine_rows_bwd(const void* p, int64_t ldp, const float* d, int64_t ldd, const float* cosv, const float* pn2,
                              const float* dn2, float gscale, const float* gscale_dev, void* dp, int64_t lddp, int64_t M,
                              int64_t E, float eps, dl_stream_t stream);

DL_API int dl_gather_tokens(const void* src, int64_t ld_src, const int32_t* idx, const int32_t* keep, void* dst,
                            int64_t ld_dst, int64_t B, int64_t N, int64_t k, int64_t D, dl_stream_t stream);
DL_API int dl_scatter_tokens_add(const void* src, int64_t ld_src, const int32_t* idx, void* dst, int64_t ld_dst, int64_t B,
                                 int64_t N, int64_t k, int64_t D, dl_stream_t stream);
DL_API int dl_restore_tokens(const void* xd, int64_t ld_xd, const int32_t* inv, const float* mask, void* out, int64_t ld_out,
                             int64_t B, int64_t N, int64_t k, int64_t D, dl_stream_t stream);
DL_API int dl_masked_colsum(const void* x, int64_t ld, const int32_t* sel, float* out, int64_t R, int64_t C,
                            dl_stream_t stream);
DL_API int dl_copy_rows3d(const void* src, int64_t src_bs, int64_t src_rs, void* dst, int64_t dst_bs, int64_t dst_rs, int64_t B,
                          int64_t rows, int64_t cols, dl_stream_t stream);
DL_API int dl_gated_residual_fwd(const void* x, const void* t, const void* gate, int64_t ld_gate, int64_t rows_per_mod,
                                 void* out, int64_t ld_out, int64_t M, int64_t D, dl_stream_t stream);

DL_API int dl_adamw_step(float* p, const float* g, float* m, float* v, int64_t n, float lr, float beta1,
                         float beta2, float eps, float weight_decay, float bias_corr1, float bias_corr2,
                         float grad_scale, dl_stream_t stream);
DL_API int dl_adamw_step_dev(float* p, const float* g, float* m, float* v, int64_t n, const float* hyper, dl_stream_t stream);
DL_API int64_t dl_grad_sumsq_slots(int64_t n);
DL_API int64_t dl_grad_sumsq_chain(int64_t n);
DL_API int dl_grad_sumsq(const float* x, int64_t n, float* partials, int64_t slot, int64_t capacity, dl_stream_t stream);
DL_API int dl_clip_coef(const float* partials, int64_t n_slots, float grad_scale, const float* hyper, float max_norm, float* out,
                        dl_stream_t stream);
DL_API int dl_adamw_step_clip(float* p, const float* g, float* m, float* v, int64_t n, float lr, float beta1, float beta2,
                              float eps, float weight_decay, float bias_corr1, float bias_corr2, float grad_scale,
                              const float* coef, dl_stream_t stream);
DL_API int dl_adamw_step_dev_clip(float* p, const float* g, float* m, float* v, int64_t n, const float* hyper, const float* coef,
                                  dl_stream_t stream);
DL_API int dl_scale_inplace(float* g, int64_t n, const float* coef, dl_stream_t stream);
enum { DL_SGD_NESTEROV = 1, DL_SGD_FIRST = 2, DL_SGD_MAXIMIZE = 4 };
DL_API int dl_sgd_step(float* p, const float* g, float* buf, int64_t n, float lr, float momentum, float dampening,
                       float weight_decay, float grad_scale, const float* coef, int flags, dl_stream_t stream);
DL_API int dl_sgd_step_dev(float* p, const float* g, float* buf, int64_t n, const float* hyper, const float* coef, int flags,
                           dl_stream_t stream);
enum { DL_MUON_MAT_FIELDS = 10, DL_MUON_CHUNK_FIELDS = 3, DL_MUON_CHUNK = 2048 };
DL_API int dl_muon_pre(float* p, const float* g, float* m, float* v, int64_t n, const int64_t* chunks_host,
                       const int64_t* chunks_dev, int64_t n_chunks, const int64_t* mats_host, const int64_t* mats_dev,
                       int64_t n_mat, void* xws, int64_t x_cap, float* partials, int64_t partials_cap, float lr, float beta1,
                       float beta2, float eps, float weight_decay, float bias_corr1, float bias_corr2, float momentum,
                       float grad_scale, const float* coef, int nesterov, dl_stream_t stream);
DL_API int dl_muon_orthogonalize(const int64_t* mats_host, const int64_t* mats_dev, int64_t n_mat, const float* partials,
                                 float* norms, void* xws, int64_t x_cap, void* aws, int64_t a_cap, float eps, float a, float b,
                                 float c, int ns_steps, dl_stream_t stream);
DL_API int dl_muon_post(float* p, int64_t n, const int64_t* mats_host, const int64_t* mats_dev, int64_t n_mat, const void* xo,
                        int64_t x_cap, float lr, float weight_decay, dl_stream_t stream);
DL_API int dl_cast_weight(const float* src, int64_t R, int64_t C, void* dst, int64_t ld_dst, void* dstT,
                          int64_t ld_t, dl_stream_t stream);
DL_API int dl_cast_weight_swiglu(const float* src, int64_t F, int64_t C, void* dst, int64_t ld_dst, dl_stream_t stream);
typedef struct {
  const void* src;
  int64_t R, C;
  void* dst;
  int64_t ld_dst;
  void* dst_t;
  int64_t ld_t;
  void* dst_swiglu;
  int64_t ld_swiglu;
  int64_t tile_begin, tiles_c;
} dl_cast_desc_t;
DL_API int dl_cast_weights_batched(const dl_cast_desc_t* desc_dev, int n_desc, int64_t total_tiles, dl_stream_t stream);
DL_API int dl_cast_f32_to_bf16(const float* src, void* dst, int64_t n, dl_stream_t stream);
DL_API int dl_cast_bf16_to_f32(const void* src, float* dst, int64_t n, dl_stream_t stream);
DL_API int dl_cast2d_f32_to_bf16(const float* src, int64_t ld_src, void* dst, int64_t ld_dst, int64_t rows, int64_t cols,
                                 dl_stream_t stream);

DL_API int dl_ema_update(float* ema, const float* p, float beta, int64_t n, dl_stream_t stream);
enum { DL_LINCOMB_ACCUMULATE = 1 };
DL_API int dl_ema_update_multi(float* ema0, float* ema1, float* ema2, float* ema3, const float* p, int K, float w0, float w1, float w2,
                               float w3, int64_t n, dl_stream_t stream);
DL_API int dl_arena_lincomb(float* out, const int64_t* srcs_host, const int64_t* srcs_dev, const float* w_host, const float* w_dev,
                            int K, int64_t n, int flags, dl_stream_t stream);

DL_API int dl_nchw_to_nhwc(const float* x, void* out, int64_t B, int64_t C, int64_t HW, int64_t ld, dl_stream_t stream);
DL_API int dl_nhwc_to_nchw(const void* x, float* out, int64_t B, int64_t C, int64_t HW, int64_t ld, dl_stream_t stream);
DL_API int dl_gn_stats(const void* x, float* stats, int64_t B, int64_t HW, int64_t C, int64_t G, float eps,
                       dl_stream_t stream);
DL_API int dl_gn_apply_fwd(const void* x, const float* stats, const float* w, const float* b, const void* film_scale,
                           const void* film_shift, int64_t ld_film, int act_silu, void* out, int64_t B, int64_t HW,
                           int64_t C, int64_t G, dl_stream_t stream);
DL_API int dl_gn_fwd(const void* x, const float* w, const float* b, const void* film_scale, const void* film_shift, int64_t ld_film,
                     int act_silu, void* out, float* stats, int64_t B, int64_t HW, int64_t C, int64_t G, float eps, dl_stream_t stream);
#define DL_GN_BWD_MAX_RANGES 8
DL_API int dl_gn_bwd(const void* dout, const void* x, const float* stats, const float* w, const float* b,
// ... 50 lines not shown
DL_API int dl_rowbias_bwd(const void* dy, void* de, int64_t lde, int64_t B, int64_t HW, int64_t C, dl_stream_t stream);
DL_API int dl_attn_small_fwd(const void* q, const void* k, const void* v, int64_t ldq, int64_t ldkv, void* out,
                             int64_t ldo, float* probs, int64_t B, int64_t n, int64_t H, int64_t dh, float scale,
                             dl_stream_t stream);
DL_API int dl_attn_small_bwd(const void* q, const void* k, const void* v, int64_t ldq, int64_t ldkv, const void* dout,
                             int64_t ldo, const float* probs, void* dq, void* dk, void* dv, int64_t B, int64_t n,
                             int64_t H, int64_t dh, float scale, dl_stream_t stream);
DL_API int dl_attn_cross_fwd(const void* q, const void* k, const void* v, int64_t ldq, int64_t ldkv, const float* key_bias,
                             void* out, int64_t ldo, float* probs, int64_t B, int64_t Nq, int64_t L, int64_t H, int64_t dh,
                             float scale, dl_stream_t stream);
DL_API int dl_attn_cross_bwd(const void* q, const void* k, const void* v, int64_t ldq, int64_t ldkv, const float* key_bias,
                             const void* dout, int64_t ldo, const float* probs, float* ds, void* dq, void* dk, void* dv,
                             int64_t B, int64_t Nq, int64_t L, int64_t H, int64_t dh, float scale, dl_stream_t stream);
DL_API int dl_geglu_fwd(const void* u, int64_t ldu, void* h, int64_t ldh, int64_t M, int64_t F, dl_stream_t stream);
DL_API int dl_geglu_bwd(const void* dh, int64_t ldd, const void* u, int64_t ldu, void* du, int64_t lddu, int64_t M, int64_t F,
                        dl_stream_t stream);
DL_API int dl_add_bf16(const void* a, const void* b, void* out, int64_t n, dl_stream_t stream);
DL_API int dl_copy2d_bf16(const void* src, int64_t lds, void* dst, int64_t ldd, int64_t rows, int64_t cols,
                          dl_stream_t stream);
DL_API int dl_dropout(const void* x, int64_t ldx, const void* resid, int64_t ldr, void* out, int64_t ldo, int64_t rows, int64_t cols,
                      int dtype, const uint64_t* rng_state, int32_t site, int32_t T, float scale, dl_stream_t stream);

typedef struct dl_f32_gemm_t {
  const float* A;
  const float* B;
  float* C;
  int64_t lda, ldb, ldc;
  int64_t M, N, K;
  int32_t trans_a, trans_b;
  int64_t batch1, batch2;
  int64_t stride_a1, stride_a2, stride_b1, stride_b2, stride_c1, stride_c2;
  float alpha;
  const float* bias;
  int32_t act;
  float* pre_out;
  int32_t accumulate;
  float* scratch;
  int64_t scratch_floats;
} dl_f32_gemm_t;
DL_API int dl_f32_gemm(const dl_f32_gemm_t* desc, dl_stream_t stream);
DL_API int dl_f32_ln_modulate_fwd(const float* x, const float* w, const float* b, const float* scale, const float* shift,
                                  int64_t ld_mod, int64_t rows_per_mod, float eps, float* out, float* mean, float* rstd,
                                  const float* t, const float* gate, int64_t ld_gate, float* x_out, int64_t M, int64_t D,
                                  dl_stream_t stream);
DL_API int dl_f32_ln_modulate_bwd(const float* dout, const float* x, const float* w, const float* b, const float* scale,
                                  int64_t ld_mod, int64_t rows_per_mod, const float* mean, const float* rstd, const float* dres,
                                  float* dx, float* dscale, float* dshift, int64_t ld_dmod, float* dwb_partial, const float* gate_t,
                                  const float* gate, int64_t ld_gate, float* dt, float* dgate, int64_t M, int64_t D,
                                  dl_stream_t stream);
DL_API int dl_f32_qk_norm_rope_fwd(const float* qkv, int64_t ld, const float* scale_q, const float* scale_k, const float* cos,
                                   const float* sin, float* qk, float* rrms, int64_t B, int64_t N, int64_t H, int64_t dh,
                                   int64_t rot, float eps, const int32_t* pos, dl_stream_t stream);
DL_API int dl_f32_qk_norm_rope_bwd(const float* dqk, const float* qkv, int64_t ld, const float* scale_q, const float* scale_k,
                                   const float* cos, const float* sin, const float* rrms, float* dqkv, int64_t ld_d,
                                   float* dscale_partials, int64_t B, int64_t N, int64_t H, int64_t dh, int64_t rot,
                                   const int32_t* pos, dl_stream_t stream);
DL_API int dl_f32_scatter_tokens_add(const float* src, int64_t ld_src, const int32_t* idx, float* dst, int64_t ld_dst, int64_t B,
                                     int64_t N, int64_t k, int64_t D, dl_stream_t stream);
DL_API int dl_f32_restore_tokens(const float* xd, int64_t ld_xd, const int32_t* inv, const float* mask, float* out, int64_t ld_out,
                                 int64_t B, int64_t N, int64_t k, int64_t D, dl_stream_t stream);
DL_API int dl_f32_masked_colsum_partials(const float* x, int64_t ld, const int32_t* sel, float* partials, int64_t slabs, int64_t R,
                                         int64_t C, dl_stream_t stream);
DL_API int dl_f32_gated_residual_fwd(const float* x, const float* t, const float* gate, int64_t ld_gate, int64_t rows_per_mod,
                                     float* out, int64_t ld_out, int64_t M, int64_t D, dl_stream_t stream);
DL_API int dl_f32_gate_bwd(const float* dout, const float* t, const float* gate, int64_t ld_gate, int64_t rows_per_mod, float* dt,
                           float* dgate, int64_t ld_dgate, int64_t M, int64_t D, dl_stream_t stream);
DL_API int dl_f32_ddt_cond_fwd(const float* enc, int64_t ld, const float* temb, int64_t ld_t, int64_t B, int64_t N, int64_t D, float* out,
                               dl_stream_t stream);
DL_API int dl_f32_ddt_cond_bwd(const float* dsz, const float* enc, int64_t ld, const float* temb, int64_t ld_t, int64_t B, int64_t N,
                               int64_t D, float* denc, float* dtemb, dl_stream_t stream);
DL_API int dl_f32_softmax_fwd(float* s, int64_t rows, int64_t cols, dl_stream_t stream);
DL_API int dl_f32_softmax_bwd(const float* p, float* dp, int64_t rows, int64_t cols, dl_stream_t stream);
DL_API int dl_f32_softmax_keymask_fwd(float* s, const float* key_bias, int64_t B, int64_t rows_per_sample, int64_t cols,
                                      dl_stream_t stream);
DL_API int dl_f32_geglu_fwd(const float* u, float* h, int64_t M, int64_t F, dl_stream_t stream);
DL_API int dl_f32_geglu_bwd(const float* dh, const float* u, float* du, int64_t M, int64_t F, dl_stream_t stream);
DL_API int dl_f32_swiglu_fwd(const float* u, float* h, int64_t M, int64_t F, dl_stream_t stream);
DL_API int dl_f32_swiglu_bwd(const float* dh, const float* u, float* du, int64_t M, int64_t F, dl_stream_t stream);
DL_API int dl_f32_add(const float* a, const float* b, float* out, int64_t n, dl_stream_t stream);
DL_API int dl_f32_silu_bwd(const float* dy, const float* pre, float* dx, int64_t n, dl_stream_t stream);
DL_API int dl_f32_patchify(const float* x, float* tok, int64_t B, int64_t C, int64_t H, int64_t W, int64_t p, int64_t ld, int order,
                           dl_stream_t stream);
DL_API int dl_f32_timestep_embedding(const float* t, float* out, int64_t B, int64_t dim, float max_period, dl_stream_t stream);
DL_API int dl_f32_cond_combine_fwd(const float* e, const float* table, const int64_t* idx, float* emb, float* act, int64_t B,
                                   int64_t E, dl_stream_t stream);
DL_API int dl_f32_cond_combine_bwd(const float* dact, const float* emb, const int64_t* idx, float* demb, float* dtable, int64_t B,
                                   int64_t E, dl_stream_t stream);

DL_API int dl_f32_im2col3x3(const float* x, int64_t ldx, float* cols, int64_t B, int64_t H, int64_t W, int64_t C, dl_stream_t stream);
DL_API int dl_f32_col2im3x3(const float* dcols, float* dx, int64_t ld_dx, int64_t B, int64_t H, int64_t W, int64_t C,
                            dl_stream_t stream);
DL_API int dl_f32_gn_stats(const float* x, float* stats, int64_t B, int64_t HW, int64_t C, int64_t G, float eps, dl_stream_t stream);
DL_API int dl_f32_gn_apply_fwd(const float* x, const float* stats, const float* w, const float* b, const float* film_scale,
                               const float* film_shift, int64_t ld_film, int act_silu, float* out, int64_t B, int64_t HW, int64_t C,
                               int64_t G, dl_stream_t stream);
DL_API int dl_f32_gn_bwd(const float* dout, const float* x, const float* stats, const float* w, const float* b,
                         const float* film_scale, const float* film_shift, int64_t ld_film, int act_silu, const float* dres, float* dx,
                         float* dw_partial, float* db_partial, float* dfilm_scale, float* dfilm_shift, int64_t B, int64_t HW, int64_t C,
                         int64_t G, dl_stream_t stream);
DL_API int dl_f32_resample2x2(const float* x, float* out, int64_t B, int64_t Hs, int64_t Ws, int64_t C, float scale, int mode,
                              dl_stream_t stream);
DL_API int dl_f32_nchw_to_nhwc(const float* x, float* out, int64_t B, int64_t C, int64_t HW, int64_t ld, dl_stream_t stream);
DL_API int dl_f32_nhwc_to_nchw(const float* x, float* out, int64_t B, int64_t C, int64_t HW, int64_t ld, dl_stream_t stream);
DL_API int dl_f32_copy2d(const float* src, int64_t ld_src, float* dst, int64_t ld_dst, int64_t rows, int64_t cols, dl_stream_t stream);
DL_API int dl_f32_rowbias_add(const float* x, const float* e, int64_t lde, float* out, int64_t B, int64_t HW, int64_t C,
                              dl_stream_t stream);
DL_API int dl_f32_rowbias_bwd(const float* dy, float* de, int64_t lde, int64_t B, int64_t HW, int64_t C, dl_stream_t stream);

enum {
  DL_BLK_X_IN = 0,
  DL_BLK_PEND_X,
  DL_BLK_PEND_T,
  DL_BLK_PEND_GATE,
  DL_BLK_SCALE1, DL_BLK_SHIFT1, DL_BLK_GATE1, DL_BLK_SCALE2, DL_BLK_SHIFT2, DL_BLK_GATE2,
  DL_BLK_LN1_W, DL_BLK_LN1_B, DL_BLK_LN2_W, DL_BLK_LN2_B, DL_BLK_QN_SCALE, DL_BLK_KN_SCALE,
  DL_BLK_W_QKV, DL_BLK_W_PROJ, DL_BLK_W_UP, DL_BLK_W_UP_PERM, DL_BLK_W_DOWN,
  DL_BLK_WT_QKV, DL_BLK_WT_PROJ, DL_BLK_WT_UP, DL_BLK_WT_DOWN,
  DL_BLK_ROPE_COS, DL_BLK_ROPE_SIN,
  DL_BLK_XM1, DL_BLK_MEAN1, DL_BLK_RSTD1, DL_BLK_QKV, DL_BLK_Q, DL_BLK_K, DL_BLK_V , DL_BLK_RRMS,
  DL_BLK_A, DL_BLK_LSE, DL_BLK_T1, DL_BLK_X1, DL_BLK_XM2, DL_BLK_MEAN2, DL_BLK_RSTD2, DL_BLK_U, DL_BLK_H, DL_BLK_T2,
  DL_BLK_DT2,
  DL_BLK_DX_IN,
  DL_BLK_DX_MID,
  DL_BLK_DX_OUT,
  DL_BLK_DH, DL_BLK_DU, DL_BLK_DXM, DL_BLK_DT1, DL_BLK_DA, DL_BLK_DQ, DL_BLK_DK, DL_BLK_DV, DL_BLK_DQKV, DL_BLK_DFEAT ,
  DL_BLK_DSCALE1, DL_BLK_DSHIFT1, DL_BLK_DGATE1, DL_BLK_DSCALE2, DL_BLK_DSHIFT2,
  DL_BLK_DWB1, DL_BLK_DWB2,
  DL_BLK_PREV_T2, DL_BLK_PREV_GATE2, DL_BLK_PREV_DT2, DL_BLK_PREV_DGATE2,
  DL_BLK_G_QKV, DL_BLK_G_PROJ, DL_BLK_G_UP, DL_BLK_G_DOWN, DL_BLK_G_LN1, DL_BLK_G_LN2, DL_BLK_G_QK_SCALE,
  DL_BLK_NEXT_LN_W, DL_BLK_NEXT_LN_B, DL_BLK_NEXT_SCALE, DL_BLK_NEXT_SHIFT,
  DL_BLK_NEXT_X,
  DL_BLK_NEXT_XM, DL_BLK_NEXT_MEAN, DL_BLK_NEXT_RSTD,
  DL_BLK_TN_SLAB,
  DL_BLK_QK_PARTIALS,
  DL_BLK_SSQ,
  DL_BLK_NPTR
};
typedef struct dl_dit_block_t {
  void* p[96];
  int64_t B, N, D, H, F;
  int64_t ld_mod, ld_dmod;
  int64_t ldw_d, ldw_f;
  int64_t ldwt_d, ldwt_f2, ldwt_3d;
  int64_t rot;
  float eps;
  float next_eps;
  int32_t row_gemms;
  int64_t tn_slab_floats;
  int32_t max_workgroups;
} dl_dit_block_t;
DL_API int dl_dit_block_fwd(const dl_dit_block_t* blk, int train, dl_stream_t stream);
DL_API int dl_dit_block_fwd_chain(const dl_dit_block_t* blk, int train, dl_stream_t stream);
DL_API int dl_dit_block_bwd(const dl_dit_block_t* blk, dl_stream_t main_stream, dl_stream_t side_stream, int side_workgroups);

#ifdef __cplusplus
}
#endif
#endif
```

Measured before the change: 12960.

## Fuse LN2 backward with dA GEMM per sample and defer QK-scale folds

Adds a per-sample kernel that runs the LayerNorm-2 backward row GEMM and then the dA GEMM that consumes its dt1 in one launch. The two steps are separated by a phase sync inside the kernel, which removes a kernel boundary and lets dt1 be reused while it is still hot. The stationary GEMM body gets a new epilogue variant that skips the sum-of-squares work. Separately, the QK-norm scale partials from each block's in-place backward are kept in per-block slices and folded once for all blocks with a new batched fold kernel, instead of a small fold launch on the main chain of every block. This costs extra workspace memory and relies on shape constraints (N=256, D=384) that limit where the fused path applies.

```diff
diff --git a/diffulab_amd/_lib.py b/diffulab_amd/_lib.py
--- a/diffulab_amd/_lib.py
+++ b/diffulab_amd/_lib.py
@@ -19,7 +19,8 @@
 }
 
 
-_VALUE_RETURNING = {"dl_version", "dl_mse_loss_partials", "dl_grad_sumsq", "dl_muon_orthogonalize"}
+_VALUE_RETURNING = {"dl_version", "dl_mse_loss_partials", "dl_grad_sumsq", "dl_muon_orthogonalize",
+                    "dl_qk_norm_rope_bwd_inplace_parts"}
 
 
 def _ctype_of(decl: str):
diff --git a/diffulab_amd/csrc/block.hip b/diffulab_amd/csrc/block.hip
--- a/diffulab_amd/csrc/block.hip
+++ b/diffulab_amd/csrc/block.hip
@@ -142,7 +142,14 @@
   }
   RUN(wgrad(P(DU), 2 * F, P(XM2), D, P(G_UP), 2 * F, D));
   const bool rows = (b->row_gemms & 1) != 0, fold_here = (b->row_gemms & 4) == 0;
-  if (rows) {
+  bool da_done = false;
+  if (rows && (b->row_gemms & 32)) {
+    const int rc = dl_dit_block_bwd_ln2_da(b, main_);
+    if (rc != DL_ERR_UNSUPPORTED && rc != DL_OK) return rc;
+    da_done = rc == DL_OK;
+  }
+  if (da_done) {
+  } else if (rows) {
     RUN(dl_ln_modulate_gemm_bwd(P(DU), 2 * F, P(WT_UP), b->ldwt_f2, M, 2 * F, P(X1), (const float*)P(LN2_W), (const float*)P(LN2_B),
                                 P(SCALE2), b->ld_mod, N, (const float*)P(MEAN2), (const float*)P(RSTD2), P(DX_IN), P(DX_MID),
                                 (float*)P(DSCALE2), (float*)P(DSHIFT2), b->ld_dmod, (float*)P(DWB2), P(T1), P(GATE1), b->ld_mod, P(DT1),
@@ -156,13 +163,15 @@
   }
   if (fold_here) RUN(fold(P(DWB2), P(G_LN2)));
   RUN(wgrad(P(DT1), D, P(A), D, P(G_PROJ), D, D));
-  RUN(dl_gemm_nt(P(DT1), D, P(WT_PROJ), b->ldwt_d, P(DA), D, M, D, D, nullptr, DL_ACT_NONE, DL_BF16, nullptr, nullptr, 0, nullptr, 0, 1, main));
+  if (!da_done)
+    RUN(dl_gemm_nt(P(DT1), D, P(WT_PROJ), b->ldwt_d, P(DA), D, M, D, D, nullptr, DL_ACT_NONE, DL_BF16, nullptr, nullptr, 0, nullptr, 0, 1, main));
   const bool v_in_place = P(V) == nullptr;
   if (v_in_place && P(QK_PARTIALS) && D <= 512) {
     RUN(dl_attn_bwd_tok(P(Q), P(K), P(QKV), P(A), P(DA), (const float*)P(LSE), P(DQKV), B, H, N, dh, sm, main));
     RUN(dl_qk_norm_rope_bwd_inplace(P(QKV), (const float*)P(QN_SCALE), (const float*)P(KN_SCALE), (const float*)P(ROPE_COS),
-                                    (const float*)P(ROPE_SIN), (const float*)P(RRMS), P(DQKV), (float*)P(G_QK_SCALE),
-                                    (float*)P(QK_PARTIALS), B, N, H, dh, b->rot, nullptr, main));
+                                    (const float*)P(ROPE_SIN), (const float*)P(RRMS), P(DQKV),
+                                    (b->row_gemms & 16) ? nullptr : (float*)P(G_QK_SCALE), (float*)P(QK_PARTIALS), B, N, H, dh, b->rot,
+                                    nullptr, main));
   } else {
     if (v_in_place)
       RUN(dl_attn_bwd_sv(P(Q), P(K), (const char*)P(QKV) + 2 * D * 2, N * 3 * D, dh, 3 * D, P(A), P(DA), (const float*)P(LSE), P(DQ), P(DK),
diff --git a/diffulab_amd/csrc/block_fused.hip b/diffulab_amd/csrc/block_fused.hip
--- a/diffulab_amd/csrc/block_fused.hip
+++ b/diffulab_amd/csrc/block_fused.hip
@@ -83,8 +83,95 @@
   }
 }
 
+struct BwdLn2DaArgs {
+  int B;
+  ChainRowGemm ln2;
+  StArgs da;
+};
+static __device__ __forceinline__ const BwdLn2DaArgs* ch_bwd_args() {
+  auto p = __builtin_amdgcn_kernarg_segment_ptr();
+  asm volatile("" : "+s"(p));
+  return (const BwdLn2DaArgs*)p;
+}
+static __device__ __forceinline__ void ch_row_gemm_bwd(const ChainRowGemm* gp, char* smem, int sample) {
+  const ChainRowGemm g = *gp;
+  rk_gemm_body<RK_LNB>(g.A, g.lda, g.W, g.ldw, RK_BN, g.K, g.ep, smem, ch_tid(), sample, 0, 1);
+}
+__global__ __launch_bounds__(CH_THREADS, 2) void dit_block_bwd_ln2_da_k(BwdLn2DaArgs a) {
+  extern __shared__ __attribute__((aligned(16))) char smem[];
+  for (int s = blockIdx.x; s < a.B; s += gridDim.x) {
+    ch_row_gemm_bwd(&ch_bwd_args()->ln2, smem, s);
+    ch_phase_sync();
+    ch_st_gemm<2>(&ch_bwd_args()->da, smem, s);
+    ch_phase_sync();
+  }
+}
+
 #define P(k) (b->p[DL_BLK_##k])
 #define CH_ALIGNED16(p) ((((uintptr_t)(p)) & 15) == 0)
+
+extern "C" int dl_dit_block_bwd_ln2_da(const dl_dit_block_t* b, dl_stream_t stream) {
+  DL_CHECK_ARG(b, "dl_dit_block_bwd_ln2_da: null block");
+  const int64_t B = b->B, N = b->N, D = b->D, F = b->F;
+  DL_CHECK_ARG(B > 0 && N > 0 && D > 0 && F > 0, "dl_dit_block_bwd_ln2_da: bad dims");
+  if (!(b->row_gemms & 1) || N != RK_BM || D != RK_BN || (2 * F) % RK_BK || B * N >= (1ll << 31) || F >= (1ll << 29)) {
+    dl_set_error("dl_dit_block_bwd_ln2_da: needs row_gemms bit 0, N == 256, D == 384, 2F %% 64 == 0 (N=%lld D=%lld F=%lld)", (long long)N,
+                 (long long)D, (long long)F);
+    return DL_ERR_UNSUPPORTED;
+  }
+  DL_CHECK_ARG(P(DU) && P(WT_UP) && P(X1) && P(SCALE2) && P(MEAN2) && P(RSTD2) && P(DX_MID) && P(DSCALE2) && P(DSHIFT2) && P(T1) && P(GATE1) &&
+                   P(DT1) && P(DGATE1) && P(WT_PROJ) && P(DA),
+               "dl_dit_block_bwd_ln2_da: null operand");
+  DL_CHECK_ARG((P(LN2_W) == nullptr) == (P(LN2_B) == nullptr), "dl_dit_block_bwd_ln2_da: LayerNorm w and b must both be given or both NULL");
+  DL_CHECK_ARG(b->ldwt_f2 % 8 == 0 && b->ldwt_d % 8 == 0 && b->ldwt_f2 >= 2 * F && b->ldwt_d >= D && b->ldwt_d < (1ll << 24) &&
+                   b->ld_mod % 8 == 0 && b->ldwt_f2 * (int64_t)RK_BN < (1ll << 30),
+               "dl_dit_block_bwd_ln2_da: leading dimensions");
+  DL_CHECK_ARG(CH_ALIGNED16(P(DU)) && CH_ALIGNED16(P(WT_UP)) && CH_ALIGNED16(P(X1)) && CH_ALIGNED16(P(SCALE2)) && CH_ALIGNED16(P(DX_IN)) &&
+                   CH_ALIGNED16(P(DX_MID)) && CH_ALIGNED16(P(T1)) && CH_ALIGNED16(P(GATE1)) && CH_ALIGNED16(P(DT1)) && CH_ALIGNED16(P(LN2_W)) &&
+                   CH_ALIGNED16(P(WT_PROJ)) && CH_ALIGNED16(P(DA)),
+               "dl_dit_block_bwd_ln2_da: 16-byte alignment");
+  BwdLn2DaArgs a{};
+  a.B = (int)B;
+  a.ln2.A = (const bf16_t*)P(DU);
+  a.ln2.lda = 2 * F;
+  a.ln2.W = (const bf16_t*)P(WT_UP);
+  a.ln2.ldw = b->ldwt_f2;
+  a.ln2.K = (int)(2 * F);
+  RowEpi& ep = a.ln2.ep;
+  ep.x = (const bf16_t*)P(X1);
+  ep.ln_w = (const float*)P(LN2_W);
+  ep.ln_b = (const float*)P(LN2_B);
+  ep.scale = (const bf16_t*)P(SCALE2);
+  ep.ld_mod = b->ld_mod;
+  ep.mean_i = (const float*)P(MEAN2);
+  ep.rstd_i = (const float*)P(RSTD2);
+  ep.dres = (const bf16_t*)P(DX_IN);
+  ep.dx = (bf16_t*)P(DX_MID);
+  ep.dscale = (float*)P(DSCALE2);
+  ep.dshift = (float*)P(DSHIFT2);
+  ep.ld_dmod = b->ld_dmod;
+  ep.dwb = (float*)P(DWB2);
+  ep.gt = (const bf16_t*)P(T1);
+  ep.gate = (const bf16_t*)P(GATE1);
+  ep.ld_gate = b->ld_mod;
+  ep.gdt = (bf16_t*)P(DT1);
+  ep.dgate = (float*)P(DGATE1);
+  a.da = StArgs{(const bf16_t*)P(DT1), D, (const bf16_t*)P(WT_PROJ), b->ldwt_d, (bf16_t*)P(DA), D, nullptr, 0, 0, nullptr, 0, (int)(B * N),
+                (int)D};
+
+  constexpr int LDS = ch_lds_bytes();
+  static DevOnce once;
+  const int n_cu = dev_cus(once, [] {
+    (void)hipFuncSetAttribute((const void*)dit_block_bwd_ln2_da_k, hipFuncAttributeMaxDynamicSharedMemorySize, LDS);
+  });
+  const DlWgCapScope cap_scope(b->max_workgroups);
+  const int budget = dl_wg_budget(n_cu);
+  int grid = (int)(B < budget ? B : budget);
+  if (b->max_workgroups > 0 && b->max_workgroups < grid) grid = b->max_workgroups;
+  hipLaunchKernelGGL(dit_block_bwd_ln2_da_k, grid, CH_THREADS, LDS, (hipStream_t)stream, a);
+  DL_LAUNCH_CHECK();
+  return DL_OK;
+}
 
 static void ch_row_epi(RowEpi& ep, const void* resid, const void* gate, int64_t ld_gate, const void* ln_w, const void* ln_b,
                        const void* scale, const void* shift, int64_t ld_mod, float eps, void* t_out, void* x_out, void* xm_out,
diff --git a/diffulab_amd/csrc/gemm_stationary_body.h b/diffulab_amd/csrc/gemm_stationary_body.h
--- a/diffulab_amd/csrc/gemm_stationary_body.h
+++ b/diffulab_amd/csrc/gemm_stationary_body.h
@@ -152,11 +152,14 @@
           }
           const u32x4_t pk = pack8(v);
           *(u32x4_t*)(a.C + (int64_t)m * a.ldc + n_base + j * 32 + 16 * gp + 8 * hi) = pk;
-          float r[8];
-          unpack8(pk, r);
-#pragma unroll
-          for (int e = 0; e < 8; ++e) ss += r[e] * r[e];
-        }
+          if constexpr (EPI == 1) {
+            float r[8];
+            unpack8(pk, r);
+#pragma unroll
+            for (int e = 0; e < 8; ++e) ss += r[e] * r[e];
+          }
+        }
+      if constexpr (EPI == 1) {
       if (st % 6 == 2) {
         ss_lo = xor32_sum(ss);
         ss = 0.f;
@@ -168,6 +171,7 @@
         }
         ss = 0.f;
         ss_lo = 0.f;
+      }
       }
     }
   };
@@ -178,7 +182,7 @@
     constexpr int YOUNG = (NST - 2) * NKS;
     if (it + NST - 2 < total) {
       if (st < 2) st_wait_vmcnt<YOUNG>();
-      else if (EPI == 1) st_wait_vmcnt<YOUNG + 4>();
+      else if (EPI != 0) st_wait_vmcnt<YOUNG + 4>();
       else if (a.C) st_wait_vmcnt<YOUNG + 6>();
       else st_wait_vmcnt<YOUNG + 2>();
     } else {
diff --git a/diffulab_amd/csrc/norm.hip b/diffulab_amd/csrc/norm.hip
--- a/diffulab_amd/csrc/norm.hip
+++ b/diffulab_amd/csrc/norm.hip
@@ -1383,10 +1383,13 @@
   qk_norm_rope_bwd_inplace_body<3>(qkv, sq, sk, cs, sn, rrms, dqkv, partials, M, N, H, dh, rot, pos);
 }
 #define FOLD_LANES 16
-__global__ __launch_bounds__(64 * FOLD_LANES) void fold_rows_k(const float* __restrict__ partial, float* __restrict__ out, int G, int n) {
+__global__ __launch_bounds__(64 * FOLD_LANES) void fold_rows_k(const float* __restrict__ partial, float* __restrict__ out, int G, int n,
+                                                               int64_t pstride, int64_t ostride) {
   __shared__ float red[FOLD_LANES][64];
   const int cl = threadIdx.x & 63, rl = threadIdx.x >> 6;
   const int c = blockIdx.x * 64 + cl;
+  partial += (int64_t)blockIdx.y * pstride;
+  out += (int64_t)blockIdx.y * ostride;
   float a0 = 0.f, a1 = 0.f, a2 = 0.f, a3 = 0.f;
   if (c < n) {
     const float* p = partial + c;
@@ -1409,15 +1412,31 @@
   if (rl == 0 && c < n) out[c] += (red[0][cl] + red[1][cl]) + (red[2][cl] + red[3][cl]);
 }
 int dl_fold_rows_launch(const float* partial, float* out, int G, int n, hipStream_t stream) {
-  hipLaunchKernelGGL(fold_rows_k, cdiv(n, 64), 64 * FOLD_LANES, 0, stream, partial, out, G, n);
+  hipLaunchKernelGGL(fold_rows_k, cdiv(n, 64), 64 * FOLD_LANES, 0, stream, partial, out, G, n, (int64_t)0, (int64_t)0);
   DL_LAUNCH_CHECK();
   return DL_OK;
 }
+extern "C" int dl_fold_rows_batched_f32(const float* partial, int64_t partial_stride, float* out, int64_t out_stride, int64_t K, int64_t G,
+                                        int64_t n, dl_stream_t stream) {
+  DL_CHECK_ARG(partial && out && K > 0 && K < 65536 && G > 0 && G < (1 << 24) && n > 0 && n < (1 << 24),
+               "dl_fold_rows_batched_f32: bad args (K < 65536; G, n < 2^24)");
+  DL_CHECK_ARG(K == 1 || (partial_stride >= G * n && out_stride >= n), "dl_fold_rows_batched_f32: problems overlap (strides %lld / %lld)",
+               (long long)partial_stride, (long long)out_stride);
+  hipLaunchKernelGGL(fold_rows_k, dim3(cdiv(n, 64), (unsigned)K), 64 * FOLD_LANES, 0, (hipStream_t)stream, partial, out, (int)G, (int)n,
+                     partial_stride, out_stride);
+  DL_LAUNCH_CHECK();
+  return DL_OK;
+}
+static int qki_grid(int64_t M) {
+  const int64_t grid = cdiv(M, M >= 32768 ? 4 * 16 : 4 * 4);
+  return grid > 768 ? 768 : (int)grid;
+}
+extern "C" int dl_qk_norm_rope_bwd_inplace_parts(int64_t B, int64_t N) { return B > 0 && N > 0 ? qki_grid(B * N) : 0; }
 extern "C" int dl_qk_norm_rope_bwd_inplace(const void* qkv, const float* scale_q, const float* scale_k, const float* cos,
                                            const float* sin, const float* rrms, void* dqkv, float* dscale, float* dscale_partials,
                                            int64_t B, int64_t N, int64_t H, int64_t dh, int64_t rot, const int32_t* pos,
                                            dl_stream_t stream) {
-  DL_CHECK_ARG(qkv && scale_q && scale_k && cos && sin && rrms && dqkv && dscale && dscale_partials && B > 0 && N > 0,
+  DL_CHECK_ARG(qkv && scale_q && scale_k && cos && sin && rrms && dqkv && dscale_partials && B > 0 && N > 0,
                "dl_qk_norm_rope_bwd_inplace: null operand");
   const int64_t D = H * dh;
   if (D > 512 || D % 8) {
@@ -1428,12 +1447,13 @@
   DL_CHECK_ARG((((uintptr_t)qkv | (uintptr_t)dqkv | (uintptr_t)cos | (uintptr_t)sin) & 15) == 0,
                "dl_qk_norm_rope_bwd_inplace: 16-byte alignment");
   const int64_t M = B * N;
-  int grid = cdiv(M, M >= 32768 ? 4 * 16 : 4 * 4);
-  if (grid > 768) grid = 768;
+  const int grid = qki_grid(M);
   const size_t lds = (size_t)4 * 2 * D * sizeof(float);
   hipLaunchKernelGGL(qk_norm_rope_bwd_inplace_k, grid, 256, lds, (hipStream_t)stream, (const bf16_t*)qkv, scale_q, scale_k, cos, sin,
                      rrms, (bf16_t*)dqkv, dscale_partials, M, (int)N, (int)H, (int)dh, (int)rot, pos);
-  hipLaunchKernelGGL(fold_rows_k, cdiv(2 * D, 64), 64 * FOLD_LANES, 0, (hipStream_t)stream, dscale_partials, dscale, grid, (int)(2 * D));
+  if (dscale)
+    hipLaunchKernelGGL(fold_rows_k, cdiv(2 * D, 64), 64 * FOLD_LANES, 0, (hipStream_t)stream, dscale_partials, dscale, grid, (int)(2 * D),
+                       (int64_t)0, (int64_t)0);
   DL_LAUNCH_CHECK();
   return DL_OK;
 }
diff --git a/diffulab_amd/engine.py b/diffulab_amd/engine.py
--- a/diffulab_amd/engine.py
+++ b/diffulab_amd/engine.py
@@ -523,6 +523,8 @@
             if ops.v_in_place(N) and D <= 512 and M >= 32768 and type(self) is DiTEngine and tuning.on("DL_QK_INPLACE"):
                 w["qk_part"] = torch.empty(1024 * 2 * D, device=self.dev, dtype=f32)
                 w["dq"] = w["dk"] = None
+                if self._row_gemms(M, N) and tuning.on("DL_QK_FOLD_DEFER"):
+                    w["qk_part_all"] = torch.empty(L, ops.QK_PART_ROWS, 2 * D, device=self.dev, dtype=f32)
             else:
                 w["dq"], w["dk"] = z(B, d.num_heads, Nd, 64), z(B, d.num_heads, Nd, 64)
             w["dv"] = None if ops.v_in_place(N) else z(B, d.num_heads, Nd, 64)
@@ -640,7 +642,7 @@
             blk.set(next_ln_w=lnw, next_ln_b=lnb, next_scale=mrow(mn), next_shift=mrow(mn + D),
                     next_x=xs[i + 1] if train else xs[(i + 1) & 1], next_xm=xm_n, next_mean=mu_n, next_rstd=rs_n)
             blk.row_gemms = (1 | (2 if tuning.on("DL_ROW_GEMM_QK") else 0) | (4 if self.reducer is None else 0)
-                             | (8 if tuning.on("DL_BLOCK_CHAIN") else 0))
+                             | (8 if tuning.on("DL_BLOCK_CHAIN") else 0) | (32 if tuning.on("DL_BWD_LN2_DA") else 0))
         if train and self.grads is not None:
             g, dmod = w["wg"][i], w["dmod32"]
             blk.ld_dmod = dmod.stride(0)
@@ -660,6 +662,9 @@
                     g_ln1=self.G(pre + "norm_1.weight"), g_ln2=self.G(pre + "norm_2.weight"),
                     g_qk_scale=self.G(pre + "attention.qk_norm.query_norm.scale"), tn_slab=w.get("tn_slab"),
                     qk_partials=w.get("qk_part"))
+            if rows and self._defer_qk():
+                blk.set(qk_partials=w["qk_part_all"][i])
+                blk.row_gemms |= 16
             blk.tn_slab_floats = w["tn_slab"].numel() if "tn_slab" in w else 0
         self._blk_cache[key] = blk
         return blk
@@ -790,16 +795,17 @@
         return nx
 
     def _attn_bwd(self, a: dict, g: dict, nm: dict, s: dict, nt: int, cos: Tensor, sin: Tensor, pos: Tensor | None,
-                  kb: Tensor | None, dao: Tensor | None) -> None:
+                  kb: Tensor | None, dao: Tensor | None, qk_parts: Tensor | None = None) -> None:
         w = self.ws
         B, Hh, D, rot = self.geo[0], self.d.num_heads, self.d.inner_dim, sum(self.d.rope_axes_dim)
         sq, sk = self.P(nm["qk"] + ".query_norm.scale"), self.P(nm["qk"] + ".key_norm.scale")
         dscale = self._qk_scale_sink(nm["qk"]) if self._input_only else self.G(nm["qk"] + ".query_norm.scale")
         if ops.qk_inplace_ok(w, B, nt):
             ops.attn_bwd_tok(a["q"], a["k"], a["qkv"], a["a"], s["da"], a["lse"], g["dqkv"], B, Hh, nt, 64, 64**-0.5)
-            _must(ops.qk_norm_rope_bwd_inplace(a["qkv"], sq, sk, cos, sin, a["rrms"], g["dqkv"], dscale, w["qk_part"], B, nt, Hh, 64, rot,
-                                                pos=pos))
+            _must(ops.qk_norm_rope_bwd_inplace(a["qkv"], sq, sk, cos, sin, a["rrms"], g["dqkv"], None if qk_parts is not None else dscale,
+                                                qk_parts if qk_parts is not None else w["qk_part"], B, nt, Hh, 64, rot, pos=pos))
             return
+        assert qk_parts is None
         v_in_place = ops.v_in_place(nt)
         if a.get("ao") is not None:
             Np = a["q"].shape[2]
@@ -827,6 +833,9 @@
     def _qkn_on_load(self, M: int, N: int) -> bool:
         return (self._row_gemms(M, N) and self.d.inner_dim % 384 == 0 and (M // 256) * (3 * self.d.inner_dim // 384) >= 64
                 and tuning.on("DL_QKN_ON_LOAD") and not tuning.on("DL_ROW_GEMM_QK"))
+
+    def _defer_qk(self) -> bool:
+        return self.ws.get("qk_part_all") is not None and self.reducer is None
 
     def _row_gemms(self, M: int, N: int) -> bool:
         return type(self) is DiTEngine and ops.v_in_place(N) and ops.row_gemm_ok(M, self.d.inner_dim, N)
@@ -1030,6 +1039,7 @@
         native = self._native_blocks() and not serial
         inline_wgrad = tuning.on("DL_WGRAD_INLINE")
         defer_fold = fused and self.reducer is None
+        defer_qk = fused and self._defer_qk()
         for i in reversed(range(L)):
             dres = dfeats.get(i - 1)
             if native:
@@ -1037,7 +1047,7 @@
                 blk.set(dfeat=dres)
                 ops.dit_block_bwd(blk, main.cuda_stream, main.cuda_stream if inline_wgrad else side.cuda_stream, sw.side_wgs)
             elif fused:
-                dx = self._block_bwd_row_gemms(i, dx, dres, s, sw, not defer_fold)
+                dx = self._block_bwd_row_gemms(i, dx, dres, s, sw, not defer_fold, defer_qk)
             else:
                 prev = (w["layers"][i - 1]["t2"], (i - 1) * 6 * D + 5 * D, w["wg"][i - 1]["dt2"]) if i > 0 else None
                 m = Modulation(mod, dmod, i * 6 * D, D, N, part=(w["dwb"][2 * i], w["dwb"][2 * i + 1]), groups=B)
@@ -1052,6 +1062,11 @@
             stride = ent[self.prefixes[1] + "norm_1.weight"][0] - ent[self.prefixes[0] + "norm_1.weight"][0] if L > 1 else 0
             for j, nm in enumerate(("norm_1.weight", "norm_2.weight")):
                 ops.reduce_rows_batched_f32(w["dwb"][j], 2 * B * 2 * D, self.G(self.prefixes[0] + nm), stride, L, B, 2 * D)
+        if defer_qk:
+            ent, qn = self.layout.entries, "attention.qk_norm.query_norm.scale"
+            stride = ent[self.prefixes[1] + qn][0] - ent[self.prefixes[0] + qn][0] if L > 1 else 0
+            ops.fold_rows_batched_f32(w["qk_part_all"], ops.QK_PART_ROWS * 2 * D, self.G(self.prefixes[0] + qn), stride, L,
+                                      ops.qk_inplace_parts(B, N), 2 * D)
 
         self._cond_bwd(dx)
         if join_last:
@@ -1110,7 +1125,8 @@
                                          kb=w.get("kb"), dao=w.get("dao"))
         return self._input_grad(dx)
 
-    def _block_bwd_row_gemms(self, i: int, dx: Tensor, dres: Tensor | None, s: dict, sw: "SideWork", fold: bool) -> Tensor:
+    def _block_bwd_row_gemms(self, i: int, dx: Tensor, dres: Tensor | None, s: dict, sw: "SideWork", fold: bool,
+                             defer_qk: bool = False) -> Tensor:
         d, w, sh = self.d, self.ws, self.sh
         _, _, _, gh, gw, N, _, _, _ = self.geo
         D = d.inner_dim
@@ -1130,7 +1146,7 @@
         dx = nx
         sw.wgrad(g["dt1"], a["a"], nm["proj"] + ".weight")
         ops.gemm_nt(g["dt1"], sh[nm["proj"] + ".weight|t"], s["da"])
-        self._attn_bwd(a, g, nm, s, N, *self._rope[(gh, gw)], None, None, None)
+        self._attn_bwd(a, g, nm, s, N, *self._rope[(gh, gw)], None, None, None, qk_parts=w["qk_part_all"][i] if defer_qk else None)
         sw.wgrad(g["dqkv"], a["xm1"], nm["qkv"] + ".weight")
         if dres is not None:
             ops.add_bf16(dx, dres, dx)
diff --git a/diffulab_amd/ops.py b/diffulab_amd/ops.py
--- a/diffulab_amd/ops.py
+++ b/diffulab_amd/ops.py
@@ -826,6 +826,10 @@
     _call("dl_dit_block_bwd", ctypes.addressof(blk), main_stream, side_stream, int(side_wgs))
 
 
+def dit_block_bwd_ln2_da(blk) -> bool:
+    return _maybe("dl_dit_block_bwd_ln2_da", ctypes.addressof(blk), _s())
+
+
 def attn_fwd_qkv(q, k, qkv, out, lse, B, H, N, dh, scale):
     D = H * dh
     _call("dl_attn_fwd_sv", _p(q), _p(k), qkv.data_ptr() + 2 * D * 2, N * 3 * D, dh, 3 * D, _p(out), _p(lse), B, H, N, dh,
@@ -859,9 +863,20 @@
 
 
 def qk_norm_rope_bwd_inplace(qkv, scale_q, scale_k, cos, sin, rrms, dqkv, dscale, partials, B, N, H, dh, rot, pos=None) -> bool:
-    assert partials.numel() >= 1024 * 2 * H * dh and partials.dtype == torch.float32
+    assert partials.numel() >= (1024 if dscale is not None else QK_PART_ROWS) * 2 * H * dh and partials.dtype == torch.float32
     return _maybe("dl_qk_norm_rope_bwd_inplace", _p(qkv), _p(scale_q), _p(scale_k), _p(cos), _p(sin), _p(rrms), _p(dqkv), _p(dscale),
                   _p(partials), B, N, H, dh, rot, _p(pos), _s())
+
+
+QK_PART_ROWS = 768
+
+
+def qk_inplace_parts(B: int, N: int) -> int:
+    return lib().call("dl_qk_norm_rope_bwd_inplace_parts", B, N)
+
+
+def fold_rows_batched_f32(partial, partial_stride, out, out_stride, K, G, n):
+    _call("dl_fold_rows_batched_f32", _p(partial), partial_stride, _p(out), out_stride, K, G, n, _s())
 
 
 def attn_fwd_ex(q, k, v, out, lse, B, H, Nq, Nk, dh, scale, key_bias=None):
diff --git a/diffulab_amd/tuning.py b/diffulab_amd/tuning.py
--- a/diffulab_amd/tuning.py
+++ b/diffulab_amd/tuning.py
@@ -11,9 +11,14 @@
                        "forward stages q and k (dl_attn_fwd_qkn): no qk_norm_rope_fwd pass (row-complete path, <= 256 tokens)"),
     "DL_BLOCK_CHAIN": ("1", "block forward of the row-complete path as one per-sample chain launch (dl_dit_block_fwd_chain; native block "
                        "driver, 256 tokens per sample, QK-norm on load)"),
+    "DL_BWD_LN2_DA": ("1", "block backward of the row-complete path: the LayerNorm-2 backward GEMM and the dA GEMM that reads its dt1 as one "
+                      "per-sample launch (dl_dit_block_bwd_ln2_da; native block driver, 256 tokens per sample); bit-identical"),
     "DL_MLP_RECOMPUTE": ("1", "SwiGLU backward recomputes the MLP-up pre-activations instead of storing them in the forward"),
     "DL_ATTN_V_IN_PLACE": ("1", "attention reads V / writes dV inside the token-major qkv rows (N <= 256)"),
     "DL_QK_INPLACE": ("1", "attention backward writes dQ / dK token-major and the QK-norm backward runs in place on the dqkv rows"),
+    "DL_QK_FOLD_DEFER": ("1", "row-complete path, no gradient reducer: the QK-scale partials of the in-place QK-norm backward stay in a "
+                         "per-block slice and ONE launch folds all blocks after the last block's backward (dl_fold_rows_batched_f32; "
+                         "row_gemms bit 4) instead of a 12-workgroup fold on the main chain of every block; bit-identical"),
     "DL_WGRAD_GROUP": ("1", "the four weight gradients of a block as one atomics-free launch (dl_gemm_tn_group)"),
     "DL_WGRAD_INLINE": ("0", "grouped weight gradients on the main stream instead of the side stream"),
     "DL_WGRAD_SERIAL": ("0", "per-problem weight gradients on the main stream (engines without the grouped form)"),
diff --git a/include/diffulab_hip.h b/include/diffulab_hip.h
--- a/include/diffulab_hip.h
+++ b/include/diffulab_hip.h
@@ -243,6 +243,9 @@
                                        const float* sin, const float* rrms, void* dqkv, float* dscale, float* dscale_partials,
                                        int64_t B, int64_t N, int64_t H, int64_t dh, int64_t rot, const int32_t* pos,
                                        dl_stream_t stream);
+DL_API int dl_qk_norm_rope_bwd_inplace_parts(int64_t B, int64_t N);
+DL_API int dl_fold_rows_batched_f32(const float* partial, int64_t partial_stride, float* out, int64_t out_stride, int64_t K,
+                                    int64_t G, int64_t n, dl_stream_t stream);
 DL_API int dl_attn_fwd(const void* q, const void* k, const void* v, void* out, float* lse, int64_t B, int64_t H,
                        int64_t N, int64_t dh, float scale, dl_stream_t stream);
 DL_API int dl_attn_bwd(const void* q, const void* k, const void* v, const void* out, const void* dout,
@@ -599,6 +602,7 @@
 DL_API int dl_dit_block_fwd(const dl_dit_block_t* blk, int train, dl_stream_t stream);
 DL_API int dl_dit_block_fwd_chain(const dl_dit_block_t* blk, int train, dl_stream_t stream);
 DL_API int dl_dit_block_bwd(const dl_dit_block_t* blk, dl_stream_t main_stream, dl_stream_t side_stream, int side_workgroups);
+DL_API int dl_dit_block_bwd_ln2_da(const dl_dit_block_t* blk, dl_stream_t stream);
 
 #ifdef __cplusplus
 }
```

New measurement: 13070 (median of 6 runs). No clear change (+0.8%).
